# WesleyHsieh0806/TAO-Amodal

Measured on AMD Instinct MI355X. Metric: box-pair IoU+match throughput, higher is better.
Workload: dtype f64

## Files before the change

include/tao_amodal_hip.h:

```cpp
#ifndef TAO_AMODAL_HIP_H
#define TAO_AMODAL_HIP_H

#include <stddef.h>
#include <stdint.h>

#ifdef __cplusplus
extern "C" {
#endif

#define TAOAMD_N_THR 10
#define TAOAMD_N_REC 101
#define TAOAMD_LVIS_RNG 6
#define TAOAMD_TAO_RNG 20

#define TAOAMD_GT_IGNORE 1
#define TAOAMD_GT_OOF 2
#define TAOAMD_GT_ID_HIDDEN 4
#define TAOAMD_DT_IGNORE_UNMATCHED 1
#define TAOAMD_DT_NO_CONSUME 2

#define TAOAMD_OK 0
#define TAOAMD_ERR_HIP 1
#define TAOAMD_ERR_ARG 2
#define TAOAMD_ERR_TOO_LARGE 3
#define TAOAMD_ERR_WORKSPACE 4
#define TAOAMD_JSON_FALLBACK 16

const char *taoamd_strerror(int status);
const char *taoamd_last_error(void);
int taoamd_version(void);

int taoamd_kernel_timing_enable(int on);
int taoamd_kernel_timing_label(const char *label);
int taoamd_kernel_timing_collect(char *names_host, size_t names_bytes,
                                 double *total_ms_host, int64_t *calls_host,
                                 int32_t max_kernels, int32_t *n_kernels_host);

int taoamd_thresholds_host(double *iou_thrs, double *rec_thrs);

int taoamd_set_thresholds(const double *iou_thrs, const double *rec_thrs);
int taoamd_set_ranges(const double *visibility_rng, const double *area_rng,
                      const double *time_rng);

int taoamd_bb_iou(const double *dt, const double *gt, size_t m, size_t n,
                  const unsigned char *iscrowd, double *o, void *stream);
int taoamd_bb_iou_host(const double *dt, const double *gt, size_t m, size_t n,
                       const unsigned char *iscrowd, double *o);

int taoamd_lvis_ranges(int64_t n_gt, const double *gt_vis,
                       const uint8_t *gt_flags, const int32_t *gt_cat,
                       const int32_t *gt_cat_off, int64_t n_dt,
                       const uint8_t *dt_flags, int32_t n_cat,
                       uint32_t *gt_rng, uint32_t *dt_rng, int32_t *num_gt,
                       void *stream);
int taoamd_tao_ranges(int64_t n_gt, const double *gt_area,
                      const int32_t *gt_len, const int32_t *gt_nhp,
                      const uint8_t *gt_flags, const int32_t *gt_cat,
                      const int32_t *gt_cat_off, int64_t n_dt,
                      const double *dt_area, const int32_t *dt_len,
                      const uint8_t *dt_flags, int32_t n_cat,
                      uint32_t *gt_rng, uint32_t *dt_rng, int32_t *num_gt,
                      void *stream);

size_t taoamd_rle_iou_workspace(int64_t n_dt, int64_t dt_total, int64_t n_gt,
                                int64_t gt_total);
int taoamd_rle_iou(int64_t n_cells, const int32_t *cell_dt_off,
                   const int32_t *cell_gt_off, const int64_t *cell_iou_off,
                   int64_t n_dt, int64_t dt_total, const int64_t *dt_off,
                   const uint32_t *dt_runs, const int32_t *dt_hw,
                   const double *dt_bb, int64_t n_gt, int64_t gt_total,
                   const int64_t *gt_off, const uint32_t *gt_runs,
                   const int32_t *gt_hw, const double *gt_bb, double *iou,
                   void *workspace, size_t workspace_bytes, void *stream);

size_t taoamd_track_mask_iou_workspace(int64_t dt_frames, int64_t dt_total,
                                       int64_t gt_frames, int64_t gt_total);
int taoamd_track_mask_iou(int64_t n_cells, const int32_t *cell_dt_off,
                          const int32_t *cell_gt_off, const int64_t *cell_iou_off,
                          int64_t n_pairs, const int32_t *dt_frame_off,
                          const int32_t *dt_frame_pos, int64_t dt_frames,
                          int64_t dt_total, const int64_t *dt_off,
                          const uint32_t *dt_runs, const int32_t *dt_hw,
                          const int32_t *gt_frame_off,
                          const int32_t *gt_frame_pos, int64_t gt_frames,
                          int64_t gt_total, const int64_t *gt_off,
                          const uint32_t *gt_runs, const int32_t *gt_hw,
                          int32_t mode, double *iou,
                          int64_t *pair_frames, void *workspace,
                          size_t workspace_bytes, void *stream);

int taoamd_track_iou(int64_t n_cells, const int32_t *cell_dt_off,
                     const int32_t *cell_gt_off, const int64_t *cell_iou_off,
                     int64_t n_pairs, const int32_t *dt_frame_off,
                     const int32_t *dt_frame_pos, const double *dt_frame_box,
                     const int32_t *gt_frame_off, const int32_t *gt_frame_pos,
                     const double *gt_frame_box, int32_t mode, double *iou,
                     int64_t *pair_frames, void *stream);
int taoamd_track_iou_planned(int64_t n_tasks, const int32_t *tasks,
                             const int32_t *task_rows, const int32_t *task_pairs,
                             const int64_t *task_out, const double *frames,
                             const int32_t *task_base, const int32_t *trk_meta,
                             int32_t mode, double *iou, int64_t *pair_frames,
                             void *stream);

int taoamd_track_iou_single(int64_t n_dt, const int32_t *dt_group,
                            const int64_t *cell_iou_off, const int32_t *dt_frame_pos,
                            const double *dt_frame_box, const int32_t *gt_frame_pos,
                            const double *gt_frame_box, int32_t mode, double *iou,
                            int64_t *pair_frames, void *stream);

int taoamd_track_pad(int64_t n_trk, int64_t n_frames, const int32_t *frame_off,
                     const int32_t *frame_pos, const double *frame_box,
                     const int32_t *meta, int64_t slot_first, int64_t n_slots,
                     double *padded, int32_t *inexact, void *stream);

int taoamd_track_stream(int64_t n_tasks, const int32_t *tasks,
                        const int32_t *task_rows, const int32_t *trk_meta,
                        const int32_t *task_base, const double *padded,
                        double *frames, void *stream);

int taoamd_track_iou_near(int64_t n_cells, const int32_t *cell_gt_off,
                          const int64_t *cell_iou_off, int64_t n_pairs,
                          const double *iou, int32_t max_ulp, int32_t capacity,
                          int32_t *count, int64_t *list, void *stream);

int64_t taoamd_track_iou_setorder_table(int64_t max_dt_frames, int64_t max_gt_frames);
int taoamd_track_iou_setorder(
    int64_t n_cells, const int32_t *cell_dt_off, const int32_t *cell_gt_off,
    const int64_t *cell_iou_off, const int32_t *cell_unit, const int64_t *tl_vid_start,
    const int64_t *tl_image_id, const int32_t *dt_frame_off, const int32_t *dt_frame_pos,
    const double *dt_frame_box, const int32_t *gt_frame_off, const int32_t *gt_frame_pos,
    const double *gt_frame_box, int32_t mode, const int32_t *count, int32_t capacity,
    const int64_t *list, double *iou, int32_t *scratch, int64_t scratch_slots,
    int64_t table_cap, int32_t *status, void *stream);

int taoamd_set_order_iou_host(const int64_t *tl_image_id, int32_t n_dt,
                              const int32_t *dt_pos, const double *dt_box, int32_t n_gt,
                              const int32_t *gt_pos, const double *gt_box, int32_t mode,
                              double *out);
int taoamd_pyset_union_order_host(int64_t n_a, const int64_t *a, int64_t n_b,
                                  const int64_t *b, int64_t *out, int64_t *n_out);

int taoamd_track_iou_plan_host(int64_t n_cells, const int32_t *cell_dt_off_host,
                               const int32_t *cell_gt_off_host,
                               const int64_t *cell_iou_off_host,
                               const int32_t *trk_meta_host, int64_t *sizes,
                               int32_t *tasks_host, int32_t *task_rows_host,
                               int32_t *task_pairs_host, int64_t *task_out_host);

#define TAOAMD_MAX_GT_PER_CELL 3072
int taoamd_match(int64_t n_cells, const int32_t *cell_dt_off,
                 const int32_t *cell_gt_off, const int64_t *cell_iou_off,
                 int32_t max_gt_per_cell, const double *dt_box,
                 const double *gt_box, const double *iou, int32_t n_rng,
                 const uint32_t *gt_rng, const uint32_t *dt_rng,
                 const uint8_t *gt_flags, const uint8_t *dt_flags,
                 const int32_t *dst, int64_t out_stride, uint64_t *matched,
                 uint64_t *ignored, int32_t *match_gt, double *ious_out,
                 const int32_t *dt_group, const uint32_t *dt_meta,
                 const int32_t *groups, int32_t n_groups, const int32_t *singles,
                 int32_t n_singles, void *stream);

int taoamd_flat_map(int64_t n, const int64_t *image_id, const int64_t *category_id,
                    const double *bbox, const double *area_in, int64_t n_img,
                    const int64_t *img_ids, int64_t n_cat, const int64_t *cat_ids,
                    int32_t *img, int32_t *cat, double *area, int32_t *img_count,
                    int32_t *img_start, int32_t *img_first, int32_t *status,
                    void *stream);
int taoamd_flat_rank_drop(int64_t n, const int32_t *order, const int32_t *img,
                          const int32_t *img_start, int32_t max_dets,
                          uint8_t *dropped, void *stream);
int taoamd_flat_filter(int64_t n, const int32_t *unit, const int32_t *cat,
                       const double *area, const int64_t *category_id,
                       const uint8_t *dropped, int32_t n_unit, int64_t n_gkeys,
                       const int32_t *gkeys, const int32_t *unit_row,
                       const int64_t *neg_off, const int64_t *neg_val,
                       const int64_t *nel_off, const int64_t *nel_val,
                       int32_t area_flag, int32_t *key, uint8_t *flags,
                       int32_t *n_keep, void *stream);
int taoamd_flat_gather(int64_t n_keep, const int32_t *order, const double *score,
                       const uint8_t *flags, const int32_t *key,
                       const double *bbox, int32_t n_unit, int32_t *dt_row,
                       double *dt_score, uint8_t *dt_flags, int32_t *dt_key,
                       int32_t *dt_cat, double *dt_box, void *stream);
int taoamd_flat_count_bad(int64_t n, const double *bbox, const uint8_t *dropped,
                          int32_t *count, void *stream);
int taoamd_flat_ordscore(int64_t n, const int32_t *img, const int32_t *img_count,
                         const double *score, int32_t max_dets, double *out,
                         void *stream);
int taoamd_flat_ordinal(int64_t n, const int32_t *order, const int32_t *img,
                        const int32_t *img_start, int32_t max_dets,
                        int32_t *ordinal, uint8_t *dropped, void *stream);
int taoamd_flat_merge_cat(int64_t n, const int64_t *category_id, int64_t n_merge,
                          const int64_t *merge_src, const int64_t *merge_dst,
                          int64_t n_cat, const int64_t *cat_ids, int64_t *merged_id,
                          int32_t *cat, void *stream);
int taoamd_flat_split64(int64_t n, const int64_t *key, const int32_t *order,
                        int32_t *lo, int32_t *hi, void *stream);
int taoamd_flat_compose(int64_t n, const int32_t *outer, const int32_t *inner,
                        int32_t *out, void *stream);
int taoamd_flat_gather_cols(int64_t n, const int32_t *idx, const int32_t *src_i32,
                            int32_t *out_i32, const double *src_f64,
                            double *out_f64, const uint8_t *src_u8,
                            uint8_t *out_u8, void *stream);
int taoamd_flat_track_of(int64_t n, const int32_t *order, const int32_t *run_id,
                         const int32_t *run_start, const int64_t *video_id,
                         int32_t *trk, int32_t *status, void *stream);
int taoamd_flat_keys(int64_t n, const int32_t *img, const int32_t *ordinal,
                     const uint8_t *dropped, const int32_t *cat, const double *area,
                     const int32_t *trk, const int32_t *img_rank,
                     const int32_t *visit_rank, const double *img_frame,
                     const int32_t *tl_pos, double M, double *keep_key,
                     double *visit_key, double *frame_key, double *pos_key,
                     int32_t *trk_keep, int32_t *trk_sel, void *stream);
int taoamd_flat_track_kept(int64_t n_runs, const int32_t *run_trk,
                           const int32_t *run_start, int64_t n_sorted,
                           const int32_t *order_k, const double *score,
                           const int64_t *merged_id, double *trk_score,
                           int32_t *trk_first_kept, int32_t *status, void *stream);
int taoamd_flat_track_sel(int64_t n_runs, const int32_t *run_trk,
                          const int32_t *run_start, int64_t n_sorted,
                          const int32_t *order_s, const double *area,
                          const double *visit_key, const int32_t *img,
                          double *sel_area, int32_t *sel_len, int32_t *sel_frames,
                          double *sel_first, void *stream);
int taoamd_flat_track_filter(int64_t n_runs, const int32_t *run_trk,
                             const int32_t *sel_len, const int32_t *trk_first_kept,
                             const int32_t *cat, const int64_t *merged_id,
                             const int64_t *video_id, const int64_t *track_id,
                             int64_t n_vid, const int64_t *vid_ids, int64_t n_gkeys,
                             const int32_t *gkeys, const int32_t *vid_row,
                             const int64_t *neg_off, const int64_t *neg_val,
                             const int64_t *nel_off, const int64_t *nel_val,
                             int32_t *key, uint8_t *flags, int32_t *n_keep,
                             int32_t *status, void *stream);
int taoamd_flat_frames(int64_t n_trk, const int32_t *trk_run,
                       const int32_t *run_start, int64_t n_runs, int64_t n_sorted,
                       const int32_t *order_s, const int32_t *img,
                       const int32_t *tl_pos, const double *bbox,
                       const int32_t *frame_off, int32_t *frame_pos,
                       double *frame_box, void *stream);
int taoamd_flat_scan(int64_t n, const int32_t *count, int32_t *start,
                     int32_t *status2, void *stream);
size_t taoamd_flat_runs_workspace(int64_t n);
int taoamd_flat_runs(int64_t n, const int32_t *sorted_key, int32_t *run_id,
                     int32_t *run_key, int32_t *run_start, int32_t *n_runs,
                     void *workspace, size_t workspace_bytes, void *stream);
int taoamd_flat_runs_by(int64_t n, const int32_t *key, const int32_t *order,
                        int32_t *run_id, int32_t *run_key, int32_t *run_start,
                        int32_t *n_runs, void *workspace, size_t workspace_bytes,
                        void *stream);
int taoamd_flat_runs64_by(int64_t n, const int64_t *key, const int32_t *order,
                          int32_t *run_id, int64_t *run_key, int32_t *run_start,
                          int32_t *n_runs, void *workspace, size_t workspace_bytes,
                          void *stream);
int taoamd_flat_remap(int64_t n, const int32_t *id, const int32_t *map,
                      int32_t *out, void *stream);

int taoamd_match_plan_host(int64_t n_cells, const int32_t *cell_dt_off_host,
                           const int32_t *cell_gt_off_host, int32_t cap_d,
                           int32_t cap_g, int32_t cap_cell_g, int64_t *sizes,
                           int32_t *groups_host, int32_t *singles_host);

size_t taoamd_sort_workspace(int64_t n);
int taoamd_sort_by_cat_score(int64_t n, const int32_t *dt_cat,
                             const double *dt_score, int32_t *order,
                             int32_t *dst, void *workspace,
                             size_t workspace_bytes, void *stream);

#define TAOAMD_SORT_CHUNK (16 * 2816)
int taoamd_sort_plan_host(int32_t n_cat, const int32_t *cat_off_host, int64_t *sizes,
                          int32_t *chunks, int32_t *split_list, int32_t *stile_chunk,
                          int32_t *bucket_chunk);
size_t taoamd_sort_sampled_workspace(int64_t n, int64_t n_buckets, int32_t merge);
int taoamd_sort_sampled_cap_limit(int32_t limit);
int taoamd_sort_sampled_notify(void *event);
int taoamd_event_create(void **event);
int taoamd_event_destroy(void *event);
int taoamd_stream_wait_event(void *stream, void *event);
int taoamd_sort_sampled(int64_t n, int32_t n_cat, const int32_t *cat_off,
                        const int32_t *tile_off, int32_t n_tiles, int32_t max_segment,
                        const double *dt_score, int32_t n_chunks, const int32_t *chunks,
                        int32_t n_split, const int32_t *split_list, int32_t n_stiles,
                        const int32_t *stile_chunk, int32_t n_buckets,
                        const int32_t *bucket_chunk, int32_t *order, int32_t *dst,
                        void *workspace, size_t workspace_bytes, void *stream);

#define TAOAMD_SEGMENT_TILE 2816
size_t taoamd_sort_segments_workspace(int64_t n);
int taoamd_sort_segments(int64_t n, int32_t n_cat, const int32_t *cat_off,
                         const int32_t *tile_off, int32_t n_tiles,
                         int32_t max_segment, const int32_t *dt_cat,
                         const double *dt_score, int32_t *order, int32_t *dst,
                         void *workspace, size_t workspace_bytes, void *stream);

int taoamd_gather_rows(int64_t n, int32_t n_words, const uint64_t *src_matched,
                       const uint64_t *src_ignored, int64_t src_stride,
                       const int32_t *order, uint64_t *dst_matched,
                       uint64_t *dst_ignored, void *stream);

size_t taoamd_accumulate_workspace(int64_t n_dt, int32_t n_cat, int32_t n_rng);
size_t taoamd_compact_elems(int32_t n_cat, int32_t n_rng);
int taoamd_accumulate_compact(int64_t n_dt, int32_t n_cat, int32_t n_rng,
                              const int32_t *cat_off, const uint64_t *matched,
                              const uint64_t *ignored, const int32_t *num_gt,
                              int32_t k_begin, int32_t k_end, int32_t max_segment,
                              double *val, double *rec, void *workspace,
                              size_t workspace_bytes, void *stream);
int taoamd_finalize(int32_t n_cat, int32_t n_rng, const int32_t *num_gt,
                    const double *val, const double *rec, double *precision,
                    double *recall, void *stream);
int taoamd_accumulate(int64_t n_dt, int32_t n_cat, int32_t n_rng,
                      const int32_t *cat_off, const uint64_t *matched,
                      const uint64_t *ignored,
                      const int32_t *num_gt, int32_t max_segment, double *precision,
                      double *recall, void *workspace, size_t workspace_bytes,
                      void *stream);
int taoamd_accumulate_error(const void *workspace, void *stream, int32_t *flag_host);
int taoamd_accumulate_chunked(int64_t n_dt, int32_t n_cat, int32_t n_rng,
                      const int32_t *cat_off, const uint64_t *matched,
                      const uint64_t *ignored,
                      const int32_t *num_gt, int32_t max_segment, double *precision,
                      double *recall, void *workspace, size_t workspace_bytes,
                      void *stream);
int taoamd_accumulate_compact_chunked(int64_t n_dt, int32_t n_cat, int32_t n_rng,
                              const int32_t *cat_off, const uint64_t *matched,
                              const uint64_t *ignored, const int32_t *num_gt,
                              int32_t k_begin, int32_t k_end, int32_t max_segment,
                              double *val, double *rec, void *workspace,
                              size_t workspace_bytes, void *stream);
int taoamd_accumulate_sweep_mode(int32_t mode);
int taoamd_accumulate_plan_kind(int64_t n_dt, int32_t n_rng, int32_t max_segment);
int taoamd_accumulate_spin_limit(int32_t polls);
int taoamd_accumulate_giveup_counter(uint32_t *device_word);
int taoamd_accumulate_prepare(int64_t n_dt, int32_t n_cat, int32_t n_rng,
                              const int32_t *cat_off, int32_t max_segment,
                              void *workspace, size_t workspace_bytes, void *stream);
int taoamd_accumulate_prepared(int64_t n_dt, int32_t n_cat, int32_t n_rng,
                      const int32_t *cat_off, const uint64_t *matched,
                      const uint64_t *ignored,
                      const int32_t *num_gt, int32_t max_segment, double *precision,
                      double *recall, void *workspace, size_t workspace_bytes,
                      void *stream);
int taoamd_accumulate_by_order(int64_t n_dt, int32_t n_cat, int32_t n_rng,
                               const int32_t *cat_off, const int32_t *order,
                               const uint64_t *matched, const uint64_t *ignored,
                               const int32_t *num_gt, int32_t max_segment,
                               double *precision, double *recall, void *workspace,
                               size_t workspace_bytes, void *stream);
int taoamd_accumulate_by_order_prepared(int64_t n_dt, int32_t n_cat, int32_t n_rng,
                               const int32_t *cat_off, const int32_t *order,
                               const uint64_t *matched, const uint64_t *ignored,
                               const int32_t *num_gt, int32_t max_segment,
                               double *precision, double *recall, void *workspace,
                               size_t workspace_bytes, void *stream);
int taoamd_accumulate_by_order_chunked(int64_t n_dt, int32_t n_cat, int32_t n_rng,
                               const int32_t *cat_off, const int32_t *order,
                               const uint64_t *matched, const uint64_t *ignored,
                               const int32_t *num_gt, int32_t max_segment,
                               double *precision, double *recall, void *workspace,
                               size_t workspace_bytes, void *stream);

size_t taoamd_score_at_recall_workspace(int64_t n_dt, int32_t n_cat, int32_t n_rng);
int taoamd_score_at_recall(int64_t n_dt, int32_t n_cat, int32_t n_rng,
                           const int32_t *cat_off, const int32_t *order,
                           const uint64_t *matched, const uint64_t *ignored,
                           const double *score, const int32_t *score_order,
                           const int32_t *num_gt, double *scores, void *workspace, size_t workspace_bytes,
                           void *stream);

#define TAOAMD_ERROR_TYPES_TILE 256
#define TAOAMD_ERROR_TYPES_MAX_RNG 8
size_t taoamd_error_types_workspace(int64_t n_dt, int64_t n_gt, int32_t n_rng);
int taoamd_error_types(int64_t n_dt, int64_t n_gt, int32_t n_img, int32_t n_cat,
                       int32_t n_rng, int32_t slot, double bg_thr,
                       const int32_t *dt_cat, const double *dt_box,
                       const uint8_t *dt_flags, const int32_t *dt_gt0,
                       const int32_t *match_gt, int64_t match_stride,
                       const int32_t *gt_cat, const double *gt_box,
                       const uint32_t *gt_rng, const int32_t *img_gt_off,
                       const int32_t *img_gt, const int32_t *img_dt_off,
                       const int32_t *img_dt, int64_t *dt_counts, int64_t *gt_counts,
                       uint8_t *dt_type, void *workspace, size_t workspace_bytes,
                       void *stream);

#define TAOAMD_TRACK_ERROR_TYPES_TILE 16
size_t taoamd_track_error_types_workspace(int64_t n_dt, int64_t n_gt, int32_t n_rng);
int taoamd_track_error_types(int64_t n_dt, int64_t n_gt, int64_t n_cells, int64_t n_iou,
                             int32_t n_vid, int32_t n_cat, int32_t n_rng, int32_t slot,
                             double bg_thr, const int32_t *dt_cat, const uint32_t *dt_rng,
                             const int32_t *dt_group, const int64_t *cell_iou_off,
                             const double *iou, const int32_t *match_gt, int64_t match_stride,
                             const int32_t *gt_cat, const uint32_t *gt_rng,
                             const int32_t *dt_frame_off, const int32_t *dt_frame_pos,
                             const double *dt_frame_box, const int32_t *gt_frame_off,
                             const int32_t *gt_frame_pos, const double *gt_frame_box,
                             const int32_t *vid_gt_off, const int32_t *vid_gt,
                             const int32_t *vid_dt_off, const int32_t *vid_dt,
                             int64_t *dt_counts, int64_t *gt_counts, uint8_t *dt_type,
                             uint32_t *dt_over, void *workspace, size_t workspace_bytes,
                             void *stream);

size_t taoamd_exchange_chunk_bytes(int32_t block_cats, int32_t n_rng, int64_t capacity);
size_t taoamd_exchange_workspace(int32_t block_cats, int32_t n_rng, int32_t world);
int taoamd_exchange_sizes(int32_t block_cats, int32_t n_rng, int32_t world,
                          const int32_t *num_gt, int64_t *totals, void *workspace,
                          size_t workspace_bytes, void *stream);
int taoamd_exchange_pack(int32_t n_cat, int32_t n_rng, int32_t block_cats,
                         int32_t world, int32_t rank, const int32_t *num_gt,
                         const double *val, const double *rec, void *chunk,
                         int64_t capacity, int32_t *overflow, void *workspace,
                         size_t workspace_bytes, int32_t maps_ready, void *stream);
int taoamd_exchange_unpack(int32_t n_cat, int32_t n_rng, int32_t block_cats,
                           int32_t world, const void *chunks, int64_t capacity,
                           int32_t *num_gt_out, double *precision, double *recall,
                           int32_t *overflow, void *workspace,
                           size_t workspace_bytes, int32_t maps_ready, void *stream);

int taoamd_exchange_scores(int64_t n, const int32_t *dst, const double *score,
                           int64_t *out, void *stream);
int taoamd_exchange_positions(int64_t n_recv, int32_t world, int32_t block_cats,
                              const int64_t *scores, const int64_t *own_scores,
                              int32_t own_rank, const int64_t *src_base,
                              const int64_t *run_off, const int64_t *cat_base,
                              int32_t *pos, void *stream);
int taoamd_exchange_place(int64_t n_recv, int32_t world, int32_t n_words,
                          const uint64_t *rows, const uint64_t *own_rows,
                          int32_t own_rank, const int64_t *src_base,
                          const int32_t *pos, uint64_t *out, void *stream);

size_t taoamd_json_pred_workspace(size_t file_bytes);
void *taoamd_json_pred_open(const char *path, void *work, size_t work_bytes,
                            int32_t *status, char *err, size_t errlen, void *stream);
int64_t taoamd_json_pred_count(void *handle);
int taoamd_json_pred_convert(void *handle, int64_t *image_id, int64_t *category_id,
                             double *bbox, double *score, int64_t *track_id,
                             int64_t *video_id, int64_t *flag, int64_t *flag_at,
                             int32_t flag_cap, int32_t *n_flagged);
int taoamd_json_pred_read(void *handle, int64_t *image_id, int64_t *category_id,
                          double *bbox, double *score, int64_t *track_id,
                          int64_t *video_id, int64_t *flag, int64_t *flag_at,
                          int32_t flag_cap, int32_t *n_flagged);
void taoamd_json_pred_close(void *handle);

#ifdef __cplusplus
}
#endif
#endif
```

tao_amodal_amd/_lib.py:

```python
import ctypes as C
import os

HERE = os.path.dirname(os.path.abspath(__file__))
SO_PATH = os.environ.get("TAOAMD_LIBRARY") or os.path.join(HERE, "libtao_amodal_hip.so")

OK = 0
ERR_HIP, ERR_ARG, JSON_FALLBACK = 1, 2, 16
N_THR, N_REC = 10, 101
LVIS_RNG, TAO_RNG = 6, 20
MAX_GT_PER_CELL = 3072
SEGMENT_TILE = 2816
ERROR_TYPES_TILE = 256
TRACK_ERROR_TYPES_TILE = 16
ERROR_TYPES = ("TP", "IGNORED", "DUP", "LOC", "CLS", "BOTH", "BKG")

_vp, _i64, _i32, _sz = C.c_void_p, C.c_int64, C.c_int32, C.c_size_t

SIGNATURES = {
    "taoamd_strerror": (C.c_char_p, [C.c_int]),
    "taoamd_last_error": (C.c_char_p, []),
    "taoamd_version": (C.c_int, []),
    "taoamd_thresholds_host": (C.c_int, [_vp, _vp]),
    "taoamd_set_thresholds": (C.c_int, [_vp, _vp]),
    "taoamd_set_ranges": (C.c_int, [_vp, _vp, _vp]),
    "taoamd_kernel_timing_enable": (C.c_int, [C.c_int]),
    "taoamd_kernel_timing_label": (C.c_int, [C.c_char_p]),
    "taoamd_kernel_timing_collect": (C.c_int, [_vp, _sz, _vp, _vp, _i32, _vp]),
    "taoamd_bb_iou": (C.c_int, [_vp, _vp, _sz, _sz, _vp, _vp, _vp]),
    "taoamd_bb_iou_host": (C.c_int, [_vp, _vp, _sz, _sz, _vp, _vp]),
    "taoamd_lvis_ranges": (C.c_int, [_i64, _vp, _vp, _vp, _vp, _i64, _vp,
                                     _i32, _vp, _vp, _vp, _vp]),
    "taoamd_tao_ranges": (C.c_int, [_i64, _vp, _vp, _vp, _vp, _vp, _vp, _i64,
                                    _vp, _vp, _vp, _i32, _vp, _vp, _vp, _vp]),
    "taoamd_sort_segments_workspace": (_sz, [_i64]),
    "taoamd_sort_segments": (C.c_int, [_i64, _i32, _vp, _vp, _i32, _i32, _vp,
                                       _vp, _vp, _vp, _vp, _sz, _vp]),
    "taoamd_sort_plan_host": (C.c_int, [_i32, _vp, _vp, _vp, _vp, _vp, _vp]),
    "taoamd_sort_sampled_workspace": (_sz, [_i64, _i64, _i32]),
    "taoamd_sort_sampled_cap_limit": (C.c_int, [_i32]),
    "taoamd_sort_sampled_notify": (C.c_int, [_vp]),
    "taoamd_event_create": (C.c_int, [_vp]),
    "taoamd_event_destroy": (C.c_int, [_vp]),
    "taoamd_stream_wait_event": (C.c_int, [_vp, _vp]),
    "taoamd_sort_sampled": (C.c_int, [_i64, _i32, _vp, _vp, _i32, _i32, _vp, _i32, _vp,
                                      _i32, _vp, _i32, _vp, _i32, _vp, _vp, _vp, _vp,
                                      _sz, _vp]),
    "taoamd_track_iou": (C.c_int, [_i64, _vp, _vp, _vp, _i64, _vp, _vp, _vp,
                                   _vp, _vp, _vp, _i32, _vp, _vp, _vp]),
    "taoamd_track_iou_single": (C.c_int, [_i64, _vp, _vp, _vp, _vp, _vp, _vp, _i32,
                                          _vp, _vp, _vp]),
    "taoamd_track_iou_planned": (C.c_int, [_i64, _vp, _vp, _vp, _vp, _vp, _vp, _vp,
                                           _i32, _vp, _vp, _vp]),
    "taoamd_track_stream": (C.c_int, [_i64, _vp, _vp, _vp, _vp, _vp, _vp, _vp]),
    "taoamd_json_pred_workspace": (_sz, [_sz]),
    "taoamd_json_pred_open": (_vp, [C.c_char_p, _vp, _sz, _vp, C.c_char_p, _sz, _vp]),
    "taoamd_json_pred_count": (_i64, [_vp]),
    "taoamd_json_pred_read": (C.c_int, [_vp, _vp, _vp, _vp, _vp, _vp, _vp, _vp, _vp,
                                        _i32, _vp]),
    "taoamd_json_pred_convert": (C.c_int, [_vp, _vp, _vp, _vp, _vp, _vp, _vp, _vp, _vp,
                                           _i32, _vp]),
    "taoamd_json_pred_close": (None, [_vp]),
    "taoamd_track_pad": (C.c_int, [_i64, _i64, _vp, _vp, _vp, _vp, _i64, _i64,
                                   _vp, _vp, _vp]),
    "taoamd_track_iou_near": (C.c_int, [_i64, _vp, _vp, _i64, _vp, _i32, _i32,
                                        _vp, _vp, _vp]),
    "taoamd_track_iou_setorder_table": (_i64, [_i64, _i64]),
    "taoamd_track_iou_setorder": (C.c_int, [_i64, _vp, _vp, _vp, _vp, _vp, _vp, _vp,
                                            _vp, _vp, _vp, _vp, _vp, _i32, _vp, _i32,
                                            _vp, _vp, _vp, _i64, _i64, _vp, _vp]),
    "taoamd_set_order_iou_host": (C.c_int, [_vp, _i32, _vp, _vp, _i32, _vp, _vp,
                                            _i32, _vp]),
    "taoamd_pyset_union_order_host": (C.c_int, [_i64, _vp, _i64, _vp, _vp, _vp]),
    "taoamd_track_iou_plan_host": (C.c_int, [_i64, _vp, _vp, _vp, _vp, _vp,
                                             _vp, _vp, _vp, _vp]),
    "taoamd_flat_map": (C.c_int, [_i64, _vp, _vp, _vp, _vp, _i64, _vp, _i64, _vp,
                                  _vp, _vp, _vp, _vp, _vp, _vp, _vp, _vp]),
    "taoamd_flat_count_bad": (C.c_int, [_i64, _vp, _vp, _vp, _vp]),
    "taoamd_flat_ordscore": (C.c_int, [_i64, _vp, _vp, _vp, _i32, _vp, _vp]),
    "taoamd_flat_ordinal": (C.c_int, [_i64, _vp, _vp, _vp, _i32, _vp, _vp, _vp]),
    "taoamd_flat_merge_cat": (C.c_int, [_i64, _vp, _i64, _vp, _vp, _i64, _vp, _vp,
                                        _vp, _vp]),
    "taoamd_flat_split64": (C.c_int, [_i64, _vp, _vp, _vp, _vp, _vp]),
    "taoamd_flat_compose": (C.c_int, [_i64, _vp, _vp, _vp, _vp]),
    "taoamd_flat_gather_cols": (C.c_int, [_i64, _vp, _vp, _vp, _vp, _vp, _vp, _vp,
                                          _vp]),
    "taoamd_flat_track_of": (C.c_int, [_i64, _vp, _vp, _vp, _vp, _vp, _vp, _vp]),
    "taoamd_flat_keys": (C.c_int, [_i64, _vp, _vp, _vp, _vp, _vp, _vp, _vp, _vp,
                                   _vp, _vp, C.c_double, _vp, _vp, _vp, _vp, _vp,
                                   _vp, _vp]),
    "taoamd_flat_track_kept": (C.c_int, [_i64, _vp, _vp, _i64, _vp, _vp, _vp, _vp,
                                         _vp, _vp, _vp]),
    "taoamd_flat_track_sel": (C.c_int, [_i64, _vp, _vp, _i64, _vp, _vp, _vp, _vp,
                                        _vp, _vp, _vp, _vp, _vp]),
    "taoamd_flat_track_filter": (C.c_int, [_i64, _vp, _vp, _vp, _vp, _vp, _vp, _vp,
                                           _i64, _vp, _i64, _vp, _vp, _vp, _vp, _vp,
                                           _vp, _vp, _vp, _vp, _vp, _vp]),
    "taoamd_flat_frames": (C.c_int, [_i64, _vp, _vp, _i64, _i64, _vp, _vp, _vp,
                                     _vp, _vp, _vp, _vp, _vp]),
    "taoamd_flat_scan": (C.c_int, [_i64, _vp, _vp, _vp, _vp]),
    "taoamd_flat_runs_by": (C.c_int, [_i64, _vp, _vp, _vp, _vp, _vp, _vp, _vp, _sz,
                                      _vp]),
    "taoamd_flat_runs64_by": (C.c_int, [_i64, _vp, _vp, _vp, _vp, _vp, _vp, _vp,
                                        _sz, _vp]),
    "taoamd_flat_rank_drop": (C.c_int, [_i64, _vp, _vp, _vp, _i32, _vp, _vp]),
    "taoamd_flat_filter": (C.c_int, [_i64, _vp, _vp, _vp, _vp, _vp, _i32, _i64,
                                     _vp, _vp, _vp, _vp, _vp, _vp, _i32, _vp, _vp,
                                     _vp, _vp]),
    "taoamd_flat_gather": (C.c_int, [_i64, _vp, _vp, _vp, _vp, _vp, _i32, _vp,
                                     _vp, _vp, _vp, _vp, _vp, _vp]),
    "taoamd_flat_runs_workspace": (_sz, [_i64]),
    "taoamd_flat_runs": (C.c_int, [_i64, _vp, _vp, _vp, _vp, _vp, _vp, _sz, _vp]),
    "taoamd_flat_remap": (C.c_int, [_i64, _vp, _vp, _vp, _vp]),
    "taoamd_match_plan_host": (C.c_int, [_i64, _vp, _vp, _i32, _i32, _i32, _vp,
                                         _vp, _vp]),
    "taoamd_match": (C.c_int, [_i64, _vp, _vp, _vp, _i32, _vp, _vp, _vp, _i32,
                               _vp, _vp, _vp, _vp, _vp, _i64, _vp, _vp, _vp,
                               _vp, _vp, _vp, _vp, _i32, _vp, _i32, _vp]),
    "taoamd_gather_rows": (C.c_int, [_i64, _i32, _vp, _vp, _i64, _vp, _vp,
                                     _vp, _vp]),
    "taoamd_compact_elems": (_sz, [_i32, _i32]),
    "taoamd_accumulate_compact": (C.c_int, [_i64, _i32, _i32, _vp, _vp, _vp,
                                            _vp, _i32, _i32, _i32, _vp, _vp,
                                            _vp, _sz, _vp]),
    "taoamd_rle_iou_workspace": (_sz, [_i64, _i64, _i64, _i64]),
    "taoamd_rle_iou": (C.c_int, [_i64, _vp, _vp, _vp, _i64, _i64, _vp, _vp, _vp,
                                 _vp, _i64, _i64, _vp, _vp, _vp, _vp, _vp, _vp,
                                 _sz, _vp]),
    "taoamd_track_mask_iou_workspace": (_sz, [_i64, _i64, _i64, _i64]),
    "taoamd_track_mask_iou": (C.c_int, [_i64, _vp, _vp, _vp, _i64, _vp, _vp, _i64, _i64,
                                        _vp, _vp, _vp, _vp, _vp, _i64, _i64, _vp, _vp,
                                        _vp, _i32, _vp, _vp, _vp, _sz, _vp]),
    "taoamd_finalize": (C.c_int, [_i32, _i32, _vp, _vp, _vp, _vp, _vp, _vp]),
    "taoamd_exchange_chunk_bytes": (_sz, [_i32, _i32, _i64]),
    "taoamd_exchange_workspace": (_sz, [_i32, _i32, _i32]),
    "taoamd_exchange_sizes": (C.c_int, [_i32, _i32, _i32, _vp, _vp, _vp, _sz, _vp]),
    "taoamd_exchange_pack": (C.c_int, [_i32, _i32, _i32, _i32, _i32, _vp, _vp,
                                       _vp, _vp, _i64, _vp, _vp, _sz, _i32, _vp]),
    "taoamd_exchange_unpack": (C.c_int, [_i32, _i32, _i32, _i32, _vp, _i64, _vp,
                                         _vp, _vp, _vp, _vp, _sz, _i32, _vp]),
    "taoamd_exchange_scores": (C.c_int, [_i64, _vp, _vp, _vp, _vp]),
    "taoamd_exchange_positions": (C.c_int, [_i64, _i32, _i32, _vp, _vp, _i32, _vp, _vp,
                                            _vp, _vp, _vp]),
    "taoamd_exchange_place": (C.c_int, [_i64, _i32, _i32, _vp, _vp, _i32, _vp, _vp, _vp,
                                        _vp]),
    "taoamd_sort_workspace": (_sz, [_i64]),
    "taoamd_sort_by_cat_score": (C.c_int, [_i64, _vp, _vp, _vp, _vp, _vp, _sz,
                                           _vp]),
    "taoamd_accumulate_workspace": (_sz, [_i64, _i32, _i32]),
    "taoamd_accumulate": (C.c_int, [_i64, _i32, _i32, _vp, _vp, _vp, _vp, _i32,
                                    _vp, _vp, _vp, _sz, _vp]),
    "taoamd_accumulate_error": (C.c_int, [_vp, _vp, _vp]),
    "taoamd_accumulate_chunked": (C.c_int, [_i64, _i32, _i32, _vp, _vp, _vp, _vp, _i32,
                                            _vp, _vp, _vp, _sz, _vp]),
    "taoamd_accumulate_compact_chunked": (C.c_int, [_i64, _i32, _i32, _vp, _vp, _vp,
                                                    _vp, _i32, _i32, _i32, _vp, _vp,
                                                    _vp, _sz, _vp]),
    "taoamd_accumulate_sweep_mode": (C.c_int, [_i32]),
    "taoamd_accumulate_plan_kind": (C.c_int, [_i64, _i32, _i32]),
    "taoamd_accumulate_spin_limit": (C.c_int, [_i32]),
    "taoamd_accumulate_giveup_counter": (C.c_int, [_vp]),
    "taoamd_accumulate_prepare": (C.c_int, [_i64, _i32, _i32, _vp, _i32, _vp, _sz, _vp]),
    "taoamd_accumulate_prepared": (C.c_int, [_i64, _i32, _i32, _vp, _vp, _vp, _vp, _i32,
                                    _vp, _vp, _vp, _sz, _vp]),
    "taoamd_accumulate_by_order": (C.c_int, [_i64, _i32, _i32, _vp, _vp, _vp, _vp,
                                             _vp, _i32, _vp, _vp, _vp, _sz, _vp]),
    "taoamd_accumulate_by_order_prepared": (C.c_int, [_i64, _i32, _i32, _vp, _vp, _vp, _vp,
                                             _vp, _i32, _vp, _vp, _vp, _sz, _vp]),
    "taoamd_accumulate_by_order_chunked": (C.c_int, [_i64, _i32, _i32, _vp, _vp, _vp, _vp,
                                             _vp, _i32, _vp, _vp, _vp, _sz, _vp]),
    "taoamd_score_at_recall_workspace": (_sz, [_i64, _i32, _i32]),
    "taoamd_score_at_recall": (C.c_int, [_i64, _i32, _i32, _vp, _vp, _vp, _vp, _vp, _vp,
                                         _vp, _vp, _vp, _sz, _vp]),
    "taoamd_error_types_workspace": (_sz, [_i64, _i64, _i32]),
    "taoamd_error_types": (C.c_int, [_i64, _i64, _i32, _i32, _i32, _i32, C.c_double,
                                     _vp, _vp, _vp, _vp, _vp, _i64, _vp, _vp, _vp, _vp,
                                     _vp, _vp, _vp, _vp, _vp, _vp, _vp, _sz, _vp]),
    "taoamd_track_error_types_workspace": (_sz, [_i64, _i64, _i32]),
    "taoamd_track_error_types": (C.c_int, [_i64, _i64, _i64, _i64, _i32, _i32, _i32, _i32,
                                           C.c_double, _vp, _vp, _vp, _vp, _vp, _vp, _i64,
                                           _vp, _vp, _vp, _vp, _vp, _vp, _vp, _vp, _vp, _vp,
                                           _vp, _vp, _vp, _vp, _vp, _vp, _vp, _sz, _vp]),
}

_lib = None


class TaoAmdError(RuntimeError):
    pass


def load():
    global _lib
    if _lib is not None:
        return _lib
    import torch
    if not os.path.exists(SO_PATH):
        raise TaoAmdError(
            "HIP extension not built: %s is missing.  Run "
            "tao_amodal_amd/csrc/build.sh (or __graft_entry__.build()).  "
            "There is no CPU fallback." % SO_PATH)
    lib = C.CDLL(SO_PATH)
    for name, (res, args) in SIGNATURES.items():
        fn = getattr(lib, name)
        fn.restype = res
        fn.argtypes = args
    _lib = lib
    return lib


TIMING = False


def kernel_timing(on):
    global TIMING
    TIMING = bool(on)
    check(load().taoamd_kernel_timing_enable(int(TIMING)),
          "taoamd_kernel_timing_enable")


def kernel_timing_label(label):
    load().taoamd_kernel_timing_label(label.encode() if label else None)


def kernel_timings():
    import numpy as np
    names = C.create_string_buffer(8192)
    ms = np.zeros(128)
    calls = np.zeros(128, dtype=np.int64)
    n = C.c_int32(0)
    check(load().taoamd_kernel_timing_collect(
        C.addressof(names), len(names), ms.ctypes.data, calls.ctypes.data, 128,
        C.addressof(n)), "taoamd_kernel_timing_collect")
    out, raw = {}, names.raw.split(b"\0")
    for k in range(n.value):
        out[raw[k].decode()] = (float(ms[k]), int(calls[k]))
    return out


def set_constants(iou_thrs=None, rec_thrs=None, visibility_rng=None, area_rng=None,
                  time_rng=None):
    import numpy as np

    def arr(a, shape):
        if a is None:
            return None, None
        a = np.ascontiguousarray(a, dtype=np.float64).reshape(shape)
        return a, a.ctypes.data
    lib = load()
    i, ip = arr(iou_thrs, (N_THR,))
    r, rp = arr(rec_thrs, (N_REC,))
    check(lib.taoamd_set_thresholds(ip, rp), "taoamd_set_thresholds")
    v, vp = arr(visibility_rng, (5, 2))
    a, ap = arr(area_rng, (5, 2))
    t, tp = arr(time_rng, (4, 2))
    check(lib.taoamd_set_ranges(vp, ap, tp), "taoamd_set_ranges")


SWEEP_MODES = {"auto": -1, "chunked": 0, "lookback": 1, "twopass": 2}


def sweep_mode(mode="auto", spin_limit=0):
    lib = load()
    check(lib.taoamd_accumulate_sweep_mode(SWEEP_MODES[mode]), "taoamd_accumulate_sweep_mode")
    check(lib.taoamd_accumulate_spin_limit(int(spin_limit)), "taoamd_accumulate_spin_limit")


def check(status, what):
    if status != OK:
        lib = load()
        raise TaoAmdError("%s failed: %s [%s]" % (
            what, lib.taoamd_strerror(status).decode(),
            lib.taoamd_last_error().decode()))
```

tao_amodal_amd/csrc/accumulate.hip:

```cpp
#include <atomic>
#include <cstdlib>
#include <cstring>

#include "common.hpp"
#include "transpose64.hpp"
#include "workspace.hpp"

using namespace taoamd;

#ifndef ACC_CH
#define ACC_CH 256
#endif
#ifndef ACC_INLINE_CHUNKS
#define ACC_INLINE_CHUNKS 64
#endif

struct AccArgs {
    int64_t n_dt;
    int32_t n_cat, n_rng, n_words, n_chunks_max;
    int32_t paired;
    int32_t wide;
    const int32_t *cat_off;
    const uint64_t *matched;
    const uint64_t *ignored;
    const int32_t *order;
    const int32_t *num_gt;
    int32_t *cat_chunk_off;
    const int32_t *chunk_tab;
    uint32_t *cnt_tp, *cnt_fp;
    uint32_t *pre_tp, *pre_fp;
    uint64_t *t_tp, *t_fp;
    uint64_t *cmax;
    int32_t *cj;
    uint64_t *val;
    double *rec;
    int32_t k_begin, k_end;
    int32_t fused_rows;
    int32_t fused_lo;
    int32_t inline_scans;
    int32_t sc_rows;
    uint32_t sc_gen;
    uint64_t *sc_stat;
    uint64_t *sc_max;
    uint8_t *sc_jhi;
    uint32_t *sc_error;
    uint32_t *sc_giveups;
    int32_t *xcd_start;
    int32_t sc_spin;
};

__global__ __launch_bounds__(256) void acc_chunks_kernel(AccArgs a)
{
    __shared__ int32_t part[256];
    const int per = (a.n_cat + 255) / 256;
    const int lo = threadIdx.x * per, hi = min(lo + per, a.n_cat);
    int32_t s = 0;
    auto chunks_of = [&](int k) {
        const int32_t rows = a.cat_off[k + 1] - a.cat_off[k];
        if (a.fused_rows > 0 && rows <= a.fused_rows) return 0;
        if ((a.inline_scans || a.sc_rows) && rows == 0) return 1;
        const int32_t per = a.sc_rows ? a.sc_rows : ACC_CH;
        return (rows + per - 1) / per;
    };
    for (int k = lo; k < hi; k++) s += chunks_of(k);
    part[threadIdx.x] = s;
    __syncthreads();
    for (int off = 1; off < 256; off <<= 1) {
        int32_t v = threadIdx.x >= off ? part[threadIdx.x - off] : 0;
        __syncthreads();
        part[threadIdx.x] += v;
        __syncthreads();
    }
    int32_t run = part[threadIdx.x] - s;
    for (int k = lo; k < hi; k++) {
        a.cat_chunk_off[k] = run;
        run += chunks_of(k);
    }
    if (threadIdx.x == 255) a.cat_chunk_off[a.n_cat] = part[255];
    if (a.xcd_start == nullptr) return;
    __syncthreads();
    if (threadIdx.x <= N_XCD) {
        const int32_t total = part[255];
        const int32_t want = (int32_t)((int64_t)total * threadIdx.x / N_XCD);
        int32_t lo = 0, hi = a.n_cat;
        while (lo < hi) {
            const int32_t mid = (lo + hi) >> 1;
            if (a.cat_chunk_off[mid] < want) lo = mid + 1; else hi = mid;
        }
        a.xcd_start[threadIdx.x] = threadIdx.x == N_XCD ? total : a.cat_chunk_off[lo];
    }
}

__device__ __forceinline__ int32_t chunk_cat(const int32_t *__restrict__ off,
                                             int32_t n_cat, int32_t c)
{
    int32_t lo = 0, hi = n_cat;
    while (hi - lo > 1) {
        int32_t mid = (lo + hi) >> 1;
        if (off[mid] <= c) lo = mid; else hi = mid;
    }
    return lo;
}

__global__ void acc_chunktab_kernel(AccArgs a, int32_t *__restrict__ tab)
{
    const int32_t c = blockIdx.x * blockDim.x + threadIdx.x;
    if (c < a.cat_chunk_off[a.n_cat]) tab[c] = chunk_cat(a.cat_chunk_off, a.n_cat, c);
}

__device__ __forceinline__ uint64_t readlane_u64(uint64_t v, int lane)
{
    uint32_t lo = (uint32_t)__builtin_amdgcn_readlane((int)(uint32_t)v, lane);
    uint32_t hi = (uint32_t)__builtin_amdgcn_readlane((int)(uint32_t)(v >> 32), lane);
    return ((uint64_t)hi << 32) | lo;
}

__device__ __forceinline__ void load_rows(const AccArgs &a, int64_t first, int word,
                                          int n, int lane, uint64_t &tpw,
                                          uint64_t &fpw)
{
    uint64_t m = 0, i = ~0ull;
    if (lane < n) {
        int64_t r = first + lane;
        if (a.order) r = a.order[r];
        if (a.wide) {
            const ulonglong2 v =
                *reinterpret_cast<const ulonglong2 *>(a.matched + 2 * (r * a.n_words + word));
            m = v.x;
            i = v.y;
        } else if (a.paired) {
            m = a.matched[2 * (r * a.n_words + word)];
            i = a.matched[2 * (r * a.n_words + word) + 1];
        } else {
            m = a.matched[r * a.n_words + word];
            i = a.ignored[r * a.n_words + word];
        }
    }
    tpw = m & ~i;
    fpw = ~m & ~i;
}

template <int ACC_BLK_N>
__device__ __forceinline__ void load_chunk(const AccArgs &a, int64_t start, int word, int len,
                                           int lane, uint64_t (&tpw)[ACC_BLK_N],
                                           uint64_t (&fpw)[ACC_BLK_N])
{
    if (a.wide && a.order == nullptr && len > 0) {
        ulonglong2 v[ACC_BLK_N];
#pragma unroll
        for (int blk = 0; blk < ACC_BLK_N; blk++) {
            const int i = blk * WAVE + lane;
            const int64_t r = start + (i < len ? i : 0);
            v[blk] = *reinterpret_cast<const ulonglong2 *>(a.matched + 2 * (r * a.n_words + word));
        }
#pragma unroll
        for (int blk = 0; blk < ACC_BLK_N; blk++) {
            const bool in = blk * WAVE + lane < len;
            const uint64_t m = in ? v[blk].x : 0, i_ = in ? v[blk].y : ~0ull;
            tpw[blk] = m & ~i_;
            fpw[blk] = ~m & ~i_;
        }
        return;
    }
    if (a.wide && a.order != nullptr && len > 0) {
        int32_t at[ACC_BLK_N];
#pragma unroll
        for (int blk = 0; blk < ACC_BLK_N; blk++) {
            const int i = blk * WAVE + lane;
            at[blk] = a.order[start + (i < len ? i : 0)];
        }
        ulonglong2 v[ACC_BLK_N];
#pragma unroll
        for (int blk = 0; blk < ACC_BLK_N; blk++)
            v[blk] = *reinterpret_cast<const ulonglong2 *>(
                a.matched + 2 * ((int64_t)at[blk] * a.n_words + word));
#pragma unroll
        for (int blk = 0; blk < ACC_BLK_N; blk++) {
            const bool in = blk * WAVE + lane < len;
            const uint64_t m = in ? v[blk].x : 0, i_ = in ? v[blk].y : ~0ull;
            tpw[blk] = m & ~i_;
            fpw[blk] = ~m & ~i_;
        }
        return;
    }
#pragma unroll
    for (int blk = 0; blk < ACC_BLK_N; blk++)
        load_rows(a, start + blk * WAVE, word, max(0, min(WAVE, len - blk * WAVE)), lane,
                  tpw[blk], fpw[blk]);
}

template <int ACC_BLK_N, bool GATHER = false>
__device__ __forceinline__ void load_chunk_tv(const AccArgs &a, int64_t start, int word, int len,
                                              int lane, uint64_t (&tpw)[ACC_BLK_N],
                                              uint64_t (&vw)[ACC_BLK_N])
{
    if (GATHER && a.wide && len == ACC_BLK_N * WAVE) {
        const int32_t *__restrict__ ob = a.order + start;
        uint32_t at[ACC_BLK_N];
#pragma unroll
        for (int blk = 0; blk < ACC_BLK_N; blk++) at[blk] = (uint32_t)ob[blk * WAVE + lane];
        const char *base = reinterpret_cast<const char *>(a.matched + 2 * word);
        const uint32_t row_bytes = (uint32_t)a.n_words * 16u;
        ulonglong2 v[ACC_BLK_N];
#pragma unroll
        for (int blk = 0; blk < ACC_BLK_N; blk++)
            v[blk] = *reinterpret_cast<const ulonglong2 *>(base + (uint64_t)at[blk] * row_bytes);
#pragma unroll
        for (int blk = 0; blk < ACC_BLK_N; blk++) {
            tpw[blk] = v[blk].x & ~v[blk].y;
            vw[blk] = ~v[blk].y;
        }
        return;
    }
    if (!GATHER && a.wide && a.order == nullptr && len == ACC_BLK_N * WAVE) {
        const char *base = reinterpret_cast<const char *>(a.matched + 2 * (start * a.n_words + word));
        const uint32_t lane_off = (uint32_t)lane * (uint32_t)a.n_words * 16u;
        const uint32_t blk_off = (uint32_t)WAVE * (uint32_t)a.n_words * 16u;
        ulonglong2 v[ACC_BLK_N];
#pragma unroll
        for (int blk = 0; blk < ACC_BLK_N; blk++)
            v[blk] = *reinterpret_cast<const ulonglong2 *>(base + ((uint32_t)blk * blk_off + lane_off));
#pragma unroll
        for (int blk = 0; blk < ACC_BLK_N; blk++) {
            tpw[blk] = v[blk].x & ~v[blk].y;
            vw[blk] = ~v[blk].y;
        }
        return;
    }
    uint64_t fpw[ACC_BLK_N];
    load_chunk(a, start, word, len, lane, tpw, fpw);
#pragma unroll
    for (int blk = 0; blk < ACC_BLK_N; blk++) vw[blk] = tpw[blk] | fpw[blk];
}

#define ACC_BLK (ACC_CH / WAVE)

struct ChunkInfo {
    int32_t k, first, last;
    int64_t start;
    int32_t len, c, word;
    bool valid;
};

__device__ __forceinline__ ChunkInfo chunk_info(const AccArgs &a)
{
    ChunkInfo ci;
    const int wave = __builtin_amdgcn_readfirstlane(threadIdx.x >> 6);
    const int64_t item = (int64_t)blockIdx.x * 4 + wave;
    ci.c = (int32_t)(item / a.n_words);
    ci.word = (int32_t)(item - (int64_t)ci.c * a.n_words);
    const int32_t total = a.cat_chunk_off[a.n_cat];
    ci.valid = ci.c < total;
    if (!ci.valid) return ci;
    ci.k = a.chunk_tab ? a.chunk_tab[ci.c] : chunk_cat(a.cat_chunk_off, a.n_cat, ci.c);
    const int32_t j = ci.c - a.cat_chunk_off[ci.k];
    ci.start = (int64_t)a.cat_off[ci.k] + (int64_t)j * ACC_CH;
    const int64_t end = a.cat_off[ci.k + 1];
    ci.len = (int32_t)min((int64_t)ACC_CH, end - ci.start);
    ci.first = j == 0;
    ci.last = ci.c + 1 == a.cat_chunk_off[ci.k + 1];
    return ci;
}

__global__ __launch_bounds__(256) void acc_count_kernel(AccArgs a)
{
    const ChunkInfo ci = chunk_info(a);
    if (!ci.valid) return;
    const int lane = lane_id();
    uint32_t tp = 0, fp = 0;
    const int64_t tb = (((int64_t)ci.c * a.n_words + ci.word) * ACC_BLK) * WAVE + lane;
    uint64_t tpw[ACC_BLK], fpw[ACC_BLK];
    load_chunk(a, ci.start, ci.word, ci.len, lane, tpw, fpw);
#pragma unroll
    for (int blk = 0; blk < ACC_BLK; blk++) {
        uint64_t T = 0, F = 0;
        if (blk * WAVE < ci.len) {
            T = transpose64(tpw[blk], lane);
            F = transpose64(fpw[blk], lane);
        }
        a.t_tp[tb + (int64_t)blk * WAVE] = T;
        a.t_fp[tb + (int64_t)blk * WAVE] = F;
        tp += (uint32_t)__popcll(T);
        fp += (uint32_t)__popcll(F);
    }
    const int64_t o = ((int64_t)ci.c * a.n_words + ci.word) * WAVE + lane;
    a.cnt_tp[o] = tp;
    a.cnt_fp[o] = fp;
}

__global__ __launch_bounds__(256) void acc_prefix_kernel(AccArgs a, RecThr rec)
{
    __shared__ uint32_t s_tp[4][WAVE], s_fp[4][WAVE];
    const int wave = __builtin_amdgcn_readfirstlane(threadIdx.x >> 6);
    const int64_t item = blockIdx.x;
    const int32_t k = a.k_begin + (int32_t)(item / a.n_words);
    const int word = (int)(item % a.n_words);
    const int lane = lane_id();
    if (a.fused_rows > 0 && a.cat_off[k + 1] - a.cat_off[k] <= a.fused_rows)
        return;
    if (word == 0)
        for (int i = threadIdx.x; i < a.n_rng * N_REC; i += 256) {
            const int64_t kr = (int64_t)k * a.n_rng + i / N_REC;
            const int32_t ng = a.num_gt[kr];
            if (ng > 0)
                a.cj[kr * N_REC + i % N_REC] = recall_crossing(rec.v[i % N_REC], ng);
        }
    const int32_t c0 = a.cat_chunk_off[k], c1 = a.cat_chunk_off[k + 1];
    const int32_t q = (c1 - c0 + 3) / 4;
    const int32_t lo = min(c1, c0 + wave * q), hi = min(c1, lo + q);
    uint32_t tp = 0, fp = 0;
    for (int32_t c = lo; c < hi; c += 8) {
        uint32_t t_[8], f_[8];
#pragma unroll
        for (int u = 0; u < 8; u++) {
            const int64_t o = ((int64_t)min(c + u, hi - 1) * a.n_words + word) * WAVE + lane;
            t_[u] = a.cnt_tp[o];
            f_[u] = a.cnt_fp[o];
        }
#pragma unroll
        for (int u = 0; u < 8; u++) {
            if (c + u < hi) {
                const int64_t o = ((int64_t)(c + u) * a.n_words + word) * WAVE + lane;
                a.pre_tp[o] = tp;
                a.pre_fp[o] = fp;
                tp += t_[u];
                fp += f_[u];
            }
        }
    }
    s_tp[wave][lane] = tp;
    s_fp[wave][lane] = fp;
    __syncthreads();
    uint32_t btp = 0, bfp = 0;
    for (int w = 0; w < wave; w++) { btp += s_tp[w][lane]; bfp += s_fp[w][lane]; }
    if (wave > 0 && (__ballot(btp | bfp) != 0))
        for (int32_t c = lo; c < hi; c++) {
            const int64_t o = ((int64_t)c * a.n_words + word) * WAVE + lane;
            a.pre_tp[o] += btp;
            a.pre_fp[o] += bfp;
        }
    if (wave != 3) return;
    tp += btp;
    const int combo = word * WAVE + lane;
    if (combo < a.n_rng * N_THR) {
        const int r = combo / N_THR, t = combo - r * N_THR;
        const int32_t ng = a.num_gt[(int64_t)k * a.n_rng + r];
        if (ng > 0) {
            const int64_t kr = (int64_t)k * a.n_rng + r;
            a.rec[kr * N_THR + t] = (double)tp / (double)ng;
// ... 338 lines not shown
    __shared__ uint64_t s_max[FW][WAVE];
    __shared__ int32_t s_cj[32 * N_REC];
    const int lane = lane_id();
    const int wave = __builtin_amdgcn_readfirstlane(threadIdx.x >> 6);
    const int32_t k = a.k_begin + (int32_t)blockIdx.x;
    const int32_t sb = a.cat_off[k], se = a.cat_off[k + 1];
    if (se - sb > a.fused_rows || se - sb <= a.fused_lo) return;
    const int nw = a.n_words;
    const int nch = (se - sb + ACC_CH - 1) / ACC_CH;
    const int j = wave / nw, word = wave - j * nw;
    const bool mine = j < nch;
    const int32_t start = sb + j * ACC_CH;
    const int len = mine ? min(ACC_CH, se - start) : 0;
    for (int i = threadIdx.x; i < a.n_rng * N_REC; i += FW * WAVE) {
        const int q = i / N_REC;
        const int32_t ngq = a.num_gt[(int64_t)k * a.n_rng + q];
        s_cj[i] = ngq > 0 ? recall_crossing(rec.v[i - q * N_REC], ngq) : 0;
    }
    uint64_t T[ACC_BLK], TF[ACC_BLK];
    uint32_t tp_own = 0, fp_own = 0;
    {
        uint64_t tpw[ACC_BLK], fpw[ACC_BLK];
        load_chunk(a, (int64_t)start, word, len, lane, tpw, fpw);
#pragma unroll
        for (int blk = 0; blk < ACC_BLK; blk++) {
            const int base = blk * WAVE;
            uint64_t t_ = 0, f_ = 0;
            if (base < len) {
                t_ = transpose64(tpw[blk], lane);
                f_ = transpose64(fpw[blk], lane);
            }
            T[blk] = t_;
            TF[blk] = t_ | f_;
            tp_own += (uint32_t)__popcll(t_);
            fp_own += (uint32_t)__popcll(f_);
        }
    }
    s_tp[wave][lane] = tp_own;
    s_fp[wave][lane] = fp_own;
    __syncthreads();
    uint32_t tp0 = 0, fp0 = 0;
    for (int jj = 0; jj < j && jj < nch; jj++) {
        tp0 += s_tp[jj * nw + word][lane];
        fp0 += s_fp[jj * nw + word][lane];
    }
    const int combo = word * WAVE + lane;
    const bool active = combo < a.n_rng * N_THR;
    const int r = active ? combo / N_THR : 0;
    const int t = active ? combo - r * N_THR : 0;
    const int32_t ng = active ? a.num_gt[(int64_t)k * a.n_rng + r] : 0;
    const bool live = active && ng > 0;
    const int64_t kr = (int64_t)k * a.n_rng + r;
    uint64_t *__restrict__ out = a.val + (kr * N_THR + t) * N_REC;
    const bool last = mine && j == nch - 1, first = mine && j == 0;
    if (live && (last || (nch == 0 && j == 0 && wave < nw))) {
        a.rec[kr * N_THR + t] = (double)(tp0 + tp_own) / (double)ng;
        if (nch == 0)
            for (int jj = 0; jj < N_REC; jj++) out[jj] = PR_ZERO;
    }
    uint64_t best = PR_ZERO;
    {
        uint32_t tpb = tp0, nb = tp0 + fp0;
#pragma unroll
        for (int blk = 0; blk < ACC_BLK; blk++) {
            best_of_block(T[blk], TF[blk], tpb, nb, best);
        }
    }
    s_max[wave][lane] = best;
    __syncthreads();
    if (!mine) return;
    uint64_t run = PR_ZERO;
    for (int jj = nch - 1; jj > j; jj--) {
        const uint64_t v = s_max[jj * nw + word][lane];
        if (pr_better((uint32_t)(v >> 32), (uint32_t)v, run)) run = v;
    }
    const int32_t *__restrict__ cj = s_cj + r * N_REC;
    uint32_t tp = tp0 + tp_own;
    uint32_t n = tp + fp0 + fp_own;
    int jcur = 0;
    if (live) {
        int lo = 0, hi = N_REC;
        while (lo < hi) {
            const int mid = (lo + hi) >> 1;
            if (cj[mid] <= (int32_t)tp) lo = mid + 1; else hi = mid;
        }
        jcur = lo;
    }
    if (last) {
        const int jz = live ? jcur : N_REC;
        for (int l = 0; l < WAVE; l++) {
            const int jl = __builtin_amdgcn_readlane(jz, l);
            if (jl >= N_REC) continue;
            const int cl = word * WAVE + l;
            const int rl = cl / N_THR, tl = cl - rl * N_THR;
            uint64_t *__restrict__ row =
                a.val + (((int64_t)k * a.n_rng + rl) * N_THR + tl) * N_REC;
            for (int jj = jl + lane; jj < N_REC; jj += WAVE) row[jj] = PR_ZERO;
        }
    }
    int32_t cnext = jcur > 0 ? cj[jcur - 1] : -1;
#pragma unroll
    for (int blk = ACC_BLK - 1; blk >= 0; blk--) {
        if (blk * WAVE >= len) continue;
        emit_block<4>(live ? T[blk] : 0, live ? TF[blk] : 0, tp, n, run, jcur, cnext, out, cj);
    }
    if (live && first && jcur > 0) {
        const uint64_t v = run;
        while (jcur > 0) {
            out[jcur - 1] = v;
            jcur--;
        }
    }
}

#define SC_SPIN_LIMIT (1 << 18)
#define SWEEP_NB 8
#ifndef SWEEP_SW
#define SWEEP_SW 4
#endif
#define SC_FLAG_AGG 1ull
#define SC_FLAG_PRE 2ull
__device__ __forceinline__ uint64_t sc_status(uint32_t gen, uint64_t flag, uint32_t v)
{
    return ((uint64_t)gen << 34) | (flag << 32) | v;
}
__device__ __forceinline__ void sc_publish(uint64_t *p, uint64_t v)
{
    __hip_atomic_store(p, v, __ATOMIC_RELAXED, __HIP_MEMORY_SCOPE_AGENT);
}
__device__ __forceinline__ uint64_t sc_peek(const uint64_t *p)
{
    return __hip_atomic_load(p, __ATOMIC_RELAXED, __HIP_MEMORY_SCOPE_AGENT);
}

__device__ __forceinline__ void sc_raise(uint64_t *__restrict__ out, int jlo, int jhi,
                                         uint64_t later)
{
    const uint32_t lt = (uint32_t)(later >> 32), ln = (uint32_t)later;
    for (int j = jlo; j < jhi; j++) {
        const uint64_t v = out[j];
        if (pr_better(lt, ln, v)) out[j] = later;
    }
}

__global__ void acc_cj_kernel(AccArgs a, RecThr rec)
{
    const int64_t i = (int64_t)blockIdx.x * blockDim.x + threadIdx.x;
    if (i >= (int64_t)a.n_cat * a.n_rng * N_REC) return;
    const int64_t kr = i / N_REC;
    const int32_t ng = a.num_gt[kr];
    a.cj[i] = ng > 0 ? recall_crossing(rec.v[i - kr * N_REC], ng) : 0;
}

template <int SW, int MODE, bool GATHER = false, int NB = SWEEP_NB>
__global__ __launch_bounds__(SW * WAVE) __attribute__((amdgpu_waves_per_eu(8, 8)))
void acc_sweep_kernel(AccArgs a, RecThr rec)
{
    __shared__ uint32_t s_tp[SW][WAVE], s_fp[SW][WAVE];
    __shared__ uint64_t s_max[SW][WAVE];
    __shared__ uint32_t s_pre[2][WAVE];
    __shared__ int32_t s_cj[EMIT_RMAX][N_REC];
    __shared__ uint16_t s_jr[SW][WAVE];
    __shared__ int32_t s_done;
    const int lane = lane_id();
    const int wave = __builtin_amdgcn_readfirstlane(threadIdx.x >> 6);
    if (threadIdx.x == 0) s_done = 0;
    int32_t item = (int32_t)blockIdx.x;
    if (a.xcd_start != nullptr) {
        const int32_t x = item % (int32_t)N_XCD, i = item / (int32_t)N_XCD;
        item = a.xcd_start[x] * a.n_words + i;
        if (item >= a.xcd_start[x + 1] * a.n_words) return;
    }
    const int32_t sc = item / a.n_words;
    const int word = item - sc * a.n_words;
    if (sc >= a.cat_chunk_off[a.n_cat]) return;
    const int32_t k = a.chunk_tab ? a.chunk_tab[sc] : chunk_cat(a.cat_chunk_off, a.n_cat, sc);
    const int32_t jsc = sc - a.cat_chunk_off[k];
    const int64_t cat_begin = a.cat_off[k], cat_end = a.cat_off[k + 1];
    const int64_t start = cat_begin + ((int64_t)jsc * SW + wave) * (NB * WAVE);
    const int len = (int)max((int64_t)0, min((int64_t)(NB * WAVE), cat_end - start));
    const bool swept = k >= a.k_begin && k < a.k_end;
    uint64_t tpw[NB], vw[NB];
    load_chunk_tv<NB, GATHER>(a, start, word, len, lane, tpw, vw);
    const int r_lo = (word * WAVE) / N_THR;
    const int r_hi = min(a.n_rng - 1, (word * WAVE + WAVE - 1) / N_THR);
    if (MODE != 2) {
        const int32_t *__restrict__ src = a.cj + ((int64_t)k * a.n_rng + r_lo) * N_REC;
        for (int i = threadIdx.x; i < (r_hi - r_lo + 1) * N_REC; i += SW * WAVE)
            (&s_cj[0][0])[i] = src[i];
    }
    uint64_t T[NB], TF[NB];
    uint32_t tp_own = 0, n_own = 0;
#pragma unroll
    for (int blk = 0; blk < NB; blk++) {
        uint64_t t_ = 0, v_ = 0;
        if (blk * WAVE < len) {
#if defined(SW_ABLATE) && (SW_ABLATE & 2)
            t_ = tpw[blk];
            v_ = vw[blk];
#else
            t_ = transpose64(tpw[blk], lane);
            v_ = transpose64(vw[blk], lane);
#endif
        }
        T[blk] = t_;
        TF[blk] = v_;
        tp_own += (uint32_t)__popcll(t_);
        n_own += (uint32_t)__popcll(v_);
    }
    const uint32_t fp_own = n_own - tp_own;
#if defined(SW_ABLATE) && (SW_ABLATE & 8)
    if (tp_own + n_own == (uint32_t)a.sc_spin) a.sc_max[0] = n_own;
    return;
#endif
    s_tp[wave][lane] = tp_own;
    s_fp[wave][lane] = fp_own;
    __syncthreads();
    uint32_t tp0 = 0, fp0 = 0;
    for (int w = 0; w < wave; w++) {
        tp0 += s_tp[w][lane];
        fp0 += s_fp[w][lane];
    }
    const int64_t so = ((int64_t)sc * a.n_words + word) * WAVE + lane;
    if (MODE == 2) {
        if (wave == SW - 1) {
            a.cnt_tp[so] = tp0 + tp_own;
            a.cnt_fp[so] = fp0 + fp_own;
        }
        return;
    }
    if (wave == SW - 1) {
        const uint32_t tot_t = tp0 + tp_own, tot_f = fp0 + fp_own;
        uint32_t acc_t = 0, acc_f = 0;
        if (MODE == 0) {
            uint64_t *st = a.sc_stat + 2 * so;
            const uint64_t mine = jsc == 0 ? SC_FLAG_PRE : SC_FLAG_AGG;
            sc_publish(st, sc_status(a.sc_gen, mine, tot_t));
            sc_publish(st + 1, sc_status(a.sc_gen, mine, tot_f));
            bool open = jsc > 0;
#if defined(SW_ABLATE) && (SW_ABLATE & 4)
            open = false;
#endif
            const int64_t stride = 2 * (int64_t)a.n_words * WAVE;
            const uint64_t *p = st - stride;
            for (int32_t jj = jsc - 1; jj >= 0 && __ballot(open) != 0; jj--, p -= stride) {
                uint64_t vt, vf;
                for (int spin = 0;; spin++) {
                    vt = sc_peek(p);
                    vf = sc_peek(p + 1);
                    const uint32_t ft = (uint32_t)(vt >> 32) & 3, ff = (uint32_t)(vf >> 32) & 3;
                    const bool ready = (uint32_t)(vt >> 34) == a.sc_gen &&
                                       (uint32_t)(vf >> 34) == a.sc_gen && ft != 0 && ft == ff;
                    if (a.sc_spin >= 0 && __ballot(open && !ready) == 0) break;
                    if (spin >= a.sc_spin) {
                        if (lane == 0) {
                            atomicOr(a.sc_error, 1u);
                            if (a.sc_giveups) atomicAdd(a.sc_giveups, 1u);
                        }
                        vt = vf = 0;
                        break;
                    }
                    __builtin_amdgcn_s_sleep(2);
                }
                if (open) {
                    acc_t += (uint32_t)vt;
                    acc_f += (uint32_t)vf;
                    if (((vt >> 32) & 3) == SC_FLAG_PRE) open = false;
                }
            }
            if (jsc > 0) {
                sc_publish(st, sc_status(a.sc_gen, SC_FLAG_PRE, acc_t + tot_t));
                sc_publish(st + 1, sc_status(a.sc_gen, SC_FLAG_PRE, acc_f + tot_f));
            }
        } else {
            for (int32_t jj = 0; jj < jsc; jj++) {
                const int64_t o = ((int64_t)(sc - jsc + jj) * a.n_words + word) * WAVE + lane;
                acc_t += a.cnt_tp[o];
                acc_f += a.cnt_fp[o];
            }
        }
        s_pre[0][lane] = acc_t;
        s_pre[1][lane] = acc_f;
    }
    __syncthreads();
    tp0 += s_pre[0][lane];
    fp0 += s_pre[1][lane];
#if defined(SW_ABLATE) && (SW_ABLATE & 16)
    if (tp0 + fp0 == (uint32_t)a.sc_spin) a.sc_max[0] = T[0] ^ TF[NB - 1];
    return;
#endif
    const int combo = word * WAVE + lane;
    const bool active = combo < a.n_rng * N_THR;
    const int r = active ? combo / N_THR : 0;
    const int t = active ? combo - r * N_THR : 0;
    const int64_t kr = (int64_t)k * a.n_rng + r;
    const int32_t ng = active ? a.num_gt[kr] : 0;
    const bool live = active && ng > 0 && swept;
    const int32_t *__restrict__ cj = s_cj[active ? r - r_lo : 0];
    uint64_t *__restrict__ out = a.val + (kr * N_THR + t) * N_REC;
    uint32_t tp = tp0 + tp_own;
    uint32_t n = tp + fp0 + fp_own;
    const bool is_last = len > 0 ? start + len == cat_end : (cat_end == cat_begin && wave == 0);
    const bool is_first = jsc == 0 && wave == 0;
    int jcur = 0;
    if (live) {
        int lo = 0, hi = N_REC;
        while (lo < hi) {
            const int mid = (lo + hi) >> 1;
            if (cj[mid] <= (int32_t)tp) lo = mid + 1; else hi = mid;
        }
        jcur = lo;
    }
    const int jhi = jcur;
    if (is_last) {
        if (live) a.rec[kr * N_THR + t] = (double)tp / (double)ng;
        const int jz = live ? (len == 0 ? 0 : jcur) : N_REC;
        for (uint64_t need = __ballot(jz < N_REC); need != 0; need &= need - 1) {
            const int l = __builtin_ctzll(need);
            const int jl = __builtin_amdgcn_readlane(jz, l);
            uint64_t *__restrict__ row = (uint64_t *)readlane_u64((uint64_t)out, l);
            for (int j = jl + lane; j < N_REC; j += WAVE) row[j] = PR_ZERO;
        }
    }
    uint64_t run = PR_ZERO;
    int32_t cnext = jcur > 0 ? cj[jcur - 1] : -1;
#pragma unroll
    for (int blk = NB - 1; blk >= 0; blk--) {
        if (blk * WAVE >= len) continue;
#if defined(SW_ABLATE) && (SW_ABLATE & 1)
        run ^= T[blk] + TF[blk];
#else
        emit_block<1>(live ? T[blk] : 0, live ? TF[blk] : 0, tp, n, run, jcur, cnext, out, cj);
#endif
    }
    if (live && is_first && jcur > 0 && len > 0) {
        const uint64_t v = run;
        while (jcur > 0) {
            out[jcur - 1] = v;
            jcur--;
        }
    }
    s_max[wave][lane] = run;
    s_jr[wave][lane] = (uint16_t)((len > 0 ? jcur : jhi) | (jhi << 8));
    __builtin_amdgcn_fence(__ATOMIC_RELEASE, "workgroup");
    int done = 0;
    if (lane == 0) done = atomicAdd(&s_done, 1);
    done = __builtin_amdgcn_readfirstlane(done);
    if (done != SW - 1) return;
    __builtin_amdgcn_fence(__ATOMIC_ACQUIRE, "workgroup");
    uint64_t later = PR_ZERO;
    for (int w = SW - 1; w >= 0; w--) {
        const int jr = s_jr[w][lane];
        if (live && later != PR_ZERO) sc_raise(out, jr & 0xff, jr >> 8, later);
        const uint64_t v = s_max[w][lane];
        if (pr_better((uint32_t)(v >> 32), (uint32_t)v, later)) later = v;
    }
    a.sc_max[so] = live ? later : PR_ZERO;
    a.sc_jhi[so] = (uint8_t)(live ? s_jr[SW - 1][lane] >> 8 : 0);
}

__device__ __forceinline__ uint64_t pr_max(uint64_t a, uint64_t b)
{
    return pr_better((uint32_t)(a >> 32), (uint32_t)a, b) ? a : b;
}
__global__ __launch_bounds__(256) void acc_raise_kernel(AccArgs a)
{
    __shared__ uint64_t s_env[4][N_REC + 3];
    const int lane = lane_id();
    const int wave = __builtin_amdgcn_readfirstlane(threadIdx.x >> 6);
    const int64_t row = (int64_t)blockIdx.x * 4 + wave;
    const int64_t rows = (int64_t)(a.k_end - a.k_begin) * a.n_rng * N_THR;
    if (row >= rows) return;
    const int32_t k = a.k_begin + (int32_t)(row / (a.n_rng * N_THR));
    const int combo = (int)(row % (a.n_rng * N_THR));
    const int32_t s0 = a.cat_chunk_off[k], s1 = a.cat_chunk_off[k + 1];
    if (s1 - s0 < 2) return;
    if (a.num_gt[(int64_t)k * a.n_rng + combo / N_THR] <= 0) return;
    uint64_t *env = s_env[wave];
    for (int j = lane; j < N_REC; j += WAVE) env[j] = PR_ZERO;
    const int64_t step = (int64_t)a.n_words * WAVE;
    const int64_t o0 = ((int64_t)combo / WAVE) * WAVE + combo % WAVE;
    uint64_t behind = PR_ZERO;
    for (int32_t top = s1; top > s0; top -= WAVE) {
        const int32_t sc = top - 1 - lane;
        const bool have = sc >= s0;
        const int64_t o = (int64_t)(have ? sc : s0) * step + o0;
        uint64_t v = have ? a.sc_max[o] : PR_ZERO;
        const int jh = have ? (int)a.sc_jhi[o] : 0;
        const int jl = (have && sc > s0) ? (int)a.sc_jhi[o - step] : 0;
#pragma unroll
        for (int d = 1; d < WAVE; d <<= 1) {
            const uint32_t lo = (uint32_t)__shfl_up((int)(uint32_t)v, d, WAVE);
            const uint32_t hi = (uint32_t)__shfl_up((int)(uint32_t)(v >> 32), d, WAVE);
            const uint64_t u = ((uint64_t)hi << 32) | lo;
            if (lane >= d) v = pr_max(u, v);
        }
        const uint32_t elo = (uint32_t)__shfl_up((int)(uint32_t)v, 1, WAVE);
        const uint32_t ehi = (uint32_t)__shfl_up((int)(uint32_t)(v >> 32), 1, WAVE);
        uint64_t after = lane > 0 ? (((uint64_t)ehi << 32) | elo) : PR_ZERO;
        after = pr_max(after, behind);
        if (have && after != PR_ZERO)
            for (int j = jl; j < jh; j++) env[j] = after;
        behind = pr_max(behind, readlane_u64(v, WAVE - 1));
    }
    __builtin_amdgcn_fence(__ATOMIC_ACQ_REL, "workgroup");
    __builtin_amdgcn_wave_barrier();
    uint64_t *__restrict__ out = a.val + ((int64_t)k * a.n_rng * N_THR + combo) * N_REC;
    for (int j = lane; j < N_REC; j += WAVE) {
        const uint64_t e = env[j];
        if (e != PR_ZERO) {
            const uint64_t v = out[j];
            if (pr_better((uint32_t)(e >> 32), (uint32_t)e, v)) out[j] = e;
        }
    }
}

struct FinArgs {
    int32_t n_cat, n_rng;
    const int32_t *num_gt;
    const uint64_t *val;
    const double *rec;
    double *precision, *recall;
};

#define FIN_RT 64
#define FIN_CT 64

__global__ __launch_bounds__(256) void acc_finalize_kernel(FinArgs a)
{
    __shared__ double tile[FIN_RT][FIN_CT + 1];
    const int64_t KR = (int64_t)a.n_cat * a.n_rng;
    const int64_t COLS = (int64_t)N_THR * N_REC;
    const int64_t row0 = (int64_t)blockIdx.x * FIN_RT;
    const int64_t col0 = (int64_t)blockIdx.y * FIN_CT;
    const int lane = lane_id(), wave = threadIdx.x >> 6;
    const int ncol = (int)min((int64_t)FIN_CT, COLS - col0);
    const int64_t orow = row0 + lane;
    const bool olive = orow < KR && a.num_gt[orow] > 0;
    const uint64_t live_rows = __ballot(olive);
    static_assert(FIN_RT == 64 && FIN_CT == 64, "one mask word, one lane per column");
    if (live_rows != 0) {
        uint64_t m = live_rows & (0x1111111111111111ull << wave);
        const int64_t col = col0 + lane;
        const uint64_t *__restrict__ src =
            a.val + row0 * COLS + (lane < ncol ? col : col0);
        while (m != 0) {
            int idx[4];
#pragma unroll
            for (int q = 0; q < 4; q++) {
                idx[q] = m != 0 ? __builtin_ctzll(m) : -1;
                if (m != 0) m &= m - 1;
            }
            uint64_t v[4];
#pragma unroll
            for (int q = 0; q < 4; q++)
                v[q] = idx[q] >= 0 ? src[(int64_t)idx[q] * COLS] : PR_ZERO;
#pragma unroll
            for (int q = 0; q < 4; q++)
                if (idx[q] >= 0) tile[idx[q]][lane] = pr_value(v[q]);
        }
        __syncthreads();
    }
    if (orow < KR)
        for (int c = wave; c < ncol; c += 4)
            a.precision[(col0 + c) * KR + orow] = olive ? tile[lane][c] : -1.0;
    if (blockIdx.y == 0) {
        for (int i = threadIdx.x; i < FIN_RT * N_THR; i += 256) {
            const int64_t row = row0 + i / N_THR;
            const int t = i % N_THR;
            if (row < KR)
                a.recall[(int64_t)t * KR + row] =
                    a.num_gt[row] > 0 ? a.rec[row * N_THR + t] : -1.0;
        }
    }
}

static int32_t max_chunks(int64_t n_dt, int32_t n_cat)
{
    return (int32_t)((n_dt + ACC_CH - 1) / ACC_CH + n_cat);
}

enum { SWEEP_AUTO = -1, SWEEP_CHUNKED = 0, SWEEP_LOOKBACK = 1, SWEEP_TWOPASS = 2 };
#define SWEEP_ONEPASS_MIN 6000000
static std::atomic<int> g_sweep_set{SWEEP_AUTO};
static std::atomic<int> g_sweep_spin{0};
static std::atomic<uint32_t *> g_sweep_giveups{nullptr};
static int sweep_mode(int64_t n_dt)
{
    static const int env = [] {
        const char *e = getenv("TAOAMD_SWEEP");
        if (e && !strcmp(e, "lookback")) return (int)SWEEP_LOOKBACK;
        if (e && !strcmp(e, "twopass")) return (int)SWEEP_TWOPASS;
        if (e && !strcmp(e, "chunked")) return (int)SWEEP_CHUNKED;
        return (int)SWEEP_AUTO;
    }();
    const int set = g_sweep_set.load(std::memory_order_relaxed);
    const int m = set != SWEEP_AUTO ? set : env;
    if (m != SWEEP_AUTO) return m;
    return n_dt >= SWEEP_ONEPASS_MIN ? (int)SWEEP_LOOKBACK : (int)SWEEP_CHUNKED;
}

extern "C" int taoamd_accumulate_sweep_mode(int32_t mode)
{
    if (mode < SWEEP_AUTO || mode > SWEEP_TWOPASS) return TAOAMD_ERR_ARG;
    g_sweep_set.store(mode, std::memory_order_relaxed);
    return TAOAMD_OK;
}

static bool sweep_mode_explicit_onepass()
{
    const int set = g_sweep_set.load(std::memory_order_relaxed);
    const char *e = set == SWEEP_AUTO ? getenv("TAOAMD_SWEEP") : nullptr;
    return set == SWEEP_LOOKBACK || set == SWEEP_TWOPASS ||
           (e && (!strcmp(e, "lookback") || !strcmp(e, "twopass")));
}

extern "C" int taoamd_accumulate_plan_kind(int64_t n_dt, int32_t n_rng, int32_t max_segment)
{
    if (n_rng < 1 || n_rng > 32) return -1;
    const int32_t n_words = (n_rng * N_THR + 63) / 64;
    const int32_t fused_cap = ACC_FUSED_WAVES / n_words * ACC_CH;
    if (max_segment > 0 && max_segment <= fused_cap && !sweep_mode_explicit_onepass()) return 0;
    return 1 + sweep_mode(n_dt);
}

extern "C" int taoamd_accumulate_spin_limit(int32_t polls)
{
    g_sweep_spin.store(polls, std::memory_order_relaxed);
    return TAOAMD_OK;
}

extern "C" int taoamd_accumulate_giveup_counter(uint32_t *device_word)
{
    g_sweep_giveups.store(device_word, std::memory_order_relaxed);
    return TAOAMD_OK;
}
#define SC_TICKETS 64
static std::atomic<uint32_t> g_sc_gen{0};

static size_t max_scs(int64_t n_dt, int32_t n_cat)
{
    return (size_t)(n_dt / (SWEEP_SW * SWEEP_NB * WAVE) + n_cat + 1);
}

extern "C" size_t taoamd_compact_elems(int32_t n_cat, int32_t n_rng)
{
    return (size_t)n_cat * n_rng * N_THR * N_REC;
}

struct AccWs {
    uint32_t *header;
    size_t head_bytes;
    int32_t *xcd_start, *chunk_tab;
};

static AccWs acc_layout(Carve &c, int64_t n_dt, int32_t n_cat, int32_t n_rng, AccArgs &a)
{
    a.n_words = (n_rng * N_THR + 63) / 64;
    a.n_chunks_max = max_chunks(n_dt, n_cat);
    const size_t nw = (size_t)a.n_words, nc = (size_t)a.n_chunks_max;
    const size_t ns = max_scs(n_dt, n_cat);
    AccWs t;
    static_assert(SC_TICKETS * 4 % 256 == 0, "sc_stat starts a 256-byte line");
    t.head_bytes = SC_TICKETS * 4 + ns * nw * WAVE * 16;
    t.header = (uint32_t *)c.take<uint64_t>(t.head_bytes / 8);
    a.sc_stat = (uint64_t *)Carve::at(t.header, SC_TICKETS);
    a.sc_max = c.take<uint64_t>(ns * nw * WAVE);
    a.sc_jhi = c.take<uint8_t>(ns * nw * WAVE);
    a.cat_chunk_off = c.take<int32_t>((size_t)n_cat + 1);
    t.xcd_start = c.take<int32_t>(N_XCD + 1);
    t.chunk_tab = c.take<int32_t>(nc);
    for (uint32_t **p : {&a.cnt_tp, &a.cnt_fp, &a.pre_tp, &a.pre_fp})
        *p = c.take<uint32_t>(nc * nw * WAVE);
    a.cmax = c.take<uint64_t>(nc * nw * WAVE);
    for (uint64_t **p : {&a.t_tp, &a.t_fp}) *p = c.take<uint64_t>(nc * nw * ACC_BLK * WAVE);
    a.cj = c.take<int32_t>((size_t)n_cat * n_rng * N_REC);
    return t;
}

static void acc_full_layout(Carve &c, int64_t n_dt, int32_t n_cat, int32_t n_rng,
                            double *&val, double *&rec)
{
    AccArgs a;
    acc_layout(c, n_dt, n_cat, n_rng, a);
    val = c.take<double>(taoamd_compact_elems(n_cat, n_rng));
    rec = c.take<double>((size_t)n_cat * n_rng * N_THR);
}

extern "C" size_t taoamd_accumulate_workspace(int64_t n_dt, int32_t n_cat,
                                              int32_t n_rng)
{
    double *val, *rec;
    return measure([&](Carve &c) { acc_full_layout(c, n_dt, n_cat, n_rng, val, rec); });
}

enum { ACC_ALL = 0, ACC_PLAN = 1, ACC_SWEEP = 2 };

static int accumulate_compact(int64_t n_dt, int32_t n_cat, int32_t n_rng,
                              const int32_t *cat_off, const int32_t *order,
                              const uint64_t *matched, const uint64_t *ignored,
                              const int32_t *num_gt, int32_t k_begin, int32_t k_end,
                              int32_t max_segment, double *val, double *rec,
                              void *workspace, size_t workspace_bytes, void *stream,
                              int phase = ACC_ALL, int force_mode = SWEEP_AUTO)
{
    if (n_cat <= 0 || n_rng < 1 || n_rng > 32) return TAOAMD_ERR_ARG;
    if (k_begin < 0 || k_end > n_cat || k_begin > k_end) return TAOAMD_ERR_ARG;
    if (!cat_off || !workspace) return TAOAMD_ERR_ARG;
    if (phase != ACC_PLAN && (!num_gt || !val || !rec)) return TAOAMD_ERR_ARG;
    Carve c(workspace);
    AccArgs a;
    const AccWs t = acc_layout(c, n_dt, n_cat, n_rng, a);
    if (!c.fits(workspace, workspace_bytes)) return TAOAMD_ERR_WORKSPACE;
    if (k_begin == k_end) return TAOAMD_OK;
    hipStream_t s = (hipStream_t)stream;
    a.chunk_tab = nullptr;
    a.n_dt = n_dt; a.n_cat = n_cat; a.n_rng = n_rng;
    a.cat_off = cat_off; a.matched = matched; a.ignored = ignored; a.order = order;
    a.paired = matched != nullptr && ignored == matched + 1;
    a.wide = a.paired && ((uintptr_t)matched & 15) == 0;
    a.num_gt = num_gt; a.val = (uint64_t *)val; a.rec = rec;
    a.k_begin = k_begin; a.k_end = k_end;
    a.inline_scans = 0;
    a.sc_rows = 0; a.sc_gen = 0;
    a.sc_error = nullptr;
    a.sc_giveups = g_sweep_giveups.load(std::memory_order_relaxed);
    a.xcd_start = nullptr;
    {
        const int sp = g_sweep_spin.load(std::memory_order_relaxed);
        a.sc_spin = sp == 0 ? SC_SPIN_LIMIT : sp;
    }
    if (phase != ACC_SWEEP)
        TAO_HIP(hipMemsetAsync(t.header, 0, SC_TICKETS * 4, s));
    const int32_t fused_cap = ACC_FUSED_WAVES / a.n_words * ACC_CH;
    const bool all_fused = max_segment > 0 && max_segment <= fused_cap &&
                           (force_mode == SWEEP_CHUNKED || !sweep_mode_explicit_onepass());
    a.fused_rows = 0;
    a.fused_lo = -1;
    if (all_fused && phase == ACC_PLAN) return TAOAMD_OK;
    if (all_fused) {
        const unsigned grid = (unsigned)(k_end - k_begin);
        int32_t lo = -1;
        for (int fw = 4; fw <= ACC_FUSED_WAVES; fw *= 2) {
            const int32_t hi = fw / a.n_words * ACC_CH;
            if (hi <= lo || hi == 0) continue;
            a.fused_lo = lo;
            a.fused_rows = hi;
            if (fw == 4) {
                TAO_TIMED("acc_fused_kernel", s, acc_fused_kernel<4><<<grid, 4 * WAVE, 0, s>>>(a, rec_thr()));
            } else if (fw == 8) {
                TAO_TIMED("acc_fused_kernel", s, acc_fused_kernel<8><<<grid, 8 * WAVE, 0, s>>>(a, rec_thr()));
            } else {
                TAO_TIMED("acc_fused_kernel", s, acc_fused_kernel<16><<<grid, 16 * WAVE, 0, s>>>(a, rec_thr()));
            }
            lo = hi;
            if (max_segment > 0 && max_segment <= hi) break;
        }
        TAO_LAUNCH_CHECK();
        return TAOAMD_OK;
    }
    a.inline_scans = max_segment > 0 && max_segment <= ACC_INLINE_CHUNKS * ACC_CH;
    const size_t nc = (size_t)a.n_chunks_max, nw = (size_t)a.n_words;
    const int mode = force_mode != SWEEP_AUTO ? force_mode : sweep_mode(n_dt);
    if (mode != SWEEP_CHUNKED) {
        a.sc_rows = SWEEP_SW * SWEEP_NB * WAVE;
        a.inline_scans = 0;
    }
    if (mode != SWEEP_CHUNKED && max_segment > 0) a.xcd_start = t.xcd_start;
    if (phase == ACC_SWEEP) a.chunk_tab = t.chunk_tab;
    const unsigned chunk_blocks = (unsigned)((nc * nw + 3) / 4);
    const unsigned cat_blocks = (unsigned)((size_t)(k_end - k_begin) * nw);
    if (phase != ACC_SWEEP)
        TAO_TIMED("acc_chunks_kernel", s, acc_chunks_kernel<<<1, 256, 0, s>>>(a));
    if (phase == ACC_PLAN) {
        TAO_TIMED("acc_chunktab_kernel", s, acc_chunktab_kernel<<<(unsigned)((nc + 255) / 256), 256, 0, s>>>(a, t.chunk_tab));
        if (mode != SWEEP_CHUNKED)
            TAO_HIP(hipMemsetAsync(t.header, 0, t.head_bytes, s));
        TAO_LAUNCH_CHECK();
        return TAOAMD_OK;
    }
    if (mode != SWEEP_CHUNKED) {
        {
            const int64_t n_cj = (int64_t)n_cat * n_rng * N_REC;
            TAO_TIMED("acc_cj_kernel", s, acc_cj_kernel<<<(unsigned)((n_cj + 255) / 256), 256, 0, s>>>(a, rec_thr()));
        }
        const size_t n_sc = (size_t)(n_dt / a.sc_rows) + (size_t)n_cat + 1;
        const unsigned grid = a.xcd_start == nullptr
            ? (unsigned)(n_sc * nw)
            : (unsigned)(N_XCD * (n_sc / N_XCD + (size_t)max_segment / a.sc_rows + 3) * nw);
        if (mode == SWEEP_LOOKBACK) {
            if (phase == ACC_ALL)
                TAO_HIP(hipMemsetAsync(t.header, 0, t.head_bytes, s));
            uint32_t g = ++g_sc_gen;
            a.sc_gen = (g & 0x3fffffffu) ? (g & 0x3fffffffu) : (++g_sc_gen & 0x3fffffffu);
            a.sc_error = t.header;
            if (a.order)
                TAO_TIMED("acc_sweep_kernel", s, (acc_sweep_kernel<SWEEP_SW, 0, true><<<grid, SWEEP_SW * WAVE, 0, s>>>(a, rec_thr())));
            else
                TAO_TIMED("acc_sweep_kernel", s, (acc_sweep_kernel<SWEEP_SW, 0><<<grid, SWEEP_SW * WAVE, 0, s>>>(a, rec_thr())));
        } else if (a.order) {
            TAO_TIMED("acc_sccount_kernel", s, (acc_sweep_kernel<SWEEP_SW, 2, true><<<grid, SWEEP_SW * WAVE, 0, s>>>(a, rec_thr())));
            TAO_TIMED("acc_sweep_kernel", s, (acc_sweep_kernel<SWEEP_SW, 1, true><<<grid, SWEEP_SW * WAVE, 0, s>>>(a, rec_thr())));
        } else {
            TAO_TIMED("acc_sccount_kernel", s, (acc_sweep_kernel<SWEEP_SW, 2><<<grid, SWEEP_SW * WAVE, 0, s>>>(a, rec_thr())));
            TAO_TIMED("acc_sweep_kernel", s, (acc_sweep_kernel<SWEEP_SW, 1><<<grid, SWEEP_SW * WAVE, 0, s>>>(a, rec_thr())));
        }
        const int64_t rows = (int64_t)(k_end - k_begin) * n_rng * N_THR;
        TAO_TIMED("acc_raise_kernel", s, acc_raise_kernel<<<(unsigned)((rows + 3) / 4), 256, 0, s>>>(a));
        TAO_LAUNCH_CHECK();
        return TAOAMD_OK;
    }
    TAO_TIMED("acc_count_kernel", s, acc_count_kernel<<<chunk_blocks, 256, 0, s>>>(a));
    if (a.inline_scans) {
        TAO_TIMED("acc_chunkmax_kernel", s, acc_chunkmax_kernel<true><<<chunk_blocks, 256, 0, s>>>(a, rec_thr()));
        TAO_TIMED("acc_emit_kernel", s, acc_emit_kernel<true><<<chunk_blocks, 256, 0, s>>>(a));
    } else {
        TAO_TIMED("acc_prefix_kernel", s, acc_prefix_kernel<<<cat_blocks, 256, 0, s>>>(a, rec_thr()));
        TAO_TIMED("acc_chunkmax_kernel", s, acc_chunkmax_kernel<false><<<chunk_blocks, 256, 0, s>>>(a, rec_thr()));
        TAO_TIMED("acc_sufmax_kernel", s, acc_sufmax_kernel<<<cat_blocks, 256, 0, s>>>(a));
        TAO_TIMED("acc_emit_kernel", s, acc_emit_kernel<false><<<chunk_blocks, 256, 0, s>>>(a));
    }
    TAO_LAUNCH_CHECK();
    return TAOAMD_OK;
}

extern "C" int taoamd_accumulate_error(const void *workspace, void *stream, int32_t *flag_host)
{
    if (!workspace || !flag_host) return TAOAMD_ERR_ARG;
    Carve c((void *)workspace);
    AccArgs a;
    const uint32_t *w = acc_layout(c, 0, 1, 1, a).header;
    uint32_t f = 0;
    TAO_HIP(hipMemcpyAsync(&f, w, sizeof f, hipMemcpyDeviceToHost, (hipStream_t)stream));
    TAO_HIP(hipStreamSynchronize((hipStream_t)stream));
    *flag_host = (int32_t)f;
    return TAOAMD_OK;
}

extern "C" int taoamd_accumulate_compact(int64_t n_dt, int32_t n_cat,
                                         int32_t n_rng, const int32_t *cat_off,
                                         const uint64_t *matched,
                                         const uint64_t *ignored,
                                         const int32_t *num_gt, int32_t k_begin,
                                         int32_t k_end, int32_t max_segment,
                                         double *val, double *rec,
                                         void *workspace, size_t workspace_bytes,
                                         void *stream)
{
    return accumulate_compact(n_dt, n_cat, n_rng, cat_off, nullptr, matched, ignored,
                              num_gt, k_begin, k_end, max_segment, val, rec,
                              workspace, workspace_bytes, stream);
}

extern "C" int taoamd_finalize(int32_t n_cat, int32_t n_rng,
                               const int32_t *num_gt, const double *val,
                               const double *rec, double *precision,
                               double *recall, void *stream)
{
    if (n_cat <= 0 || n_rng < 1 || n_rng > 32) return TAOAMD_ERR_ARG;
    if (!num_gt || !val || !rec || !precision || !recall) return TAOAMD_ERR_ARG;
    FinArgs f;
    f.n_cat = n_cat; f.n_rng = n_rng; f.num_gt = num_gt; f.val = (const uint64_t *)val; f.rec = rec;
    f.precision = precision; f.recall = recall;
    const int64_t KR = (int64_t)n_cat * n_rng;
    dim3 grid((unsigned)((KR + FIN_RT - 1) / FIN_RT),
              (unsigned)((N_THR * N_REC + FIN_CT - 1) / FIN_CT));
    TAO_TIMED("acc_finalize_kernel", (hipStream_t)stream, acc_finalize_kernel<<<grid, 256, 0, (hipStream_t)stream>>>(f));
    TAO_LAUNCH_CHECK();
    return TAOAMD_OK;
}

static int accumulate_all(int64_t n_dt, int32_t n_cat, int32_t n_rng,
                          const int32_t *cat_off, const int32_t *order,
                          const uint64_t *matched, const uint64_t *ignored,
                          const int32_t *num_gt, int32_t max_segment,
                          double *precision, double *recall, void *workspace,
                          size_t workspace_bytes, void *stream, int phase = ACC_ALL,
                          int force_mode = SWEEP_AUTO)
{
    if (n_cat <= 0 || n_rng < 1 || n_rng > 32) return TAOAMD_ERR_ARG;
    if (!workspace) return TAOAMD_ERR_ARG;
    Carve c(workspace);
    double *val, *rec;
    acc_full_layout(c, n_dt, n_cat, n_rng, val, rec);
    if (!c.fits(workspace, workspace_bytes)) return TAOAMD_ERR_WORKSPACE;
    int st = accumulate_compact(n_dt, n_cat, n_rng, cat_off, order, matched, ignored,
                                num_gt, 0, n_cat, max_segment, val, rec, workspace,
                                workspace_bytes, stream, phase, force_mode);
    if (st != TAOAMD_OK || phase == ACC_PLAN) return st;
    return taoamd_finalize(n_cat, n_rng, num_gt, val, rec, precision, recall, stream);
}

extern "C" int taoamd_accumulate(int64_t n_dt, int32_t n_cat, int32_t n_rng,
                                 const int32_t *cat_off,
                                 const uint64_t *matched,
                                 const uint64_t *ignored, const int32_t *num_gt,
                                 int32_t max_segment, double *precision,
                                 double *recall, void *workspace,
                                 size_t workspace_bytes, void *stream)
{
    return accumulate_all(n_dt, n_cat, n_rng, cat_off, nullptr, matched, ignored,
                          num_gt, max_segment, precision, recall, workspace,
                          workspace_bytes, stream);
}

extern "C" int taoamd_accumulate_chunked(int64_t n_dt, int32_t n_cat, int32_t n_rng,
                                         const int32_t *cat_off,
                                         const uint64_t *matched,
                                         const uint64_t *ignored, const int32_t *num_gt,
                                         int32_t max_segment, double *precision,
                                         double *recall, void *workspace,
                                         size_t workspace_bytes, void *stream)
{
    return accumulate_all(n_dt, n_cat, n_rng, cat_off, nullptr, matched, ignored,
                          num_gt, max_segment, precision, recall, workspace,
                          workspace_bytes, stream, ACC_ALL, SWEEP_CHUNKED);
}

extern "C" int taoamd_accumulate_compact_chunked(int64_t n_dt, int32_t n_cat,
                                                 int32_t n_rng, const int32_t *cat_off,
                                                 const uint64_t *matched,
                                                 const uint64_t *ignored,
                                                 const int32_t *num_gt, int32_t k_begin,
                                                 int32_t k_end, int32_t max_segment,
                                                 double *val, double *rec,
                                                 void *workspace, size_t workspace_bytes,
                                                 void *stream)
{
    return accumulate_compact(n_dt, n_cat, n_rng, cat_off, nullptr, matched, ignored,
                              num_gt, k_begin, k_end, max_segment, val, rec,
                              workspace, workspace_bytes, stream, ACC_ALL, SWEEP_CHUNKED);
}

extern "C" int taoamd_accumulate_by_order(int64_t n_dt, int32_t n_cat, int32_t n_rng,
                                          const int32_t *cat_off,
                                          const int32_t *order,
                                          const uint64_t *matched,
                                          const uint64_t *ignored,
                                          const int32_t *num_gt, int32_t max_segment,
                                          double *precision, double *recall,
                                          void *workspace, size_t workspace_bytes,
                                          void *stream)
{
    if (!order) return TAOAMD_ERR_ARG;
    return accumulate_all(n_dt, n_cat, n_rng, cat_off, order, matched, ignored,
                          num_gt, max_segment, precision, recall, workspace,
                          workspace_bytes, stream);
}

extern "C" int taoamd_accumulate_by_order_prepared(int64_t n_dt, int32_t n_cat, int32_t n_rng,
                                                   const int32_t *cat_off,
                                                   const int32_t *order,
                                                   const uint64_t *matched,
                                                   const uint64_t *ignored,
                                                   const int32_t *num_gt, int32_t max_segment,
                                                   double *precision, double *recall,
                                                   void *workspace, size_t workspace_bytes,
                                                   void *stream)
{
    if (!order) return TAOAMD_ERR_ARG;
    return accumulate_all(n_dt, n_cat, n_rng, cat_off, order, matched, ignored,
                          num_gt, max_segment, precision, recall, workspace,
                          workspace_bytes, stream, ACC_SWEEP);
}

extern "C" int taoamd_accumulate_by_order_chunked(int64_t n_dt, int32_t n_cat, int32_t n_rng,
                                                  const int32_t *cat_off,
                                                  const int32_t *order,
                                                  const uint64_t *matched,
                                                  const uint64_t *ignored,
                                                  const int32_t *num_gt, int32_t max_segment,
                                                  double *precision, double *recall,
                                                  void *workspace, size_t workspace_bytes,
                                                  void *stream)
{
    if (!order) return TAOAMD_ERR_ARG;
    return accumulate_all(n_dt, n_cat, n_rng, cat_off, order, matched, ignored,
                          num_gt, max_segment, precision, recall, workspace,
                          workspace_bytes, stream, ACC_ALL, SWEEP_CHUNKED);
}

extern "C" int taoamd_accumulate_prepare(int64_t n_dt, int32_t n_cat, int32_t n_rng,
                                         const int32_t *cat_off, int32_t max_segment,
                                         void *workspace, size_t workspace_bytes,
                                         void *stream)
{
    return accumulate_all(n_dt, n_cat, n_rng, cat_off, nullptr, nullptr, nullptr,
                          nullptr, max_segment, nullptr, nullptr, workspace,
                          workspace_bytes, stream, ACC_PLAN);
}

extern "C" int taoamd_accumulate_prepared(int64_t n_dt, int32_t n_cat, int32_t n_rng,
                                          const int32_t *cat_off,
                                          const uint64_t *matched,
                                          const uint64_t *ignored,
                                          const int32_t *num_gt, int32_t max_segment,
                                          double *precision, double *recall,
                                          void *workspace, size_t workspace_bytes,
                                          void *stream)
{
    return accumulate_all(n_dt, n_cat, n_rng, cat_off, nullptr, matched, ignored,
                          num_gt, max_segment, precision, recall, workspace,
                          workspace_bytes, stream, ACC_SWEEP);
}
```

tao_amodal_amd/csrc/iou_match.hip:

```cpp
#include <cstdlib>

#include "common.hpp"

using namespace taoamd;

static IouThr match_thr()
{
    IouThr t = iou_thr();
    for (int q = 0; q < N_THR; q++) t.v[q] = t.v[q] < 1 - 1e-10 ? t.v[q] : 1 - 1e-10;
    return t;
}


__global__ void bb_iou_kernel(const double *__restrict__ dt,
                              const double *__restrict__ gt, size_t m,
                              size_t n, const unsigned char *__restrict__ crowd,
                              double *__restrict__ o)
{
    size_t total = m * n;
    for (size_t i = blockIdx.x * (size_t)blockDim.x + threadIdx.x; i < total;
         i += (size_t)gridDim.x * blockDim.x) {
        size_t g = i / m, d = i - g * m;
        const double4 D = reinterpret_cast<const double4 *>(dt)[d];
        const double4 G = reinterpret_cast<const double4 *>(gt)[g];
        double v;
        if (crowd != nullptr && crowd[g]) {
            double da = D.z * D.w;
            double w = raw_fmin(D.z + D.x, G.z + G.x) - raw_fmax(D.x, G.x);
            double h = raw_fmin(D.w + D.y, G.w + G.y) - raw_fmax(D.y, G.y);
            v = (w <= 0 || h <= 0) ? 0.0 : (w * h) / da;
        } else {
            v = box_iou(D.x, D.y, D.z, D.w, G.x, G.y, G.z, G.w);
        }
        o[i] = v;
    }
}

__global__ void lvis_ranges_kernel(int64_t n_gt, const double *__restrict__ vis,
                                   const uint8_t *__restrict__ gflags,
                                   const int32_t *__restrict__ gcat,
                                   int64_t n_dt,
                                   const uint8_t *__restrict__ dflags,
                                   uint32_t *__restrict__ gt_rng,
                                   uint32_t *__restrict__ dt_rng,
                                   int32_t *__restrict__ num_gt, RangeTab tab)
{
    const double *lo = tab.vis_lo, *hi = tab.vis_hi;
    int64_t i = blockIdx.x * (int64_t)blockDim.x + threadIdx.x;
    if (i < n_gt) {
        uint32_t m = 0;
        bool ign = gflags[i] & TAOAMD_GT_IGNORE;
        double v = vis[i];
#pragma unroll
        for (int r = 0; r < 5; r++)
            if (ign || v < lo[r] || v > hi[r]) m |= 1u << r;
        if (ign || !(gflags[i] & TAOAMD_GT_OOF)) m |= 1u << 5;
        gt_rng[i] = m;
        if (num_gt != nullptr) {
            int32_t *row = num_gt + (int64_t)gcat[i] * TAOAMD_LVIS_RNG;
#pragma unroll
            for (int r = 0; r < TAOAMD_LVIS_RNG; r++)
                if (!((m >> r) & 1u)) atomicAdd(row + r, 1);
        }
    }
    if (i < n_dt)
        dt_rng[i] = (dflags[i] & TAOAMD_DT_IGNORE_UNMATCHED) ? 0x3fu : 0u;
}

__global__ void tao_ranges_kernel(
    int64_t n_gt, const double *__restrict__ garea,
    const int32_t *__restrict__ glen, const int32_t *__restrict__ gnhp,
    const uint8_t *__restrict__ gflags, const int32_t *__restrict__ gcat,
    int64_t n_dt, const double *__restrict__ darea,
    const int32_t *__restrict__ dlen, const uint8_t *__restrict__ dflags,
    uint32_t *__restrict__ gt_rng, uint32_t *__restrict__ dt_rng,
    int32_t *__restrict__ num_gt, RangeTab tab)
{
    const double *alo = tab.area_lo, *ahi = tab.area_hi;
    const double *tlo = tab.time_lo, *thi = tab.time_hi;
    int64_t i = blockIdx.x * (int64_t)blockDim.x + threadIdx.x;
    if (i < n_gt) {
        uint32_t m = 0;
        bool ign = gflags[i] & TAOAMD_GT_IGNORE;
        double a_ = garea[i], len = (double)glen[i];
        bool few_hp = gnhp[i] <= 5;
#pragma unroll
        for (int a = 0; a < 5; a++)
#pragma unroll
            for (int t = 0; t < 4; t++) {
                bool bad = ign || a_ < alo[a] || a_ > ahi[a] || len < tlo[t] ||
                           len > thi[t] || (a == 4 && few_hp);
                if (bad) m |= 1u << (a * 4 + t);
            }
        gt_rng[i] = m;
        if (num_gt != nullptr) {
            int32_t *row = num_gt + (int64_t)gcat[i] * TAOAMD_TAO_RNG;
            for (int r = 0; r < TAOAMD_TAO_RNG; r++)
                if (!((m >> r) & 1u)) atomicAdd(row + r, 1);
        }
    }
    if (i < n_dt) {
        uint32_t m = 0;
        bool nel = dflags[i] & TAOAMD_DT_IGNORE_UNMATCHED;
        double a_ = darea[i], len = (double)dlen[i];
#pragma unroll
        for (int a = 0; a < 5; a++)
#pragma unroll
            for (int t = 0; t < 4; t++)
                if (nel || a_ < alo[a] || a_ > ahi[a] || len < tlo[t] ||
                    len > thi[t])
                    m |= 1u << (a * 4 + t);
        dt_rng[i] = m;
    }
}

__global__ __launch_bounds__(256) void count_gt_kernel(
    int32_t n_cat, int32_t n_rng, const int32_t *__restrict__ gt_cat_off,
    const uint32_t *__restrict__ gt_rng, int32_t *__restrict__ num_gt)
{
    __shared__ int32_t part[4][32];
    const int wave = __builtin_amdgcn_readfirstlane(threadIdx.x >> 6);
    const int32_t k = blockIdx.x;
    const int lane = lane_id();
    const int32_t b = gt_cat_off[k], e = gt_cat_off[k + 1];
    int32_t mine = 0;
    for (int32_t base = b + wave * WAVE; base < e; base += 4 * 4 * WAVE) {
        uint32_t m[4];
#pragma unroll
        for (int u = 0; u < 4; u++) {
            const int32_t i = base + u * 4 * WAVE + lane;
            m[u] = i < e ? gt_rng[i] : 0xffffffffu;
        }
#pragma unroll
        for (int u = 0; u < 4; u++)
            for (int r = 0; r < n_rng; r++) {
                const int c = __popcll(__ballot(!((m[u] >> r) & 1u)));
                if (lane == r) mine += c;
            }
    }
    if (lane < 32) part[wave][lane] = mine;
    __syncthreads();
    if (threadIdx.x < (unsigned)n_rng)
        num_gt[(int64_t)k * n_rng + threadIdx.x] =
            part[0][threadIdx.x] + part[1][threadIdx.x] + part[2][threadIdx.x] +
            part[3][threadIdx.x];
}

struct MatchArgs {
    int64_t n_cells;
    const int32_t *cell_dt_off;
    const int32_t *cell_gt_off;
    const int64_t *cell_iou_off;
    const double *dt_box;
    const double *gt_box;
    const double *iou;
    const uint32_t *gt_rng;
    const uint32_t *dt_rng;
    const uint8_t *gt_flags;
    const uint8_t *dt_flags;
    const int32_t *dst;
    uint64_t *matched;
    uint64_t *ignored;
    int32_t *match_gt;
    double *ious_out;
    int32_t n_rng;
    int32_t n_words;
    int64_t out_stride;
    int32_t paired;
    int32_t wide;
    const int32_t *dt_group;
    const uint32_t *dt_meta;
    const int32_t *groups;
    const int32_t *singles;
    int32_t n_groups, n_singles;
    int32_t xcd;
};

__device__ __forceinline__ void store_row(const MatchArgs &a, int64_t row, int word,
                                          uint64_t m, uint64_t i)
{
    if (a.wide) {
        ulonglong2 v;
        v.x = m;
        v.y = i;
        *reinterpret_cast<ulonglong2 *>(a.matched + row * a.out_stride + 2 * word) = v;
    } else if (a.paired) {
        a.matched[row * a.out_stride + 2 * word] = m;
        a.matched[row * a.out_stride + 2 * word + 1] = i;
    } else {
        a.matched[row * a.out_stride + word] = m;
        a.ignored[row * a.out_stride + word] = i;
    }
}

__device__ __forceinline__ uint32_t dt_rng_of(const MatchArgs &a, int64_t d, uint32_t flags)
{
    if (a.dt_rng != nullptr) return a.dt_rng[d];
    return (flags & TAOAMD_DT_IGNORE_UNMATCHED) ? 0xffffffffu >> (32 - a.n_rng) : 0u;
}

#define GRP_GCAP 8

template <bool FUSED>
__global__ __launch_bounds__(256) void match_kernel(MatchArgs a, IouThr thr)
{
    const int lane = lane_id();
    const int wave = __builtin_amdgcn_readfirstlane(threadIdx.x >> 6);
    const int64_t item = (int64_t)blockIdx.x * 4 + wave;
    const int64_t n_items = a.singles != nullptr ? a.n_singles : a.n_cells;
    if (item >= n_items * a.n_words) return;
    const int64_t ci = item / a.n_words;
    const int word = (int)(item - ci * a.n_words);
    const int64_t cell = a.singles != nullptr ? a.singles[ci] : ci;
    const int32_t d0 = __builtin_amdgcn_readfirstlane(a.cell_dt_off[cell]);
    const int32_t D = __builtin_amdgcn_readfirstlane(a.cell_dt_off[cell + 1]) - d0;
    const int32_t g0 = __builtin_amdgcn_readfirstlane(a.cell_gt_off[cell]);
    const int32_t G = __builtin_amdgcn_readfirstlane(a.cell_gt_off[cell + 1]) - g0;
    if (D == 0 || G > WAVE) return;
    const int n_combo = a.n_rng * N_THR;
    const int combo = word * WAVE + lane;
    const bool active = combo < n_combo;
    const int r = active ? combo / N_THR : 0;
    const int t = active ? combo - r * N_THR : 0;
    const double thr0 = thr.v[t];
    const int64_t ioff = (FUSED && a.ious_out == nullptr && a.iou == nullptr)
                             ? 0 : a.cell_iou_off[cell];

    uint64_t IG = 0, HID = 0;
    for (int g = 0; g < G; g++) {
        uint32_t m = a.gt_rng[g0 + g];
        IG |= (uint64_t)((m >> r) & 1u) << g;
        HID |= (uint64_t)((a.gt_flags[g0 + g] & TAOAMD_GT_ID_HIDDEN) ? 1 : 0) << g;
    }
    const int TD = G > 0 ? WAVE / G : WAVE;
    double gx = 0, gy = 0, gw = 0, gh = 0;
    const int my_dd = G > 0 ? lane / G : 0;
    const int my_g = G > 0 ? lane - my_dd * G : 0;
    if (FUSED && G > 0 && my_dd < TD) {
        const double4 B = reinterpret_cast<const double4 *>(a.gt_box)[g0 + my_g];
        gx = B.x; gy = B.y; gw = B.z; gh = B.w;
    }

    uint64_t taken = 0;
    for (int32_t base = 0; base < D; base += TD) {
        const int nd = min(TD, D - base);
        double v_tile = 0.0;
        if (G > 0 && my_dd < nd) {
            if (FUSED) {
                const double4 B =
                    reinterpret_cast<const double4 *>(a.dt_box)[d0 + base + my_dd];
                v_tile = box_iou(B.x, B.y, B.z, B.w, gx, gy, gw, gh);
                if (a.ious_out != nullptr && word == 0)
                    a.ious_out[ioff + (int64_t)(base + my_dd) * G + my_g] = v_tile;
            } else {
                v_tile = a.iou[ioff + (int64_t)(base + my_dd) * G + my_g];
            }
        }
        int32_t t_flags = 0, t_rng = 0;
        int64_t t_row = 0;
        if (lane < nd) {
            const int32_t d = d0 + base + lane;
            t_flags = a.dt_flags[d];
            t_rng = (int32_t)dt_rng_of(a, d, (uint32_t)t_flags);
            t_row = a.dst != nullptr ? a.dst[d] : d;
        }
        uint64_t my_m = 0, my_i = 0;
        for (int dd = 0; dd < nd; dd++) {
            const int32_t d = d0 + base + dd;
            double best1 = thr0, best2 = thr0;
            int m1 = -1, m2 = -1;
            const uint64_t free1 = ~taken & ~IG, free2 = ~taken & IG;
            for (int g = 0; g < G; g++) {
                const double v = readlane_f64(v_tile, dd * G + g);
                const bool ok1 = ((free1 >> g) & 1) && !(v < best1);
                const bool ok2 = ((free2 >> g) & 1) && !(v < best2);
                best1 = ok1 ? v : best1;  m1 = ok1 ? g : m1;
                best2 = ok2 ? v : best2;  m2 = ok2 ? g : m2;
            }
            const int m = m1 >= 0 ? m1 : m2;
            const uint32_t df = (uint32_t)__builtin_amdgcn_readlane(t_flags, dd);
            const uint32_t drng = (uint32_t)__builtin_amdgcn_readlane(t_rng, dd);
            if (m >= 0 && !(df & TAOAMD_DT_NO_CONSUME)) taken |= 1ull << m;
            const bool vis = m >= 0 && !((HID >> m) & 1);
            bool ig = m >= 0 && ((IG >> m) & 1);
            if (!vis && ((drng >> r) & 1u)) ig = true;
            const uint64_t mw = __ballot(active && vis);
            const uint64_t iw = __ballot(active && ig);
            if (lane == dd) { my_m = mw; my_i = iw; }
            if (a.match_gt != nullptr && active)
                a.match_gt[(int64_t)d * n_combo + combo] = m;
        }
        if (lane < nd) {
            store_row(a, t_row, word, my_m, my_i);
        }
    }
}

template <bool FUSED, bool FAST = false, bool SCATTER = true>
__global__ __launch_bounds__(256) __attribute__((amdgpu_waves_per_eu(8, 8))) void match_group_kernel(MatchArgs a, IouThr thr)
{
    __shared__ double4 s_gt[4][WAVE];
    __shared__ double s_iou[4][FUSED ? 1 : WAVE * GRP_GCAP];
    const int lane = lane_id();
    const int wave = __builtin_amdgcn_readfirstlane(threadIdx.x >> 6);
    const uint32_t blk = a.xcd ? xcd_block(blockIdx.x, gridDim.x) : blockIdx.x;
    const int64_t item = (int64_t)blk * 4 + wave;
    if (item >= (int64_t)a.n_groups * a.n_words) return;
    const int64_t grp = a.n_words == 1 ? item : a.n_words == 4 ? item >> 2 : item / a.n_words;
    const int word = (int)(item - grp * a.n_words);
    const int4 run = reinterpret_cast<const int4 *>(a.groups)[grp];
    const int32_t d0 = __builtin_amdgcn_readfirstlane(run.x);
    const int32_t nD = __builtin_amdgcn_readfirstlane(run.y);
    const int32_t g0 = __builtin_amdgcn_readfirstlane(run.z);
    const int32_t nG = __builtin_amdgcn_readfirstlane(run.w);
    if (nD == 0) return;
    const int n_combo = a.n_rng * N_THR;

    int32_t t_flags = 0, t_rng = 0, gb = 0, dloc = 0, Gc = 0;
    int64_t t_row = 0, t_ioff = 0;
    double4 B = make_double4(0, 0, 0, 0);
    uint32_t grng = 0xffffffffu;
    bool ghid = false;
    if (FAST) {
        const int32_t d = d0 + min(lane, nD - 1);
        const int32_t g = g0 + min(lane, max(nG, 1) - 1);
        const uint32_t mt = a.dt_meta[d];
#ifdef TAOAMD_ABLATE_SCATTER
        const int32_t row = SCATTER ? d + (a.dst[d] & 0) : d;
#else
        const int32_t row = SCATTER ? a.dst[d] : d;
#endif
        const double4 box = reinterpret_cast<const double4 *>(a.dt_box)[d];
        uint32_t gr = 0xffffffffu;
        uint8_t gf = 0;
        double4 gbx = make_double4(0, 0, 0, 0);
        if (nG > 0) {
            gr = a.gt_rng[g];
            gf = a.gt_flags[g];
            gbx = reinterpret_cast<const double4 *>(a.gt_box)[g];
        }
        if (lane < nD) {
            t_flags = (int32_t)(mt & 0xffu);
            gb = (int32_t)((mt >> 8) & 63u);
            Gc = (int32_t)((mt >> 14) & 15u);
            dloc = (int32_t)(mt >> 18);
            t_rng = (int32_t)((t_flags & TAOAMD_DT_IGNORE_UNMATCHED)
                                  ? 0xffffffffu >> (32 - a.n_rng) : 0u);
            t_row = row;
            B = box;
        }
        if (lane < nG) {
            grng = gr;
            ghid = gf & TAOAMD_GT_ID_HIDDEN;
            s_gt[wave][lane] = gbx;
        }
    } else if (lane < nD) {
        const int32_t d = d0 + lane;
        if (FUSED && a.dt_meta != nullptr) {
            static_assert(GRP_GCAP <= 15 && WAVE <= 64, "fields of dt_meta");
            const uint32_t mt = a.dt_meta[d];
            t_flags = (int32_t)(mt & 0xffu);
            gb = (int32_t)((mt >> 8) & 63u);
            Gc = (int32_t)((mt >> 14) & 15u);
            dloc = (int32_t)(mt >> 18);
        } else {
            const int4 dg = reinterpret_cast<const int4 *>(a.dt_group)[d];
            t_flags = a.dt_flags[d];
            Gc = dg.y;
            gb = dg.x - g0;
            dloc = dg.z;
            if (a.cell_iou_off != nullptr) t_ioff = a.cell_iou_off[dg.w];
        }
        t_rng = (int32_t)dt_rng_of(a, d, (uint32_t)t_flags);
        t_row = a.dst != nullptr ? a.dst[d] : d;
        if (FUSED) B = reinterpret_cast<const double4 *>(a.dt_box)[d];
    }
    if (!FAST && lane < nG) {
        grng = a.gt_rng[g0 + lane];
        ghid = a.gt_flags[g0 + lane] & TAOAMD_GT_ID_HIDDEN;
        if (FUSED) s_gt[wave][lane] = reinterpret_cast<const double4 *>(a.gt_box)[g0 + lane];
    }
    const uint64_t HID = __ballot(ghid);
    __builtin_amdgcn_fence(__ATOMIC_ACQ_REL, "workgroup");
    __builtin_amdgcn_wave_barrier();
    const double tmin = thr.v[0];
    int cand = -1, ncand = 0;
    double vc = 0.0;
    double vmem[FUSED ? 1 : GRP_GCAP];
    if (!FUSED) {
        const int64_t base = t_ioff + (int64_t)dloc * Gc;
#pragma unroll
        for (int k = 0; k < GRP_GCAP; k++)
            vmem[k] = a.iou[lane < nD && k < Gc ? base + k : 0];
    }
#pragma unroll
    for (int k = 0; k < GRP_GCAP; k++) {
        const bool has = lane < nD && k < Gc;
        if (__ballot(has) == 0) break;
        if (has) {
            double v;
            if (FUSED) {
                const double4 A = s_gt[wave][gb + k];
                v = box_iou(B.x, B.y, B.z, B.w, A.x, A.y, A.z, A.w);
                if (!FAST && a.ious_out != nullptr && word == 0)
                    a.ious_out[t_ioff + (int64_t)dloc * Gc + k] = v;
            } else {
                v = vmem[k];
                s_iou[wave][lane * GRP_GCAP + k] = v;
            }
            if (!(v < tmin)) { ncand += v != v ? 2 : 1; cand = k; vc = v; }
        }
    }
    if (!FUSED) {
        __builtin_amdgcn_fence(__ATOMIC_ACQ_REL, "workgroup");
        __builtin_amdgcn_wave_barrier();
    }
    uint64_t my_m = 0, my_i = 0;
    const uint64_t starts = __ballot(lane < nD && dloc == 0);
    const int ca = lane - dloc;
    const uint64_t above = lane >= 63 ? 0ull : starts & ~((2ull << lane) - 1);
    const int ce = above ? __builtin_ctzll(above) : nD;
    const uint64_t below_ca = (1ull << ca) - 1;
    const uint64_t cell_all = (ce >= 64 ? ~0ull : ((1ull << ce) - 1)) & ~below_ca;
    const uint64_t multi = __ballot(lane < nD && ncand >= 2);
    const bool simple = lane < nD && (multi & cell_all) == 0;
    {
        uint32_t mygrng = 0;
        bool myghid = false;
        const uint32_t grng_c = (uint32_t)__shfl((int)grng, (gb + max(cand, 0)) & 63);
        if (simple && cand >= 0) {
            mygrng = grng_c;
            myghid = (HID >> (gb + cand)) & 1ull;
        }
        const bool consumes = !(t_flags & TAOAMD_DT_NO_CONSUME);
        int qpass = 0;
        if (simple && cand >= 0) {
#pragma unroll
            for (int q = 0; q < N_THR; q++) qpass += !(vc < thr.v[q]) ? 1 : 0;
        }
        const int val = consumes ? qpass : 0;
        int M = 0;
        const uint32_t cell_no = (uint32_t)__popcll(starts & (lane >= 63 ? ~0ull : ((2ull << lane) - 1)));
        for (int c = 0; c < GRP_GCAP; c++) {
            if (__ballot(simple && cand >= c) == 0) break;
            static_assert(N_THR < 16, "value bits of the keyed scan");
            uint32_t x = (lane < nD ? cell_no << 4 : 0u) | (uint32_t)(cand == c ? val : 0);
#define TAOAMD_SCAN_STEP(CTRL, ROWS)                                                         \
            x = max(x, (uint32_t)__builtin_amdgcn_update_dpp(0, (int)x, CTRL, ROWS, 0xF, false))
            TAOAMD_SCAN_STEP(0x111, 0xF);
            TAOAMD_SCAN_STEP(0x112, 0xF);
            TAOAMD_SCAN_STEP(0x114, 0xF);
            TAOAMD_SCAN_STEP(0x118, 0xF);
            TAOAMD_SCAN_STEP(0x142, 0xA);
            TAOAMD_SCAN_STEP(0x143, 0xC);
#undef TAOAMD_SCAN_STEP
            const uint32_t prev = (uint32_t)__builtin_amdgcn_update_dpp(0, (int)x, 0x138, 0xF, 0xF, true);
            if (cand == c) M = (prev >> 4) == cell_no ? (int)(prev & 15u) : 0;
        }
        const uint32_t m10 = qpass > M ? ((1u << qpass) - 1) & ~((1u << M) - 1) : 0u;
        if (FAST) {
            static_assert(N_THR == 10, "bit layout of the fast word");
            constexpr uint64_t S_ALL = 1ull | 1ull << 10 | 1ull << 20 | 1ull << 30 |
                                       1ull << 40 | 1ull << 50;
            constexpr uint64_t C9 = 1ull | 1ull << 9 | 1ull << 18 | 1ull << 27 |
                                    1ull << 36 | 1ull << 45;
            const uint32_t all10 = (1u << N_THR) - 1;
            const uint32_t rmask = 0xffffffffu >> (32 - a.n_rng);
            const uint64_t sall = ((uint64_t)rmask * C9) & S_ALL;
            const uint64_t sg = ((uint64_t)(mygrng & rmask) * C9) & S_ALL;
            const uint64_t sd = ((uint64_t)((uint32_t)t_rng & rmask) * C9) & S_ALL;
            const uint32_t X = myghid ? all10 : (~m10 & all10);
            if (simple) {
                my_m = myghid ? 0ull : (uint64_t)m10 * sall;
                my_i = (uint64_t)m10 * sg | (uint64_t)X * sd;
            }
        } else if (simple) {
            const uint32_t all10 = (1u << N_THR) - 1;
            const int r_lo = (word * WAVE) / N_THR;
            const int r_hi = min(a.n_rng - 1, (word * WAVE + WAVE - 1) / N_THR);
            for (int q = r_lo; q <= r_hi; q++) {
                const bool igr = (mygrng >> q) & 1u, dig = ((uint32_t)t_rng >> q) & 1u;
                const uint64_t mb = myghid ? 0u : m10;
                const uint64_t ib = (igr ? m10 : 0u) |
                                    (dig ? (myghid ? all10 : (~m10 & all10)) : 0u);
                const int o = q * N_THR - word * WAVE;
                my_m |= o >= 0 ? mb << o : mb >> (-o);
                my_i |= o >= 0 ? ib << o : ib >> (-o);
            }
            if (a.match_gt != nullptr)
                for (int cc = 0; cc < WAVE && word * WAVE + cc < n_combo; cc++)
                    a.match_gt[(int64_t)(d0 + lane) * n_combo + word * WAVE + cc] =
                        ((m10 >> ((word * WAVE + cc) % N_THR)) & 1u) ? cand : -1;
        }
    }
    const uint64_t todo = __ballot(lane < nD && !simple);
    if (todo == 0) {
        if (lane < nD) store_row(a, t_row, word, my_m, my_i);
        return;
    }
    const int combo = word * WAVE + lane;
    const bool active = combo < n_combo;
    const int r = active ? combo / N_THR : 0;
    const int t = active ? combo - r * N_THR : 0;
    const double thr0 = thr.v[t];
    uint64_t IG = 0;
    for (int q = 0; q < a.n_rng; q++) {
        const uint64_t m = __ballot(lane < nG && ((grng >> q) & 1u));
        IG = (q == r) ? m : IG;
    }
    const int32_t meta = (gb & 0xff) | ((Gc & 0xff) << 8) | ((t_flags & 0xff) << 16);
    uint64_t taken = 0;
    for (uint64_t rest = todo; rest != 0; rest &= rest - 1) {
        const int i = __builtin_ctzll(rest);
        const uint32_t mt = (uint32_t)__builtin_amdgcn_readlane(meta, i);
        const int gbi = mt & 0xff, gci = (mt >> 8) & 0xff;
        const uint32_t df = (mt >> 16) & 0xff;
        const uint32_t drng = (uint32_t)__builtin_amdgcn_readlane(t_rng, i);
        const uint32_t cellbits = (1u << gci) - 1;
        const uint32_t igl = (uint32_t)(IG >> gbi) & cellbits;
        const uint32_t freel = ~(uint32_t)(taken >> gbi) & cellbits;
        const uint32_t free1 = freel & ~igl, free2 = freel & igl;
        double best1 = thr0, best2 = thr0;
        int m1 = -1, m2 = -1;
        const double *__restrict__ row = &s_iou[wave][FUSED ? 0 : i * GRP_GCAP];
        double bx = 0, by = 0, bw = 0, bh = 0;
        if (FUSED) {
            bx = readlane_f64(B.x, i); by = readlane_f64(B.y, i);
            bw = readlane_f64(B.z, i); bh = readlane_f64(B.w, i);
        }
        for (int g = 0; g < gci; g++) {
            double v;
            if (FUSED) {
                const double4 A = s_gt[wave][gbi + g];
                v = box_iou(bx, by, bw, bh, A.x, A.y, A.z, A.w);
            } else {
                v = row[g];
            }
            const bool ok1 = ((free1 >> g) & 1u) && !(v < best1);
            const bool ok2 = ((free2 >> g) & 1u) && !(v < best2);
            best1 = ok1 ? v : best1;  m1 = ok1 ? g : m1;
            best2 = ok2 ? v : best2;  m2 = ok2 ? g : m2;
        }
        const int m = m1 >= 0 ? m1 : m2;
        if (m >= 0 && !(df & TAOAMD_DT_NO_CONSUME)) taken |= 1ull << (gbi + m);
        const bool vis = m >= 0 && !((HID >> (gbi + (m >= 0 ? m : 0))) & 1);
        bool ig = m >= 0 && ((igl >> (m >= 0 ? m : 0)) & 1u);
        if (!vis && ((drng >> r) & 1u)) ig = true;
        const uint64_t mw = __ballot(active && vis);
        const uint64_t iw = __ballot(active && ig);
        if (lane == i) { my_m = mw; my_i = iw; }
        if (a.match_gt != nullptr && active)
            a.match_gt[(int64_t)(d0 + i) * n_combo + combo] = m;
    }
    if (lane < nD) {
        store_row(a, t_row, word, my_m, my_i);
    }
}

template <bool FUSED>
__global__ __launch_bounds__(64) void match_big_kernel(MatchArgs a, IouThr thr,
                                                       int32_t g_cap)
{
    extern __shared__ __attribute__((aligned(16))) unsigned char smem[];
    double *row = reinterpret_cast<double *>(smem);
    uint32_t *takenw = reinterpret_cast<uint32_t *>(smem + (size_t)g_cap * 8);
    const int lane = lane_id();
    const int64_t item = blockIdx.x;
    const int64_t ci = item / a.n_words;
    const int word = (int)(item - ci * a.n_words);
    const int64_t cell = a.singles != nullptr ? a.singles[ci] : ci;
    const int32_t d0 = a.cell_dt_off[cell], D = a.cell_dt_off[cell + 1] - d0;
    const int32_t g0 = a.cell_gt_off[cell], G = a.cell_gt_off[cell + 1] - g0;
    if (D == 0 || G <= WAVE) return;
    const int n_combo = a.n_rng * N_THR;
    const int combo = word * WAVE + lane;
    const bool active = combo < n_combo;
    const int r = active ? combo / N_THR : 0;
    const int t = active ? combo - r * N_THR : 0;
    const double thr0 = thr.v[t];
    const int64_t ioff = a.cell_iou_off != nullptr ? a.cell_iou_off[cell] : 0;
    const int n_tw = (G + 31) / 32;
    for (int w = 0; w < n_tw; w++) takenw[w * WAVE + lane] = 0;
    for (int32_t dd = 0; dd < D; dd++) {
        const int32_t d = d0 + dd;
        __syncthreads();
        if (FUSED) {
            const double4 B = reinterpret_cast<const double4 *>(a.dt_box)[d];
            for (int g = lane; g < G; g += WAVE) {
                const double4 A = reinterpret_cast<const double4 *>(a.gt_box)[g0 + g];
                const double v = box_iou(B.x, B.y, B.z, B.w, A.x, A.y, A.z, A.w);
                row[g] = v;
                if (a.ious_out != nullptr && word == 0)
                    a.ious_out[ioff + (int64_t)dd * G + g] = v;
            }
        } else {
            for (int g = lane; g < G; g += WAVE)
                row[g] = a.iou[ioff + (int64_t)dd * G + g];
        }
        __syncthreads();
        double best1 = thr0, best2 = thr0;
        int m1 = -1, m2 = -1;
        uint32_t tw = 0;
        for (int g = 0; g < G; g++) {
            if ((g & 31) == 0) tw = takenw[(g >> 5) * WAVE + lane];
            const double v = row[g];
            const bool ign = (a.gt_rng[g0 + g] >> r) & 1u;
            const bool fr = !((tw >> (g & 31)) & 1u);
            const bool ok1 = fr && !ign && !(v < best1);
            const bool ok2 = fr && ign && !(v < best2);
            best1 = ok1 ? v : best1;  m1 = ok1 ? g : m1;
            best2 = ok2 ? v : best2;  m2 = ok2 ? g : m2;
        }
        const int m = m1 >= 0 ? m1 : m2;
        const uint8_t df = a.dt_flags[d];
        if (m >= 0 && !(df & TAOAMD_DT_NO_CONSUME))
            takenw[(m >> 5) * WAVE + lane] |= 1u << (m & 31);
        const bool vis = m >= 0 && !(a.gt_flags[g0 + max(m, 0)] & TAOAMD_GT_ID_HIDDEN);
        bool ig = m >= 0 && ((a.gt_rng[g0 + max(m, 0)] >> r) & 1u);
        if (!vis && ((dt_rng_of(a, d, df) >> r) & 1u)) ig = true;
        const uint64_t mw = __ballot(active && vis);
        const uint64_t iw = __ballot(active && ig);
        if (lane == 0) {
            const int64_t rowi = a.dst != nullptr ? a.dst[d] : d;
            store_row(a, rowi, word, mw, iw);
        }
        if (a.match_gt != nullptr && active)
            a.match_gt[(int64_t)d * n_combo + combo] = m;
    }
}

extern "C" int taoamd_bb_iou(const double *dt, const double *gt, size_t m,
                             size_t n, const unsigned char *iscrowd, double *o,
                             void *stream)
{
    if (m == 0 || n == 0) return TAOAMD_OK;
    if (!dt || !gt || !o) return TAOAMD_ERR_ARG;
    size_t total = m * n;
    unsigned blocks = (unsigned)((total + 255) / 256 < 4096 ? (total + 255) / 256 : 4096);
    TAO_TIMED("bb_iou_kernel", (hipStream_t)stream, bb_iou_kernel<<<blocks, 256, 0, (hipStream_t)stream>>>(dt, gt, m, n, iscrowd, o));
    TAO_LAUNCH_CHECK();
    return TAOAMD_OK;
}

extern "C" int taoamd_bb_iou_host(const double *dt, const double *gt, size_t m,
                                  size_t n, const unsigned char *iscrowd,
                                  double *o)
{
    if (m == 0 || n == 0) return TAOAMD_OK;
    if (!dt || !gt || !o) return TAOAMD_ERR_ARG;
    double *d_dt = nullptr, *d_gt = nullptr, *d_o = nullptr;
    unsigned char *d_c = nullptr;
    TAO_HIP(hipMalloc(&d_dt, m * 32));
    TAO_HIP(hipMalloc(&d_gt, n * 32));
    TAO_HIP(hipMalloc(&d_o, m * n * 8));
    TAO_HIP(hipMemcpy(d_dt, dt, m * 32, hipMemcpyHostToDevice));
    TAO_HIP(hipMemcpy(d_gt, gt, n * 32, hipMemcpyHostToDevice));
    if (iscrowd) {
        TAO_HIP(hipMalloc(&d_c, n));
        TAO_HIP(hipMemcpy(d_c, iscrowd, n, hipMemcpyHostToDevice));
    }
    int st = taoamd_bb_iou(d_dt, d_gt, m, n, d_c, d_o, nullptr);
    if (st == TAOAMD_OK) {
        TAO_HIP(hipMemcpy(o, d_o, m * n * 8, hipMemcpyDeviceToHost));
    }
    (void)hipFree(d_dt); (void)hipFree(d_gt); (void)hipFree(d_o);
    if (d_c) (void)hipFree(d_c);
    return st;
}

extern "C" int taoamd_lvis_ranges(int64_t n_gt, const double *gt_vis,
                                  const uint8_t *gt_flags,
                                  const int32_t *gt_cat,
                                  const int32_t *gt_cat_off, int64_t n_dt,
                                  const uint8_t *dt_flags, int32_t n_cat,
                                  uint32_t *gt_rng, uint32_t *dt_rng,
                                  int32_t *num_gt, void *stream)
{
    hipStream_t s = (hipStream_t)stream;
    const bool grouped = gt_cat_off != nullptr;
    if (!grouped)
        TAO_HIP(hipMemsetAsync(num_gt, 0, sizeof(int32_t) * (size_t)n_cat * TAOAMD_LVIS_RNG, s));
    if (dt_rng == nullptr) n_dt = 0;
    int64_t n = n_gt > n_dt ? n_gt : n_dt;
    if (n > 0) {
        TAO_TIMED("lvis_ranges_kernel", s, lvis_ranges_kernel<<<(unsigned)((n + 255) / 256), 256, 0, s>>>(
            n_gt, gt_vis, gt_flags, gt_cat, n_dt, dt_flags, gt_rng, dt_rng,
            grouped ? nullptr : num_gt, range_tab()));
    }
    if (grouped)
        TAO_TIMED("count_gt_kernel", s, count_gt_kernel<<<(unsigned)n_cat, 256, 0, s>>>(
            n_cat, TAOAMD_LVIS_RNG, gt_cat_off, gt_rng, num_gt));
    TAO_LAUNCH_CHECK();
    return TAOAMD_OK;
}

extern "C" int taoamd_tao_ranges(int64_t n_gt, const double *gt_area,
                                 const int32_t *gt_len, const int32_t *gt_nhp,
                                 const uint8_t *gt_flags, const int32_t *gt_cat,
                                 const int32_t *gt_cat_off, int64_t n_dt,
                                 const double *dt_area, const int32_t *dt_len,
                                 const uint8_t *dt_flags, int32_t n_cat,
                                 uint32_t *gt_rng, uint32_t *dt_rng,
                                 int32_t *num_gt, void *stream)
{
    hipStream_t s = (hipStream_t)stream;
    const bool grouped = gt_cat_off != nullptr;
    if (!grouped)
        TAO_HIP(hipMemsetAsync(num_gt, 0, sizeof(int32_t) * (size_t)n_cat * TAOAMD_TAO_RNG, s));
    int64_t n = n_gt > n_dt ? n_gt : n_dt;
    if (n > 0) {
        TAO_TIMED("tao_ranges_kernel", s, tao_ranges_kernel<<<(unsigned)((n + 255) / 256), 256, 0, s>>>(
            n_gt, gt_area, gt_len, gt_nhp, gt_flags, gt_cat, n_dt, dt_area,
            dt_len, dt_flags, gt_rng, dt_rng, grouped ? nullptr : num_gt, range_tab()));
    }
    if (grouped)
        TAO_TIMED("count_gt_kernel", s, count_gt_kernel<<<(unsigned)n_cat, 256, 0, s>>>(
            n_cat, TAOAMD_TAO_RNG, gt_cat_off, gt_rng, num_gt));
    TAO_LAUNCH_CHECK();
    return TAOAMD_OK;
}

extern "C" int taoamd_match_plan_host(int64_t n_cells, const int32_t *cell_dt_off,
                                      const int32_t *cell_gt_off, int32_t cap_d,
                                      int32_t cap_g, int32_t cap_cell_g,
                                      int64_t *sizes, int32_t *groups,
                                      int32_t *singles)
{
    if (n_cells < 0 || !cell_dt_off || !cell_gt_off || !sizes) return TAOAMD_ERR_ARG;
    if ((groups == nullptr) != (singles == nullptr)) return TAOAMD_ERR_ARG;
    int64_t ng = 0, ns = 0, c = 0;
    auto small = [&](int64_t k) {
        return cell_dt_off[k + 1] - cell_dt_off[k] <= cap_d &&
               cell_gt_off[k + 1] - cell_gt_off[k] <= cap_cell_g;
    };
    while (c < n_cells) {
        if (!small(c)) {
            if (cell_dt_off[c + 1] > cell_dt_off[c]) {
                if (singles) singles[ns] = (int32_t)c;
                ns++;
            }
            c++;
            continue;
        }
        int64_t e = c + 1;
        while (e < n_cells && small(e) &&
               cell_dt_off[e + 1] - cell_dt_off[c] <= cap_d &&
               cell_gt_off[e + 1] - cell_gt_off[c] <= cap_g)
            e++;
        if (cell_dt_off[e] > cell_dt_off[c]) {
            if (groups) {
                groups[2 * ng] = (int32_t)c;
                groups[2 * ng + 1] = (int32_t)e;
            }
            ng++;
        }
        c = e;
    }
    sizes[0] = ng;
    sizes[1] = ns;
    return TAOAMD_OK;
}

extern "C" int taoamd_match(int64_t n_cells, const int32_t *cell_dt_off,
                            const int32_t *cell_gt_off,
                            const int64_t *cell_iou_off,
                            int32_t max_gt_per_cell, const double *dt_box,
                            const double *gt_box, const double *iou,
                            int32_t n_rng, const uint32_t *gt_rng,
                            const uint32_t *dt_rng, const uint8_t *gt_flags,
                            const uint8_t *dt_flags, const int32_t *dst,
                            int64_t out_stride, uint64_t *matched,
                            uint64_t *ignored, int32_t *match_gt,
                            double *ious_out, const int32_t *dt_group,
                            const uint32_t *dt_meta,
                            const int32_t *groups, int32_t n_groups,
                            const int32_t *singles, int32_t n_singles,
                            void *stream)
{
    if (n_cells == 0) return TAOAMD_OK;
    if (n_rng < 1 || n_rng > 32) return TAOAMD_ERR_ARG;
    const bool fused = dt_box != nullptr;
    if (fused ? (gt_box == nullptr) : (iou == nullptr)) return TAOAMD_ERR_ARG;
    if (max_gt_per_cell > TAOAMD_MAX_GT_PER_CELL) return TAOAMD_ERR_TOO_LARGE;
    if ((!fused || ious_out) && cell_iou_off == nullptr) return TAOAMD_ERR_ARG;
    const bool planned = groups != nullptr;
    if (planned && (dt_group == nullptr || (n_singles > 0 && singles == nullptr)))
        return TAOAMD_ERR_ARG;
    MatchArgs a;
    a.n_cells = n_cells; a.cell_dt_off = cell_dt_off; a.cell_gt_off = cell_gt_off;
    a.cell_iou_off = cell_iou_off; a.dt_box = dt_box; a.gt_box = gt_box;
    a.iou = iou; a.gt_rng = gt_rng; a.dt_rng = dt_rng; a.gt_flags = gt_flags;
    a.dt_flags = dt_flags; a.dst = dst; a.matched = matched; a.ignored = ignored;
    a.match_gt = match_gt; a.ious_out = ious_out; a.n_rng = n_rng;
    a.n_words = (n_rng * N_THR + 63) / 64;
    a.paired = matched != nullptr && ignored == matched + 1;
    a.out_stride = out_stride > 0 ? out_stride : (a.paired ? 2 : 1) * a.n_words;
    if (a.out_stride < (a.paired ? 2 : 1) * a.n_words) return TAOAMD_ERR_ARG;
    a.wide = a.paired && (((uintptr_t)matched) & 15) == 0 && (a.out_stride & 1) == 0;
    a.dt_meta = fused && ious_out == nullptr ? dt_meta : nullptr;
    a.dt_group = dt_group; a.groups = groups; a.n_groups = planned ? n_groups : 0;
    a.singles = planned ? singles : nullptr; a.n_singles = planned ? n_singles : 0;
    static const int xcd_env = getenv("TAOAMD_XCD") ? atoi(getenv("TAOAMD_XCD")) : 1;
    a.xcd = xcd_env;
    hipStream_t s = (hipStream_t)stream;
    if (planned && n_groups > 0) {
        const unsigned gb = (unsigned)(((int64_t)n_groups * a.n_words + 3) / 4);
        const bool fast = fused && a.dt_meta && !a.dt_rng && !a.ious_out && !a.match_gt &&
                          a.n_words == 1 && n_rng <= 6;
        if (fast && a.dst) TAO_TIMED("match_group_kernel", s, (match_group_kernel<true, true><<<gb, 256, 0, s>>>(a, match_thr())));
        else if (fast) TAO_TIMED("match_group_kernel", s, (match_group_kernel<true, true, false><<<gb, 256, 0, s>>>(a, match_thr())));
        else if (fused) TAO_TIMED("match_group_kernel", s, match_group_kernel<true><<<gb, 256, 0, s>>>(a, match_thr()));
        else TAO_TIMED("match_group_kernel", s, match_group_kernel<false><<<gb, 256, 0, s>>>(a, match_thr()));
    }
    const int64_t cells = planned ? n_singles : n_cells;
    const int64_t items = cells * a.n_words;
    if (items > 0) {
        const unsigned blocks = (unsigned)((items + 3) / 4);
        if (fused) TAO_TIMED("match_kernel", s, match_kernel<true><<<blocks, 256, 0, s>>>(a, match_thr()));
        else TAO_TIMED("match_kernel", s, match_kernel<false><<<blocks, 256, 0, s>>>(a, match_thr()));
        if (max_gt_per_cell > WAVE) {
            const int32_t cap = (max_gt_per_cell + 31) / 32 * 32;
            const size_t lds = (size_t)cap * 8 + (size_t)(cap / 32) * WAVE * 4;
            if (fused)
                TAO_TIMED("match_big_kernel", s, match_big_kernel<true><<<(unsigned)items, 64, lds, s>>>(a, match_thr(), cap));
            else
                TAO_TIMED("match_big_kernel", s, match_big_kernel<false><<<(unsigned)items, 64, lds, s>>>(a, match_thr(), cap));
        }
    }
    TAO_LAUNCH_CHECK();
    return TAOAMD_OK;
}

__global__ void gather_rows_kernel(int64_t n, int32_t n_words,
                                   const uint64_t *__restrict__ sm,
                                   const uint64_t *__restrict__ si,
                                   int64_t stride,
                                   const int32_t *__restrict__ order,
                                   uint64_t *__restrict__ dm,
                                   uint64_t *__restrict__ di)
{
    const int64_t total = n * n_words;
    for (int64_t i = blockIdx.x * (int64_t)blockDim.x + threadIdx.x; i < total;
         i += (int64_t)gridDim.x * blockDim.x) {
        const int64_t p = i / n_words;
        const int w = (int)(i - p * n_words);
        const int64_t src = (int64_t)order[p] * stride + w;
        dm[i] = sm[src];
        di[i] = si[src];
    }
}

extern "C" int taoamd_gather_rows(int64_t n, int32_t n_words,
                                  const uint64_t *src_matched,
                                  const uint64_t *src_ignored,
                                  int64_t src_stride, const int32_t *order,
                                  uint64_t *dst_matched, uint64_t *dst_ignored,
                                  void *stream)
{
    if (n == 0) return TAOAMD_OK;
    if (n_words < 1 || src_stride < n_words) return TAOAMD_ERR_ARG;
    if (dst_ignored == dst_matched + 1 && n * n_words > 1) return TAOAMD_ERR_ARG;
    const int64_t total = n * n_words;
    unsigned blocks = (unsigned)((total + 255) / 256 < 8192 ? (total + 255) / 256 : 8192);
    TAO_TIMED("gather_rows_kernel", (hipStream_t)stream, gather_rows_kernel<<<blocks, 256, 0, (hipStream_t)stream>>>(
        n, n_words, src_matched, src_ignored, src_stride, order, dst_matched,
        dst_ignored));
    TAO_LAUNCH_CHECK();
    return TAOAMD_OK;
}
```

tao_amodal_amd/engine.py:

```python
import os

import numpy as np
import torch

from . import _lib

N_THR, N_REC = _lib.N_THR, _lib.N_REC


def _ptr(t):
    return None if t is None else t.data_ptr()


def _stream():
    return torch.cuda.current_stream().cuda_stream


def _to_device(v, device):
    from .flatten import LazyRows
    if not isinstance(v, LazyRows):
        return torch.from_numpy(np.ascontiguousarray(v)).to(device)
    from .flatten_dev import device_copy
    src = device_copy(v.source, device)
    if len(v.index) == 0:
# ... 221 lines not shown
            rid = (torch.searchsorted(runs_t[:, 0].contiguous(), d, right=True) - 1
                   ).clamp_(min=0)
            self.t["dt_meta"] = (
                self.t["dt_flags"].to(torch.int32)
                | (((dg[:, 0] - runs_t[:, 2][rid]) & 63) << 8)
                | (dg[:, 1].clamp(max=15) << 14) | ((dg[:, 2] & 63) << 18)).contiguous()
        self.t["singles"] = torch.from_numpy(
            singles if len(singles) else np.zeros(1, np.int32)).to(self.device)
        self.t["cell_iou_off"] = torch.from_numpy(iou_off).to(self.device)
        self.t["cat_off"] = torch.from_numpy(cat_off).to(self.device)
        self.t["gt_cat_off"] = torch.from_numpy(gt_cat_off).to(self.device)
        self.t["tile_off"] = torch.from_numpy(tile_off).to(self.device)
        self.cat_off_host = cat_off
        self.ss_sizes, self.ss_merge = (0, 0, 0, 0), False
        if self.grouped and self.n_dt:
            tabs, self.ss_sizes, self.ss_merge = sort_plan(cat_off)
            for name, tab in zip(("ss_chunks", "ss_split", "ss_stile", "ss_bucket"), tabs):
                self.t[name] = torch.from_numpy(tab).to(self.device)

    def _plan_track_iou(self, flat):
        lib = _lib.load()
        self._drop_plan()
        if self.device.type != "cuda":
            return
        if self.mask_iou:
            return
        meta, sides, n_slots = track_meta(flat)
        n_frames = sum(int(getattr(flat, "dev", {})[k].numel())
                       if k in getattr(flat, "dev", {}) and not dict.__contains__(flat, k)
                       else len(flat[k]) for k in ("dt_frame_pos", "gt_frame_pos"))
        self.n_slots = n_slots
        if n_slots > 4 * n_frames + (1 << 20) or n_slots >= 2 ** 31 - 1:
            return
        self.single_frame = (len(meta) > 0 and n_frames == len(meta)
                             and bool((meta[:, 0] == meta[:, 1]).all())
                             and os.environ.get("TAOAMD_SINGLE_FRAME", "1") != "0")
        if self.single_frame:
            self.exact_terms = True
            return
        tasks, rows, pairs, out = track_iou_plan(flat, meta)
        self.n_tasks = len(tasks)
        if self.n_tasks == 0:
            return
        dev = self.device
        self.t["tasks"] = torch.from_numpy(tasks).to(dev)
        self.t["task_rows"] = torch.from_numpy(rows).to(dev)
        self.t["task_pairs"] = torch.from_numpy(pairs).to(dev)
        self.t["task_out"] = torch.from_numpy(out).to(dev)
        self.t["trk_meta"] = torch.from_numpy(
            np.ascontiguousarray(meta, dtype=np.int32)).to(dev)
        padded = torch.empty((n_slots, 4), dtype=torch.float64, device=dev)
        n_dt = int(self.t["dt_frame_off"].numel()) - 1
        inexact = torch.zeros(1, dtype=torch.int32, device=dev)
        with torch.cuda.device(dev):
            for side, row0 in (("dt", 0), ("gt", n_dt)):
                slot0, slots = sides[side]
                n_trk = int(self.t[side + "_frame_off"].numel()) - 1
                _lib.check(lib.taoamd_track_pad(
                    n_trk, int(self.t[side + "_frame_pos"].numel()),
                    _ptr(self.t[side + "_frame_off"]),
                    _ptr(self.t[side + "_frame_pos"]),
                    _ptr(self.t[side + "_frame_box"]),
                    self.t["trk_meta"].data_ptr() + 16 * row0, slot0, slots,
                    _ptr(padded), _ptr(inexact), _stream()),
                    "taoamd_track_pad")
            has = meta[:, 1] >= meta[:, 0]
            trk_pieces = np.where(has, (meta[:, 1] >> 3) - (meta[:, 0] >> 3) + 1, 0)
            task_pieces = np.add.reduceat(trk_pieces[rows].astype(np.int64),
                                          tasks[:, 0].astype(np.int64))
            base = 1 + np.cumsum(task_pieces) - task_pieces
            n_pieces = 1 + int(task_pieces.sum())
            if n_pieces >= 2 ** 31 - 1 or int(task_pieces.max()) * 256 >= 2 ** 32:
                self._drop_plan()
                return
            self.t["task_base"] = torch.from_numpy(base.astype(np.int32)).to(dev)
            self.t["frames"] = torch.empty(((n_pieces + 64) * 8, 4), dtype=torch.float64,
                                           device=dev)
            _lib.check(lib.taoamd_track_stream(
                self.n_tasks, _ptr(self.t["tasks"]), _ptr(self.t["task_rows"]),
                _ptr(self.t["trk_meta"]), _ptr(self.t["task_base"]), _ptr(padded),
                _ptr(self.t["frames"]), _stream()), "taoamd_track_stream")
            del padded
        longest = int((meta[:, 1] - meta[:, 0]).max()) + 1 if len(meta) else 0
        flags = int(inexact.item())
        self.exact_terms = not (flags & 1) and longest <= 4096
        if flags & 2:
            self._drop_plan()

    PLAN_TABLES = ("tasks", "task_rows", "task_pairs", "task_out", "frames",
                   "task_base", "trk_meta")

    def _drop_plan(self):
        for k in self.PLAN_TABLES:
            self.t[k] = None

    def guard_active(self):
        return (self.kind == "tao" and self.n_iou > 0 and self.iou_mode != 2
                and not self.mask_iou
                and not (self.exact_terms and self.iou_mode == 0)
                and not self.single_frame and self.device.type == "cuda")

    def _plan_guard(self, flat, guard):
        if not self.guard_active():
            return
        lens = [int(np.diff(np.asarray(flat[s + "_frame_off"])).max())
                if len(flat[s + "_frame_off"]) > 1 else 0 for s in ("dt", "gt")]
        self.max_frames = lens
        self.near_ulp = int(min(8 * (lens[0] + lens[1]) + 8, 2 ** 31 - 1))
        tl_id = np.ascontiguousarray(flat.tl_image_id, dtype=np.int64)
        ids_ok = len(tl_id) == 0 or (int(tl_id.min()) >= 0
                                     and int(tl_id.max()) < 2 ** 61 - 1)
        if guard == "device" and ids_ok:
            self.guard_on_device = True
            dev = self.device
            self.t["cell_unit"] = torch.from_numpy(
                np.ascontiguousarray(flat.cell_unit, dtype=np.int32)).to(dev)
            self.t["tl_vid_start"] = torch.from_numpy(
                np.ascontiguousarray(flat.tl_vid_start, dtype=np.int64)).to(dev)
            self.t["tl_image_id"] = torch.from_numpy(tl_id).to(dev)
        else:
            self.guard_flat = flat

    def input_bytes(self):
        return sum(v.numel() * v.element_size() for v in self.t.values()
                   if v is not None)


class Workspace:

    def __init__(self, dp, detail=False, dt_rng_table=False, keep_order=False):
        lib = _lib.load()
        dev = dp.device
        u8 = torch.uint8
        self.gather = not detail and gathers_rows(dp)

        def buf(nbytes):
            return torch.empty(max(int(nbytes), 256), dtype=u8, device=dev)
        self.gt_rng = torch.empty(max(dp.n_gt, 1), dtype=torch.int32, device=dev)
        self.dt_rng = None if dp.kind == "lvis" and not (detail or dt_rng_table) \
            else torch.empty(max(dp.n_dt, 1), dtype=torch.int32, device=dev)
        self.num_gt = torch.empty((dp.n_cat, dp.n_rng), dtype=torch.int32,
                                  device=dev)
        self.order_buf = torch.empty(max(dp.n_dt, 1), dtype=torch.int32, device=dev) \
            if (detail or keep_order or self.gather or SORT_ASIDE) else None
        self._n_dt = dp.n_dt
        self.dst = torch.empty(max(dp.n_dt, 1), dtype=torch.int32, device=dev)
        self.dst_identity = False
        self.cell_order = False
        self.sort_bytes = max(lib.taoamd_sort_workspace(dp.n_dt),
                              lib.taoamd_sort_segments_workspace(dp.n_dt),
                              lib.taoamd_sort_sampled_workspace(
                                  dp.n_dt, dp.ss_sizes[3], int(dp.ss_merge)))
        self.sort_ws = buf(self.sort_bytes)
        self.rows = torch.empty((max(dp.n_dt, 1), dp.n_words, 2),
                                dtype=torch.int64, device=dev)
        self.matched, self.ignored = self.rows[..., 0], self.rows[..., 1]
        self.acc_bytes = lib.taoamd_accumulate_workspace(dp.n_dt, dp.n_cat,
                                                         dp.n_rng)
        self.acc_ws = buf(self.acc_bytes)
        self.acc_prepared = None
        self.sweep_recovered = 0
        if torch.device(dev).type == "cuda":
            prepare_sweep(dp, self)
        self.precision = torch.empty((N_THR, N_REC, dp.n_cat, dp.n_rng),
                                     dtype=torch.float64, device=dev)
        self.recall = torch.empty((N_THR, dp.n_cat, dp.n_rng),
                                  dtype=torch.float64, device=dev)
        self.iou = None
        self.pair_frames = None
        if dp.kind == "tao":
            self.iou = torch.empty(max(dp.n_iou, 1), dtype=torch.float64,
                                   device=dev)
            self.pair_frames = torch.zeros(1, dtype=torch.int64, device=dev)
            self.near_count = torch.zeros(1, dtype=torch.int32, device=dev)
            self.guarded_pairs = 0
            self.near_cap = int(min(max(dp.n_iou, 1), 2 ** 31 - 1)) \
                if dp.guard_active() else 1
            self.near_list = torch.empty(self.near_cap, dtype=torch.int64, device=dev)
            if dp.guard_on_device:
                self.guard_table = int(lib.taoamd_track_iou_setorder_table(
                    *dp.max_frames))
                workers = GUARD_SCRATCH_BYTES // (12 * self.guard_table)
                workers = int(min(max(workers // 64 * 64, 64), 4096))
                self.guard_slots = workers * 3 * self.guard_table
                self.guard_scratch = torch.empty(self.guard_slots, dtype=torch.int32,
                                                 device=dev)
                self.guard_status = torch.zeros(1, dtype=torch.int32, device=dev)
        elif dp.mask_iou:
            self.iou = torch.empty(max(dp.n_iou, 1), dtype=torch.float64,
                                   device=dev)
        if dp.mask_iou:
            ws_bytes = lib.taoamd_rle_iou_workspace if dp.kind == "lvis" else \
                lib.taoamd_track_mask_iou_workspace
            self.rle_bytes = ws_bytes(dp.rle_rows["dt"], dp.rle_total["dt"],
                                      dp.rle_rows["gt"], dp.rle_total["gt"])
            self.rle_ws = buf(self.rle_bytes)
        self.match_gt = None
        self.ious_out = None
        if detail:
            self.match_gt = torch.empty((max(dp.n_dt, 1), dp.n_rng * N_THR),
                                        dtype=torch.int32, device=dev)
            if dp.kind == "lvis":
                self.ious_out = torch.empty(max(dp.n_iou, 1),
                                            dtype=torch.float64, device=dev)


def _order_of(ws):
    if ws.order_buf is not None:
        return ws.order_buf
    n = ws._n_dt
    out = torch.empty(max(n, 1), dtype=torch.int32, device=ws.dst.device)
    if n:
        out[ws.dst[:n].long()] = torch.arange(n, dtype=torch.int32, device=ws.dst.device)
    return out


Workspace.order = property(_order_of)


def stage_ranges(dp, ws):
    lib, t, s = _lib.load(), dp.t, _stream()
    if dp.kind == "lvis":
        _lib.check(lib.taoamd_lvis_ranges(
            dp.n_gt, _ptr(t["gt_vis"]), _ptr(t["gt_flags"]), _ptr(t["gt_cat"]),
            _ptr(t["gt_cat_off"]) if dp.grouped else None,
            dp.n_dt, _ptr(t["dt_flags"]), dp.n_cat, _ptr(ws.gt_rng),
            _ptr(ws.dt_rng), _ptr(ws.num_gt), s), "taoamd_lvis_ranges")
    else:
        _lib.check(lib.taoamd_tao_ranges(
            dp.n_gt, _ptr(t["gt_area"]), _ptr(t["gt_len"]), _ptr(t["gt_nhp"]),
            _ptr(t["gt_flags"]), _ptr(t["gt_cat"]),
            _ptr(t["gt_cat_off"]) if dp.grouped else None, dp.n_dt,
            _ptr(t["dt_area"]), _ptr(t["dt_len"]), _ptr(t["dt_flags"]),
            dp.n_cat, _ptr(ws.gt_rng), _ptr(ws.dt_rng), _ptr(ws.num_gt), s),
            "taoamd_tao_ranges")


import os as _os0
SORT_SAMPLED_MIN = 1_500_000
_SORT_FORCE = _os0.environ.get("TAOAMD_SORT", "")


def sort_is_sampled(dp):
    if _SORT_FORCE in ("sampled", "segments"):
        return _SORT_FORCE == "sampled"
    return dp.n_dt >= SORT_SAMPLED_MIN


_ASIDE_ENV = _os0.environ.get("TAOAMD_SORT_ASIDE", "")
SORT_ASIDE = None if _ASIDE_ENV == "" else _ASIDE_ENV != "0"


def gathers_rows(dp):
    if SORT_ASIDE is not None:
        return False
    return (dp.kind == "lvis" and not dp.mask_iou and dp.grouped and dp.n_dt > 0
            and dp.device.type == "cuda" and sort_is_sampled(dp)
            and _plan_key(dp)[1] in (2, 3))


def stage_sort(dp, ws, order_only=False):
    lib, t, s = _lib.load(), dp.t, _stream()
    if not order_only:
        ws.dst_identity = False
    if dp.grouped and dp.n_dt and sort_is_sampled(dp):
        nc, ns, nt, nb = dp.ss_sizes
        _lib.check(lib.taoamd_sort_sampled(
            dp.n_dt, dp.n_cat, _ptr(t["cat_off"]), _ptr(t["tile_off"]), dp.n_tiles,
            dp.max_segment, _ptr(t["dt_score"]), nc, _ptr(t["ss_chunks"]), ns,
            _ptr(t["ss_split"]), nt, _ptr(t["ss_stile"]), nb, _ptr(t["ss_bucket"]),
            _ptr(ws.order_buf), None if order_only else _ptr(ws.dst), _ptr(ws.sort_ws),
            ws.sort_bytes, s),
            "taoamd_sort_sampled")
        return
    if dp.grouped:
        _lib.check(lib.taoamd_sort_segments(
            dp.n_dt, dp.n_cat, _ptr(t["cat_off"]), _ptr(t["tile_off"]),
            dp.n_tiles, dp.max_segment, _ptr(t["dt_cat"]), _ptr(t["dt_score"]),
            _ptr(ws.order_buf), _ptr(ws.dst), _ptr(ws.sort_ws), ws.sort_bytes, s),
            "taoamd_sort_segments")
        return
    _lib.check(lib.taoamd_sort_by_cat_score(
        dp.n_dt, _ptr(t["dt_cat"]), _ptr(t["dt_score"]), _ptr(ws.order_buf),
        _ptr(ws.dst), _ptr(ws.sort_ws), ws.sort_bytes, s),
        "taoamd_sort_by_cat_score")


def stage_mask_iou(dp, ws):
    if not dp.mask_iou or dp.n_iou == 0:
        return
    lib, t, s = _lib.load(), dp.t, _stream()
    _lib.check(lib.taoamd_rle_iou(
        dp.n_cells, _ptr(t["cell_dt_off"]), _ptr(t["cell_gt_off"]),
        _ptr(t["cell_iou_off"]), dp.n_dt, dp.rle_total["dt"],
        _ptr(t["dt_rle_off"]), _ptr(t["dt_rle_runs"]), _ptr(t["dt_rle_hw"]),
        _ptr(t["dt_rle_bb"]), dp.n_gt, dp.rle_total["gt"],
        _ptr(t["gt_rle_off"]), _ptr(t["gt_rle_runs"]), _ptr(t["gt_rle_hw"]),
        _ptr(t["gt_rle_bb"]), _ptr(ws.iou), _ptr(ws.rle_ws), ws.rle_bytes, s),
        "taoamd_rle_iou")


def stage_track_mask_iou(dp, ws):
    lib, t, s = _lib.load(), dp.t, _stream()
    _lib.check(lib.taoamd_track_mask_iou(
        dp.n_cells, _ptr(t["cell_dt_off"]), _ptr(t["cell_gt_off"]),
        _ptr(t["cell_iou_off"]), dp.n_iou, _ptr(t["dt_frame_off"]),
        _ptr(t["dt_frame_pos"]), dp.rle_rows["dt"], dp.rle_total["dt"],
        _ptr(t["dt_rle_off"]), _ptr(t["dt_rle_runs"]), _ptr(t["dt_rle_hw"]),
        _ptr(t["gt_frame_off"]), _ptr(t["gt_frame_pos"]), dp.rle_rows["gt"],
        dp.rle_total["gt"], _ptr(t["gt_rle_off"]), _ptr(t["gt_rle_runs"]),
        _ptr(t["gt_rle_hw"]), dp.iou_mode, _ptr(ws.iou), _ptr(ws.pair_frames), _ptr(ws.rle_ws),
        ws.rle_bytes, s), "taoamd_track_mask_iou")


def stage_track_iou(dp, ws):
    if dp.kind == "lvis":
        return stage_mask_iou(dp, ws)
    if dp.kind != "tao" or dp.n_iou == 0:
        return
    if dp.mask_iou:
        return stage_track_mask_iou(dp, ws)
    lib, t, s = _lib.load(), dp.t, _stream()
    if dp.single_frame:
        _lib.check(lib.taoamd_track_iou_single(
            dp.n_dt, _ptr(t["dt_group"]), _ptr(t["cell_iou_off"]),
            _ptr(t["dt_frame_pos"]), _ptr(t["dt_frame_box"]), _ptr(t["gt_frame_pos"]),
            _ptr(t["gt_frame_box"]), dp.iou_mode, _ptr(ws.iou), _ptr(ws.pair_frames), s),
            "taoamd_track_iou_single")
        return
    if t["tasks"] is not None:
        counted = getattr(ws, "pairs_counted", False) and dp.iou_mode == 0
        _lib.check(lib.taoamd_track_iou_planned(
            dp.n_tasks, _ptr(t["tasks"]), _ptr(t["task_rows"]),
            _ptr(t["task_pairs"]), _ptr(t["task_out"]), _ptr(t["frames"]),
            _ptr(t["task_base"]), _ptr(t["trk_meta"]), dp.iou_mode, _ptr(ws.iou),
            None if counted else _ptr(ws.pair_frames), s), "taoamd_track_iou_planned")
        ws.pairs_counted = True
        return
    _lib.check(lib.taoamd_track_iou(
        dp.n_cells, _ptr(t["cell_dt_off"]), _ptr(t["cell_gt_off"]),
        _ptr(t["cell_iou_off"]), dp.n_iou, _ptr(t["dt_frame_off"]),
        _ptr(t["dt_frame_pos"]), _ptr(t["dt_frame_box"]),
        _ptr(t["gt_frame_off"]), _ptr(t["gt_frame_pos"]),
        _ptr(t["gt_frame_box"]), dp.iou_mode, _ptr(ws.iou),
        _ptr(ws.pair_frames), s), "taoamd_track_iou")


GUARD_SCRATCH_BYTES = 64 << 20


def stage_iou_guard(dp, ws):
    if not dp.guard_active():
        return
    lib, t, s = _lib.load(), dp.t, _stream()
    _lib.check(lib.taoamd_track_iou_near(
        dp.n_cells, _ptr(t["cell_gt_off"]), _ptr(t["cell_iou_off"]), dp.n_iou,
        _ptr(ws.iou), dp.near_ulp, ws.near_cap, _ptr(ws.near_count),
        _ptr(ws.near_list), s), "taoamd_track_iou_near")
    if not dp.guard_on_device:
        return
    _lib.check(lib.taoamd_track_iou_setorder(
        dp.n_cells, _ptr(t["cell_dt_off"]), _ptr(t["cell_gt_off"]),
        _ptr(t["cell_iou_off"]), _ptr(t["cell_unit"]), _ptr(t["tl_vid_start"]),
        _ptr(t["tl_image_id"]), _ptr(t["dt_frame_off"]), _ptr(t["dt_frame_pos"]),
        _ptr(t["dt_frame_box"]), _ptr(t["gt_frame_off"]), _ptr(t["gt_frame_pos"]),
        _ptr(t["gt_frame_box"]), dp.iou_mode, _ptr(ws.near_count), ws.near_cap,
        _ptr(ws.near_list), _ptr(ws.iou), _ptr(ws.guard_scratch), ws.guard_slots,
        ws.guard_table, _ptr(ws.guard_status), s), "taoamd_track_iou_setorder")


def apply_iou_guard(dp, ws, flat=None):
    if not dp.guard_active() or dp.guard_on_device:
        return 0
    flat = flat if flat is not None else dp.guard_flat
    n = int(ws.near_count.item())
    if n == 0:
        return 0
    pairs = ws.near_list[:n].cpu().numpy()
    vals = set_order_iou(flat, pairs, dp.iou_mode)
    ws.iou[torch.from_numpy(pairs).to(dp.device)] = torch.from_numpy(vals).to(dp.device)
    return n


def _plan_key(dp):
    return (dp.acc_hint, int(_lib.load().taoamd_accumulate_plan_kind(
        dp.n_dt, dp.n_rng, dp.acc_hint)))


def prepare_sweep(dp, ws):
    with torch.cuda.device(dp.device):
        _lib.check(_lib.load().taoamd_accumulate_prepare(
            dp.n_dt, dp.n_cat, dp.n_rng, _ptr(dp.t["cat_off"]), dp.acc_hint,
            _ptr(ws.acc_ws), ws.acc_bytes, _stream()), "taoamd_accumulate_prepare")
    ws.acc_prepared = _plan_key(dp)


def sweep_flag(acc_ws, device):
    import ctypes as C
    flag = C.c_int32(0)
    with torch.cuda.device(device):
        _lib.check(_lib.load().taoamd_accumulate_error(
            _ptr(acc_ws), _stream(), C.addressof(flag)), "taoamd_accumulate_error")
    return int(flag.value)


def sweep_ok(dp, ws):
    if dp.device.type != "cuda" or not sweep_flag(ws.acc_ws, dp.device):
        return False
    import logging
    logging.getLogger("tao_amodal_amd").warning(
        "the one-pass sweep's look-back between workgroups timed out (a busy or "
        "shared GPU?): this pass is swept again with the chunked kernels")
    lib, t = _lib.load(), dp.t
    with torch.cuda.device(dp.device):
        if ws.cell_order:
            _lib.check(lib.taoamd_accumulate_by_order_chunked(
                dp.n_dt, dp.n_cat, dp.n_rng, _ptr(t["cat_off"]), _ptr(ws.order),
                _ptr(ws.matched), _ptr(ws.ignored), _ptr(ws.num_gt), dp.acc_hint,
                _ptr(ws.precision), _ptr(ws.recall), _ptr(ws.acc_ws), ws.acc_bytes,
                _stream()), "taoamd_accumulate_by_order_chunked")
        else:
            _lib.check(lib.taoamd_accumulate_chunked(
                dp.n_dt, dp.n_cat, dp.n_rng, _ptr(t["cat_off"]), _ptr(ws.matched),
                _ptr(ws.ignored), _ptr(ws.num_gt), dp.acc_hint, _ptr(ws.precision),
                _ptr(ws.recall), _ptr(ws.acc_ws), ws.acc_bytes, _stream()),
                "taoamd_accumulate_chunked")
    prepare_sweep(dp, ws)
    torch.cuda.synchronize(dp.device)
    ws.sweep_recovered += 1
    return True


def guarded_pairs(dp, ws, check_sweep=True):
    if check_sweep:
        sweep_ok(dp, ws)
    if not dp.guard_active():
        return 0
    if dp.guard_on_device and int(ws.guard_status.item()):
        raise _lib.TaoAmdError("frame-order guard: a track pair outgrew the set "
                               "tables sized for the longest tracks")
    n = int(ws.near_count.item())
    if n > max(dp.n_iou // 8, 1024):
        import logging
        logging.getLogger("tao_amodal_amd").warning(
            "frame-order guard: %d of %d track pairs were recomputed in the "
            "reference's frame order (slow path)", n, dp.n_iou)
    return n


def _fmax(a, b):
    return b if (b > a or a != a) else a


def _fmin(a, b):
    return b if (b < a or a != a) else a


def _pos(w):
    return 0 if (0 > w or w != w) else w


def set_order_iou(flat, pairs, mode=0):
    ioff = np.asarray(flat.cell_iou_off)
    d_off, g_off = np.asarray(flat.cell_dt_off), np.asarray(flat.cell_gt_off)
    tl_id, tl_start = np.asarray(flat.tl_image_id), np.asarray(flat.tl_vid_start)
    unit = np.asarray(flat.cell_unit)
    fr = {}
    for side in ("dt", "gt"):
        fr[side] = (np.asarray(flat[side + "_frame_off"]),
                    np.asarray(flat[side + "_frame_pos"]),
                    np.asarray(flat[side + "_frame_box"]))
    cache = {}

    def track_map(side, t, v):
        key = (side, t)
        if key not in cache:
            off, pos, box = fr[side]
            a, b = int(off[t]), int(off[t + 1])
            ids = tl_id[tl_start[v] + pos[a:b]].tolist()
            cache[key] = dict(zip(ids, np.asarray(box[a:b]).tolist()))
        return cache[key]
    out = np.zeros(len(pairs))
    cells = np.searchsorted(ioff, pairs, "right") - 1
    for k, (p, c) in enumerate(zip(pairs.tolist(), cells.tolist())):
        G = int(g_off[c + 1] - g_off[c])
        local = p - int(ioff[c])
        v = int(unit[c])
        dmap = track_map("dt", int(d_off[c]) + local // G, v)
        gmap = track_map("gt", int(g_off[c]) + local % G, v)
        i = u = 0
        ious = []
        for im in set(gmap.keys()) | set(dmap.keys()):
            g, d = gmap.get(im), dmap.get(im)
            if d and g:
                w = _pos(_fmin(d[0] + d[2], g[0] + g[2]) - _fmax(d[0], g[0]))
                h = _pos(_fmin(d[1] + d[3], g[1] + g[3]) - _fmax(d[1], g[1]))
                i_ = w * h
                u_ = d[2] * d[3] + g[2] * g[3] - i_
                i += i_
                u += u_
                ious.append(i_ / u_ if u_ > 0 else 0)
            elif g:
                u += g[2] * g[3]
                ious.append(0)
            elif d:
                u += d[2] * d[3]
                ious.append(0)
        out[k] = (i / u if u > 0 else 0) if mode == 0 else float(np.mean(ious))
    return out


def stage_match(dp, ws, scatter=True, groups=None, singles=None, match_gt=None):
    if dp.n_dt == 0:
        return
    lib, t, s = _lib.load(), dp.t, _stream()
    g_ptr, n_g = _ptr(t["groups"]), dp.n_groups
    s_ptr, n_s = _ptr(t["singles"]), dp.n_singles
    if groups is not None:
        g_ptr, n_g = groups[0].data_ptr() + 16 * groups[1], groups[2]
        s_ptr, n_s = singles[0].data_ptr() + 4 * singles[1], singles[2]
        if n_g == 0 and n_s == 0:
            return
    fused = dp.kind == "lvis" and not dp.mask_iou
    if groups is None:
        ws.cell_order = not scatter
    _lib.check(lib.taoamd_match(
        dp.n_cells, _ptr(t["cell_dt_off"]), _ptr(t["cell_gt_off"]),
        _ptr(t["cell_iou_off"]), dp.max_g,
        _ptr(t["dt_box"]) if fused else None,
        _ptr(t["gt_box"]) if fused else None,
        None if fused else _ptr(ws.iou), dp.n_rng, _ptr(ws.gt_rng),
        None if dp.kind == "lvis" else _ptr(ws.dt_rng),
        _ptr(t["gt_flags"]), _ptr(t["dt_flags"]),
        _ptr(ws.dst) if scatter else None, 0, _ptr(ws.matched),
        _ptr(ws.ignored), _ptr(ws.match_gt if match_gt is None else match_gt),
        _ptr(ws.ious_out),
        _ptr(t["dt_group"]), _ptr(t["dt_meta"]), g_ptr, n_g,
        s_ptr, n_s, s), "taoamd_match")


def stage_accumulate_by_order(dp, ws):
    lib, t, s = _lib.load(), dp.t, _stream()
    fn = lib.taoamd_accumulate_by_order_prepared if ws.acc_prepared == _plan_key(dp) \
        else lib.taoamd_accumulate_by_order
    _lib.check(fn(
        dp.n_dt, dp.n_cat, dp.n_rng, _ptr(t["cat_off"]), _ptr(ws.order),
        _ptr(ws.matched), _ptr(ws.ignored), _ptr(ws.num_gt), dp.acc_hint,
        _ptr(ws.precision), _ptr(ws.recall), _ptr(ws.acc_ws), ws.acc_bytes, s),
        "taoamd_accumulate_by_order")


def stage_accumulate(dp, ws):
    lib, t, s = _lib.load(), dp.t, _stream()
    fn = lib.taoamd_accumulate_prepared if ws.acc_prepared == _plan_key(dp) \
        else lib.taoamd_accumulate
    _lib.check(fn(
        dp.n_dt, dp.n_cat, dp.n_rng, _ptr(t["cat_off"]), _ptr(ws.matched),
        _ptr(ws.ignored), _ptr(ws.num_gt), dp.acc_hint, _ptr(ws.precision),
        _ptr(ws.recall), _ptr(ws.acc_ws), ws.acc_bytes, s),
        "taoamd_accumulate")


def stage_scores(dp, ws):
    lib, t, s = _lib.load(), dp.t, _stream()
    if getattr(ws, "scores", None) is None:
        ws.score_bytes = lib.taoamd_score_at_recall_workspace(dp.n_dt, dp.n_cat, dp.n_rng)
        ws.score_ws = torch.empty(max(int(ws.score_bytes), 256), dtype=torch.uint8,
                                  device=dp.device)
        ws.scores = torch.empty((N_THR, N_REC, dp.n_cat, dp.n_rng), dtype=torch.float64,
                                device=dp.device)
    ws.score_order = ws.order
    order = _ptr(ws.score_order)
    _lib.check(lib.taoamd_score_at_recall(
        dp.n_dt, dp.n_cat, dp.n_rng, _ptr(t["cat_off"]), order if ws.cell_order else None,
        _ptr(ws.matched), _ptr(ws.ignored), _ptr(t["dt_score"]), order, _ptr(ws.num_gt),
        _ptr(ws.scores), _ptr(ws.score_ws), ws.score_bytes, s), "taoamd_score_at_recall")


def _rows_by_unit(unit, n_unit):
    off = torch.zeros(n_unit + 1, dtype=torch.int32, device=unit.device)
    if unit.numel() == 0:
        return off, torch.zeros(1, dtype=torch.int32, device=unit.device)
    off[1:] = torch.cumsum(torch.bincount(unit, minlength=n_unit), 0)
    return off, torch.argsort(unit, stable=True).to(torch.int32)


def error_match_gt(dp, ws):
    if getattr(ws, "err_match_gt", None) is None:
        ws.err_match_gt = torch.empty((max(dp.n_dt, 1), dp.n_rng * N_THR), dtype=torch.int32,
                                      device=dp.device)
    return ws.err_match_gt


def stage_error_types(dp, ws, slot, tb, per_detection=False):
    if dp.kind != "lvis" or dp.mask_iou:
        raise _lib.TaoAmdError("the error breakdown is the image level's, on boxes")
    if dp.cell_unit_host is None:
        raise _lib.TaoAmdError("the error breakdown needs the cells' images (flat.cell_unit)")
    lib, t, s = _lib.load(), dp.t, _stream()
    dev = dp.device
    if getattr(dp, "err_tabs", None) is None:
        cell_unit = torch.from_numpy(np.ascontiguousarray(dp.cell_unit_host, dtype=np.int64)
                                     ).to(dev)
        n_img = int(dp.cell_unit_host.max()) + 1 if dp.n_cells else 0
        cells = torch.arange(dp.n_cells, dtype=torch.int64, device=dev)
        gt_cell = torch.repeat_interleave(
            cells, (t["cell_gt_off"][1:] - t["cell_gt_off"][:-1]).long())
        dt_cell = t["dt_cell"][:dp.n_dt].long()
        dp.err_tabs = (n_img,) + _rows_by_unit(cell_unit[gt_cell], n_img) \
            + _rows_by_unit(cell_unit[dt_cell], n_img) \
            + (t["dt_group"][:, 0].contiguous(),)
    n_img, img_gt_off, img_gt, img_dt_off, img_dt, dt_gt0 = dp.err_tabs
    if getattr(ws, "err_dt_counts", None) is None:
        ws.err_bytes = lib.taoamd_error_types_workspace(dp.n_dt, dp.n_gt, dp.n_rng)
        ws.err_ws = torch.empty(max(int(ws.err_bytes), 256), dtype=torch.uint8, device=dev)
        ws.err_dt_counts = torch.empty((dp.n_rng, dp.n_cat, 7), dtype=torch.int64, device=dev)
        ws.err_gt_counts = torch.empty((dp.n_rng, dp.n_cat, 3), dtype=torch.int64, device=dev)
        ws.err_dt_type = None
    match_gt = ws.match_gt
    if match_gt is None:
        if getattr(ws, "err_match_gt", None) is None and dp.n_dt:
            stage_match(dp, ws, scatter=not ws.cell_order, match_gt=error_match_gt(dp, ws))
        match_gt = getattr(ws, "err_match_gt", None)
    if per_detection and ws.err_dt_type is None:
        ws.err_dt_type = torch.empty((max(dp.n_dt, 1), dp.n_rng), dtype=torch.uint8, device=dev)
    _lib.check(lib.taoamd_error_types(
        dp.n_dt, dp.n_gt, n_img, dp.n_cat, dp.n_rng, int(slot), float(tb),
        _ptr(t["dt_cat"]), _ptr(t["dt_box"]), _ptr(t["dt_flags"]), _ptr(dt_gt0),
        _ptr(match_gt), dp.n_rng * N_THR, _ptr(t["gt_cat"]), _ptr(t["gt_box"]),
        _ptr(ws.gt_rng), _ptr(img_gt_off), _ptr(img_gt), _ptr(img_dt_off), _ptr(img_dt),
        _ptr(ws.err_dt_counts), _ptr(ws.err_gt_counts),
        _ptr(ws.err_dt_type) if per_detection else None,
        _ptr(ws.err_ws), ws.err_bytes, s), "taoamd_error_types")


def stage_track_error_types(dp, ws, slot, tb, per_detection=False):
    if dp.kind != "tao" or dp.mask_iou:
        raise _lib.TaoAmdError("the track-level error breakdown is the track level's, on boxes")
    if dp.iou_mode != 0:
        raise _lib.TaoAmdError("the track-level error breakdown is defined for the 3d_iou metric")
    if dp.cell_unit_host is None:
        raise _lib.TaoAmdError("the error breakdown needs the cells' videos (flat.cell_unit)")
    lib, t, s = _lib.load(), dp.t, _stream()
    dev = dp.device
    if getattr(dp, "err_tabs", None) is None:
        cell_unit = torch.from_numpy(np.ascontiguousarray(dp.cell_unit_host, dtype=np.int64)
                                     ).to(dev)
        n_vid = int(dp.cell_unit_host.max()) + 1 if dp.n_cells else 0
        cells = torch.arange(dp.n_cells, dtype=torch.int64, device=dev)
        gt_cell = torch.repeat_interleave(
            cells, (t["cell_gt_off"][1:] - t["cell_gt_off"][:-1]).long())
        dt_cell = t["dt_cell"][:dp.n_dt].long()
        dp.err_tabs = (n_vid,) + _rows_by_unit(cell_unit[gt_cell], n_vid) \
            + _rows_by_unit(cell_unit[dt_cell], n_vid)
    n_vid, vid_gt_off, vid_gt, vid_dt_off, vid_dt = dp.err_tabs
    if getattr(ws, "err_dt_counts", None) is None:
        ws.err_bytes = lib.taoamd_track_error_types_workspace(dp.n_dt, dp.n_gt, dp.n_rng)
        ws.err_ws = torch.empty(max(int(ws.err_bytes), 256), dtype=torch.uint8, device=dev)
        ws.err_dt_counts = torch.empty((dp.n_rng, dp.n_cat, 7), dtype=torch.int64, device=dev)
        ws.err_gt_counts = torch.empty((dp.n_rng, dp.n_cat, 3), dtype=torch.int64, device=dev)
        ws.err_dt_type = None
    match_gt = ws.match_gt
    if match_gt is None:
        if getattr(ws, "err_match_gt", None) is None and dp.n_dt:
            stage_match(dp, ws, scatter=not ws.cell_order, match_gt=error_match_gt(dp, ws))
        match_gt = getattr(ws, "err_match_gt", None)
    if per_detection and ws.err_dt_type is None:
        ws.err_dt_type = torch.empty((max(dp.n_dt, 1), dp.n_rng), dtype=torch.uint8, device=dev)
    _lib.check(lib.taoamd_track_error_types(
        dp.n_dt, dp.n_gt, dp.n_cells, dp.n_iou, n_vid, dp.n_cat, dp.n_rng, int(slot), float(tb),
        _ptr(t["dt_cat"]), _ptr(ws.dt_rng), _ptr(t["dt_group"]), _ptr(t["cell_iou_off"]),
        _ptr(ws.iou), _ptr(match_gt), dp.n_rng * N_THR, _ptr(t["gt_cat"]), _ptr(ws.gt_rng),
        _ptr(t["dt_frame_off"]), _ptr(t["dt_frame_pos"]), _ptr(t["dt_frame_box"]),
        _ptr(t["gt_frame_off"]), _ptr(t["gt_frame_pos"]), _ptr(t["gt_frame_box"]),
        _ptr(vid_gt_off), _ptr(vid_gt), _ptr(vid_dt_off), _ptr(vid_dt),
        _ptr(ws.err_dt_counts), _ptr(ws.err_gt_counts),
        _ptr(ws.err_dt_type) if per_detection else None, None,
        _ptr(ws.err_ws), ws.err_bytes, s), "taoamd_track_error_types")


def stage_track_iou_guarded(dp, ws):
    stage_track_iou(dp, ws)
    stage_iou_guard(dp, ws)


STAGES = (("ranges", stage_ranges), ("sort", stage_sort),
          ("track_iou", stage_track_iou_guarded), ("match", stage_match),
          ("accumulate", stage_accumulate))


def run(dp, ws):
    if _lib.TIMING:
        _lib.kernel_timing_label(dp.kind)
    for name, fn in STAGES:
        fn(dp, ws)
        if name == "track_iou" and dp.guard_flat is not None:
# ... 220 lines not shown
```

Measured before the change: 41620.

## Emit compact 32-bit match words and decode them in the accumulate sweep

Adds a compact match path. The match kernel writes one 32-bit word per detection (match bits, gt range, flags), with an escape flag that falls back to full 16-byte rows. The sweep kernel decodes these words through a 256-entry shared table, and the full rows are expanded lazily only when other stages read them. This cuts global memory traffic between match and accumulate, at the cost of extra decode logic, a shared-memory table, and more complex lazy-state handling in Python.

```diff
diff --git a/include/tao_amodal_hip.h b/include/tao_amodal_hip.h
--- a/include/tao_amodal_hip.h
+++ b/include/tao_amodal_hip.h
@@ -160,6 +160,17 @@
                  const int32_t *dt_group, const uint32_t *dt_meta,
                  const int32_t *groups, int32_t n_groups, const int32_t *singles,
                  int32_t n_singles, void *stream);
+
+int taoamd_match_compact(int64_t n_cells, const int32_t *cell_dt_off,
+                         const int32_t *cell_gt_off, int32_t max_gt_per_cell,
+                         const double *dt_box, const double *gt_box, int32_t n_rng,
+                         const uint32_t *gt_rng, const uint8_t *gt_flags,
+                         const uint8_t *dt_flags, uint64_t *rows, uint32_t *compact,
+                         const int32_t *dt_group, const uint32_t *dt_meta,
+                         const int32_t *groups, int32_t n_groups, const int32_t *singles,
+                         int32_t n_singles, void *stream);
+int taoamd_expand_rows(int64_t n_dt, int32_t n_rng, const uint32_t *compact,
+                       uint64_t *rows, void *stream);
 
 int taoamd_flat_map(int64_t n, const int64_t *image_id, const int64_t *category_id,
                     const double *bbox, const double *area_in, int64_t n_img,
@@ -360,6 +371,12 @@
                                const int32_t *num_gt, int32_t max_segment,
                                double *precision, double *recall, void *workspace,
                                size_t workspace_bytes, void *stream);
+int taoamd_accumulate_by_order_compact(int64_t n_dt, int32_t n_cat, int32_t n_rng,
+                               const int32_t *cat_off, const int32_t *order,
+                               const uint32_t *compact, const uint64_t *rows,
+                               const int32_t *num_gt, int32_t max_segment,
+                               double *precision, double *recall, void *workspace,
+                               size_t workspace_bytes, int32_t prepared, void *stream);
 
 size_t taoamd_score_at_recall_workspace(int64_t n_dt, int32_t n_cat, int32_t n_rng);
 int taoamd_score_at_recall(int64_t n_dt, int32_t n_cat, int32_t n_rng,
diff --git a/tao_amodal_amd/_lib.py b/tao_amodal_amd/_lib.py
--- a/tao_amodal_amd/_lib.py
+++ b/tao_amodal_amd/_lib.py
@@ -116,6 +116,9 @@
     "taoamd_match": (C.c_int, [_i64, _vp, _vp, _vp, _i32, _vp, _vp, _vp, _i32,
                                _vp, _vp, _vp, _vp, _vp, _i64, _vp, _vp, _vp,
                                _vp, _vp, _vp, _vp, _i32, _vp, _i32, _vp]),
+    "taoamd_match_compact": (C.c_int, [_i64, _vp, _vp, _i32, _vp, _vp, _i32, _vp, _vp, _vp,
+                                       _vp, _vp, _vp, _vp, _vp, _i32, _vp, _i32, _vp]),
+    "taoamd_expand_rows": (C.c_int, [_i64, _i32, _vp, _vp, _vp]),
     "taoamd_gather_rows": (C.c_int, [_i64, _i32, _vp, _vp, _i64, _vp, _vp,
                                      _vp, _vp]),
     "taoamd_compact_elems": (_sz, [_i32, _i32]),
@@ -168,6 +171,9 @@
                                              _vp, _i32, _vp, _vp, _vp, _sz, _vp]),
     "taoamd_accumulate_by_order_chunked": (C.c_int, [_i64, _i32, _i32, _vp, _vp, _vp, _vp,
                                              _vp, _i32, _vp, _vp, _vp, _sz, _vp]),
+    "taoamd_accumulate_by_order_compact": (C.c_int, [_i64, _i32, _i32, _vp, _vp, _vp, _vp,
+                                                     _vp, _i32, _vp, _vp, _vp, _sz, _i32,
+                                                     _vp]),
     "taoamd_score_at_recall_workspace": (_sz, [_i64, _i32, _i32]),
     "taoamd_score_at_recall": (C.c_int, [_i64, _i32, _i32, _vp, _vp, _vp, _vp, _vp, _vp,
                                          _vp, _vp, _vp, _sz, _vp]),
diff --git a/tao_amodal_amd/csrc/accumulate.hip b/tao_amodal_amd/csrc/accumulate.hip
--- a/tao_amodal_amd/csrc/accumulate.hip
+++ b/tao_amodal_amd/csrc/accumulate.hip
@@ -24,6 +24,7 @@
     const uint64_t *matched;
     const uint64_t *ignored;
     const int32_t *order;
+    const uint32_t *compact;
     const int32_t *num_gt;
     int32_t *cat_chunk_off;
     const int32_t *chunk_tab;
@@ -189,12 +190,110 @@
                   tpw[blk], fpw[blk]);
 }
 
-template <int ACC_BLK_N, bool GATHER = false>
+#define CROW_ESCAPE 0x80000000u
+#define CROW_KEYS 256
+
+__device__ __forceinline__ uint64_t crow_all(int32_t n_rng)
+{
+    constexpr uint64_t S_ALL = 1ull | 1ull << 10 | 1ull << 20 | 1ull << 30 |
+                               1ull << 40 | 1ull << 50;
+    constexpr uint64_t C9 = 1ull | 1ull << 9 | 1ull << 18 | 1ull << 27 |
+                            1ull << 36 | 1ull << 45;
+    return ((((uint64_t)(0xffffffffu >> (32 - n_rng))) * C9) & S_ALL) * 0x3ffull;
+}
+
+__device__ __forceinline__ void crow_table(ulonglong2 *tab, int32_t n_rng)
+{
+    constexpr uint64_t S_ALL = 1ull | 1ull << 10 | 1ull << 20 | 1ull << 30 |
+                               1ull << 40 | 1ull << 50;
+    constexpr uint64_t C9 = 1ull | 1ull << 9 | 1ull << 18 | 1ull << 27 |
+                            1ull << 36 | 1ull << 45;
+    const uint32_t rmask = 0xffffffffu >> (32 - n_rng);
+    const uint64_t all = crow_all(n_rng);
+    for (int key = threadIdx.x; key < CROW_KEYS; key += blockDim.x) {
+        const uint32_t g = (uint32_t)key & 63u & rmask;
+        const bool u = (key >> 6) & 1, h = (key >> 7) & 1;
+        const uint64_t A = h && u ? all : (((uint64_t)g * C9) & S_ALL) * 0x3ffull;
+        ulonglong2 e;
+        e.x = (h ? 0ull : all) & ~A;
+        e.y = ~A;
+        tab[key] = e;
+    }
+}
+
+__device__ __forceinline__ void crow_expand(uint32_t w, const ulonglong2 *tab, uint32_t nall_lo,
+                                            uint32_t nall_hi, uint64_t &tpw, uint64_t &vw)
+{
+    const uint32_t m10 = w & 0x3ffu;
+    uint32_t lo = m10 | m10 << 10;
+    lo |= lo << 20;
+    const uint32_t hi = m10 >> 2 | m10 << 8 | m10 << 18;
+    const ulonglong2 e = tab[(w >> 10) & (CROW_KEYS - 1)];
+    const uint64_t T = e.x, nA = e.y;
+    const uint32_t nu = ~(uint32_t)((int32_t)(w << 15) >> 31);
+    const uint32_t t_lo = lo & (uint32_t)T, t_hi = hi & (uint32_t)(T >> 32);
+    const uint32_t v_lo = (lo & (uint32_t)nA) | (~lo & (nu | nall_lo));
+    const uint32_t v_hi = (hi & (uint32_t)(nA >> 32)) | (~hi & (nu | nall_hi));
+    tpw = (uint64_t)t_hi << 32 | t_lo;
+    vw = (uint64_t)v_hi << 32 | v_lo;
+}
+
+template <int ACC_BLK_N>
+__device__ __forceinline__ void load_chunk_compact(const AccArgs &a, int64_t start, int len,
+                                                   int lane, uint32_t (&w)[ACC_BLK_N],
+                                                   ulonglong2 *tab)
+{
+    const bool full = len == ACC_BLK_N * WAVE;
+    const int32_t *__restrict__ ob = a.order + start;
+    uint32_t at[ACC_BLK_N];
+    if (full) {
+#pragma unroll
+        for (int blk = 0; blk < ACC_BLK_N; blk++) at[blk] = (uint32_t)ob[blk * WAVE + lane];
+    } else {
+#pragma unroll
+        for (int blk = 0; blk < ACC_BLK_N; blk++) {
+            const int i = blk * WAVE + lane;
+            at[blk] = len > 0 ? (uint32_t)ob[i < len ? i : 0] : 0u;
+        }
+    }
+    crow_table(tab, a.n_rng);
+    __syncthreads();
+    if (full || len > 0) {
+#pragma unroll
+        for (int blk = 0; blk < ACC_BLK_N; blk++) w[blk] = a.compact[at[blk]];
+    } else {
+#pragma unroll
+        for (int blk = 0; blk < ACC_BLK_N; blk++) w[blk] = 0;
+    }
+}
+
+template <int ACC_BLK_N>
+__device__ __forceinline__ void crow_rows(const AccArgs &a, int64_t start, int len, int lane,
+                                          int blk, uint32_t w, const ulonglong2 *tab,
+                                          uint32_t nall_lo, uint32_t nall_hi,
+                                          uint64_t &tpw, uint64_t &vw)
+{
+    const bool full = len == ACC_BLK_N * WAVE;
+    crow_expand(w, tab, nall_lo, nall_hi, tpw, vw);
+    if (__ballot(w & CROW_ESCAPE) != 0) {
+        if (w & CROW_ESCAPE) {
+            const int i = blk * WAVE + lane;
+            const uint32_t r = (uint32_t)a.order[start + (full || i < len ? i : 0)];
+            const ulonglong2 v = *reinterpret_cast<const ulonglong2 *>(
+                reinterpret_cast<const char *>(a.matched) + (uint64_t)r * 16u);
+            tpw = v.x & ~v.y;
+            vw = ~v.y;
+        }
+    }
+    if (!full && blk * WAVE + lane >= len) { tpw = 0; vw = 0; }
+}
+
+template <int ACC_BLK_N, int GATHER = 0>
 __device__ __forceinline__ void load_chunk_tv(const AccArgs &a, int64_t start, int word, int len,
                                               int lane, uint64_t (&tpw)[ACC_BLK_N],
                                               uint64_t (&vw)[ACC_BLK_N])
 {
-    if (GATHER && a.wide && len == ACC_BLK_N * WAVE) {
+    if (GATHER == 1 && a.wide && len == ACC_BLK_N * WAVE) {
         const int32_t *__restrict__ ob = a.order + start;
         uint32_t at[ACC_BLK_N];
 #pragma unroll
@@ -839,7 +938,7 @@
     a.cj[i] = ng > 0 ? recall_crossing(rec.v[i - kr * N_REC], ng) : 0;
 }
 
-template <int SW, int MODE, bool GATHER = false, int NB = SWEEP_NB>
+template <int SW, int MODE, int GATHER = 0, int NB = SWEEP_NB>
 __global__ __launch_bounds__(SW * WAVE) __attribute__((amdgpu_waves_per_eu(8, 8)))
 void acc_sweep_kernel(AccArgs a, RecThr rec)
 {
@@ -849,6 +948,7 @@
     __shared__ int32_t s_cj[EMIT_RMAX][N_REC];
     __shared__ uint16_t s_jr[SW][WAVE];
     __shared__ int32_t s_done;
+    __shared__ ulonglong2 s_crow[GATHER == 2 ? CROW_KEYS : 1];
     const int lane = lane_id();
     const int wave = __builtin_amdgcn_readfirstlane(threadIdx.x >> 6);
     if (threadIdx.x == 0) s_done = 0;
@@ -868,7 +968,16 @@
     const int len = (int)max((int64_t)0, min((int64_t)(NB * WAVE), cat_end - start));
     const bool swept = k >= a.k_begin && k < a.k_end;
     uint64_t tpw[NB], vw[NB];
-    load_chunk_tv<NB, GATHER>(a, start, word, len, lane, tpw, vw);
+    uint32_t cw[NB];
+    uint32_t nall_lo = 0, nall_hi = 0;
+    if (GATHER == 2) {
+        load_chunk_compact<NB>(a, start, len, lane, cw, s_crow);
+        const uint64_t nall = ~crow_all(a.n_rng);
+        nall_lo = (uint32_t)nall;
+        nall_hi = (uint32_t)(nall >> 32);
+    } else {
+        load_chunk_tv<NB, GATHER>(a, start, word, len, lane, tpw, vw);
+    }
     const int r_lo = (word * WAVE) / N_THR;
     const int r_hi = min(a.n_rng - 1, (word * WAVE + WAVE - 1) / N_THR);
     if (MODE != 2) {
@@ -879,9 +988,13 @@
     uint64_t T[NB], TF[NB];
     uint32_t tp_own = 0, n_own = 0;
 #pragma unroll
-    for (int blk = 0; blk < NB; blk++) {
+    for (int b_ = 0; b_ < NB; b_++) {
+        const int blk = GATHER == 2 ? NB - 1 - b_ : b_;
         uint64_t t_ = 0, v_ = 0;
         if (blk * WAVE < len) {
+            if (GATHER == 2)
+                crow_rows<NB>(a, start, len, lane, blk, cw[blk], s_crow, nall_lo, nall_hi,
+                              tpw[blk], vw[blk]);
 #if defined(SW_ABLATE) && (SW_ABLATE & 2)
             t_ = tpw[blk];
             v_ = vw[blk];
@@ -1042,8 +1155,9 @@
         const uint64_t v = s_max[w][lane];
         if (pr_better((uint32_t)(v >> 32), (uint32_t)v, later)) later = v;
     }
-    a.sc_max[so] = live ? later : PR_ZERO;
-    a.sc_jhi[so] = (uint8_t)(live ? s_jr[SW - 1][lane] >> 8 : 0);
+    const int64_t so_end = GATHER == 2 ? (int64_t)sc * WAVE + lane : so;
+    a.sc_max[so_end] = live ? later : PR_ZERO;
+    a.sc_jhi[so_end] = (uint8_t)(live ? s_jr[SW - 1][lane] >> 8 : 0);
 }
 
 __device__ __forceinline__ uint64_t pr_max(uint64_t a, uint64_t b)
@@ -1289,7 +1403,8 @@
                               const int32_t *num_gt, int32_t k_begin, int32_t k_end,
                               int32_t max_segment, double *val, double *rec,
                               void *workspace, size_t workspace_bytes, void *stream,
-                              int phase = ACC_ALL, int force_mode = SWEEP_AUTO)
+                              int phase = ACC_ALL, int force_mode = SWEEP_AUTO,
+                              const uint32_t *compact = nullptr)
 {
     if (n_cat <= 0 || n_rng < 1 || n_rng > 32) return TAOAMD_ERR_ARG;
     if (k_begin < 0 || k_end > n_cat || k_begin > k_end) return TAOAMD_ERR_ARG;
@@ -1304,6 +1419,7 @@
     a.chunk_tab = nullptr;
     a.n_dt = n_dt; a.n_cat = n_cat; a.n_rng = n_rng;
     a.cat_off = cat_off; a.matched = matched; a.ignored = ignored; a.order = order;
+    a.compact = compact;
     a.paired = matched != nullptr && ignored == matched + 1;
     a.wide = a.paired && ((uintptr_t)matched & 15) == 0;
     a.num_gt = num_gt; a.val = (uint64_t *)val; a.rec = rec;
@@ -1325,6 +1441,7 @@
     a.fused_rows = 0;
     a.fused_lo = -1;
     if (all_fused && phase == ACC_PLAN) return TAOAMD_OK;
+    if (all_fused && compact != nullptr) return TAOAMD_ERR_ARG;
     if (all_fused) {
         const unsigned grid = (unsigned)(k_end - k_begin);
         int32_t lo = -1;
@@ -1349,6 +1466,8 @@
     a.inline_scans = max_segment > 0 && max_segment <= ACC_INLINE_CHUNKS * ACC_CH;
     const size_t nc = (size_t)a.n_chunks_max, nw = (size_t)a.n_words;
     const int mode = force_mode != SWEEP_AUTO ? force_mode : sweep_mode(n_dt);
+    if (compact != nullptr && (mode == SWEEP_CHUNKED || !order || !a.wide || a.n_words != 1 || n_rng > 6))
+        return TAOAMD_ERR_ARG;
     if (mode != SWEEP_CHUNKED) {
         a.sc_rows = SWEEP_SW * SWEEP_NB * WAVE;
         a.inline_scans = 0;
@@ -1381,13 +1500,18 @@
             uint32_t g = ++g_sc_gen;
             a.sc_gen = (g & 0x3fffffffu) ? (g & 0x3fffffffu) : (++g_sc_gen & 0x3fffffffu);
             a.sc_error = t.header;
-            if (a.order)
-                TAO_TIMED("acc_sweep_kernel", s, (acc_sweep_kernel<SWEEP_SW, 0, true><<<grid, SWEEP_SW * WAVE, 0, s>>>(a, rec_thr())));
+            if (a.compact)
+                TAO_TIMED("acc_sweep_kernel", s, (acc_sweep_kernel<SWEEP_SW, 0, 2><<<grid, SWEEP_SW * WAVE, 0, s>>>(a, rec_thr())));
+            else if (a.order)
+                TAO_TIMED("acc_sweep_kernel", s, (acc_sweep_kernel<SWEEP_SW, 0, 1><<<grid, SWEEP_SW * WAVE, 0, s>>>(a, rec_thr())));
             else
                 TAO_TIMED("acc_sweep_kernel", s, (acc_sweep_kernel<SWEEP_SW, 0><<<grid, SWEEP_SW * WAVE, 0, s>>>(a, rec_thr())));
+        } else if (a.compact) {
+            TAO_TIMED("acc_sccount_kernel", s, (acc_sweep_kernel<SWEEP_SW, 2, 2><<<grid, SWEEP_SW * WAVE, 0, s>>>(a, rec_thr())));
+            TAO_TIMED("acc_sweep_kernel", s, (acc_sweep_kernel<SWEEP_SW, 1, 2><<<grid, SWEEP_SW * WAVE, 0, s>>>(a, rec_thr())));
         } else if (a.order) {
-            TAO_TIMED("acc_sccount_kernel", s, (acc_sweep_kernel<SWEEP_SW, 2, true><<<grid, SWEEP_SW * WAVE, 0, s>>>(a, rec_thr())));
-            TAO_TIMED("acc_sweep_kernel", s, (acc_sweep_kernel<SWEEP_SW, 1, true><<<grid, SWEEP_SW * WAVE, 0, s>>>(a, rec_thr())));
+            TAO_TIMED("acc_sccount_kernel", s, (acc_sweep_kernel<SWEEP_SW, 2, 1><<<grid, SWEEP_SW * WAVE, 0, s>>>(a, rec_thr())));
+            TAO_TIMED("acc_sweep_kernel", s, (acc_sweep_kernel<SWEEP_SW, 1, 1><<<grid, SWEEP_SW * WAVE, 0, s>>>(a, rec_thr())));
         } else {
             TAO_TIMED("acc_sccount_kernel", s, (acc_sweep_kernel<SWEEP_SW, 2><<<grid, SWEEP_SW * WAVE, 0, s>>>(a, rec_thr())));
             TAO_TIMED("acc_sweep_kernel", s, (acc_sweep_kernel<SWEEP_SW, 1><<<grid, SWEEP_SW * WAVE, 0, s>>>(a, rec_thr())));
@@ -1463,7 +1587,7 @@
                           const int32_t *num_gt, int32_t max_segment,
                           double *precision, double *recall, void *workspace,
                           size_t workspace_bytes, void *stream, int phase = ACC_ALL,
-                          int force_mode = SWEEP_AUTO)
+                          int force_mode = SWEEP_AUTO, const uint32_t *compact = nullptr)
 {
     if (n_cat <= 0 || n_rng < 1 || n_rng > 32) return TAOAMD_ERR_ARG;
     if (!workspace) return TAOAMD_ERR_ARG;
@@ -1473,7 +1597,7 @@
     if (!c.fits(workspace, workspace_bytes)) return TAOAMD_ERR_WORKSPACE;
     int st = accumulate_compact(n_dt, n_cat, n_rng, cat_off, order, matched, ignored,
                                 num_gt, 0, n_cat, max_segment, val, rec, workspace,
-                                workspace_bytes, stream, phase, force_mode);
+                                workspace_bytes, stream, phase, force_mode, compact);
     if (st != TAOAMD_OK || phase == ACC_PLAN) return st;
     return taoamd_finalize(n_cat, n_rng, num_gt, val, rec, precision, recall, stream);
 }
@@ -1551,6 +1675,23 @@
                           workspace_bytes, stream, ACC_SWEEP);
 }
 
+extern "C" int taoamd_accumulate_by_order_compact(int64_t n_dt, int32_t n_cat, int32_t n_rng,
+                                                  const int32_t *cat_off,
+                                                  const int32_t *order,
+                                                  const uint32_t *compact,
+                                                  const uint64_t *rows,
+                                                  const int32_t *num_gt, int32_t max_segment,
+                                                  double *precision, double *recall,
+                                                  void *workspace, size_t workspace_bytes,
+                                                  int32_t prepared, void *stream)
+{
+    if (!order || !compact || !rows) return TAOAMD_ERR_ARG;
+    return accumulate_all(n_dt, n_cat, n_rng, cat_off, order, rows, rows + 1,
+                          num_gt, max_segment, precision, recall, workspace,
+                          workspace_bytes, stream, prepared ? ACC_SWEEP : ACC_ALL,
+                          SWEEP_AUTO, compact);
+}
+
 extern "C" int taoamd_accumulate_by_order_chunked(int64_t n_dt, int32_t n_cat, int32_t n_rng,
                                                   const int32_t *cat_off,
                                                   const int32_t *order,
diff --git a/tao_amodal_amd/csrc/iou_match.hip b/tao_amodal_amd/csrc/iou_match.hip
--- a/tao_amodal_amd/csrc/iou_match.hip
+++ b/tao_amodal_amd/csrc/iou_match.hip
@@ -174,7 +174,10 @@
     const int32_t *singles;
     int32_t n_groups, n_singles;
     int32_t xcd;
+    uint32_t *compact;
 };
+
+#define TAOAMD_ROW_ESCAPE 0x80000000u
 
 __device__ __forceinline__ void store_row(const MatchArgs &a, int64_t row, int word,
                                           uint64_t m, uint64_t i)
@@ -292,13 +295,15 @@
         }
         if (lane < nd) {
             store_row(a, t_row, word, my_m, my_i);
-        }
-    }
-}
-
-template <bool FUSED, bool FAST = false, bool SCATTER = true>
+            if (a.compact != nullptr) a.compact[t_row] = TAOAMD_ROW_ESCAPE;
+        }
+    }
+}
+
+template <bool FUSED, bool FAST = false, bool SCATTER = true, bool COMPACT = false>
 __global__ __launch_bounds__(256) __attribute__((amdgpu_waves_per_eu(8, 8))) void match_group_kernel(MatchArgs a, IouThr thr)
 {
+    static_assert(!COMPACT || (FAST && !SCATTER), "compact rows: the fast cell-order instance");
     __shared__ double4 s_gt[4][WAVE];
     __shared__ double s_iou[4][FUSED ? 1 : WAVE * GRP_GCAP];
     const int lane = lane_id();
@@ -416,6 +421,7 @@
         __builtin_amdgcn_wave_barrier();
     }
     uint64_t my_m = 0, my_i = 0;
+    uint32_t my_c = TAOAMD_ROW_ESCAPE;
     const uint64_t starts = __ballot(lane < nD && dloc == 0);
     const int ca = lane - dloc;
     const uint64_t above = lane >= 63 ? 0ull : starts & ~((2ull << lane) - 1);
@@ -470,7 +476,12 @@
             const uint64_t sg = ((uint64_t)(mygrng & rmask) * C9) & S_ALL;
             const uint64_t sd = ((uint64_t)((uint32_t)t_rng & rmask) * C9) & S_ALL;
             const uint32_t X = myghid ? all10 : (~m10 & all10);
-            if (simple) {
+            if (COMPACT) {
+                if (simple)
+                    my_c = m10 | (mygrng & rmask) << 10 |
+                           (((uint32_t)t_rng & rmask) ? 1u << 16 : 0u) |
+                           (myghid ? 1u << 17 : 0u);
+            } else if (simple) {
                 my_m = myghid ? 0ull : (uint64_t)m10 * sall;
                 my_i = (uint64_t)m10 * sg | (uint64_t)X * sd;
             }
@@ -495,7 +506,11 @@
     }
     const uint64_t todo = __ballot(lane < nD && !simple);
     if (todo == 0) {
-        if (lane < nD) store_row(a, t_row, word, my_m, my_i);
+        if (COMPACT) {
+            if (lane < nD) a.compact[t_row] = my_c;
+        } else if (lane < nD) {
+            store_row(a, t_row, word, my_m, my_i);
+        }
         return;
     }
     const int combo = word * WAVE + lane;
@@ -552,7 +567,10 @@
         if (a.match_gt != nullptr && active)
             a.match_gt[(int64_t)(d0 + i) * n_combo + combo] = m;
     }
-    if (lane < nD) {
+    if (COMPACT) {
+        if (lane < nD) a.compact[t_row] = my_c;
+        if ((todo >> lane) & 1ull) store_row(a, t_row, word, my_m, my_i);
+    } else if (lane < nD) {
         store_row(a, t_row, word, my_m, my_i);
     }
 }
@@ -623,6 +641,7 @@
         if (lane == 0) {
             const int64_t rowi = a.dst != nullptr ? a.dst[d] : d;
             store_row(a, rowi, word, mw, iw);
+            if (a.compact != nullptr) a.compact[rowi] = TAOAMD_ROW_ESCAPE;
         }
         if (a.match_gt != nullptr && active)
             a.match_gt[(int64_t)d * n_combo + combo] = m;
@@ -761,21 +780,21 @@
     return TAOAMD_OK;
 }
 
-extern "C" int taoamd_match(int64_t n_cells, const int32_t *cell_dt_off,
-                            const int32_t *cell_gt_off,
-                            const int64_t *cell_iou_off,
-                            int32_t max_gt_per_cell, const double *dt_box,
-                            const double *gt_box, const double *iou,
-                            int32_t n_rng, const uint32_t *gt_rng,
-                            const uint32_t *dt_rng, const uint8_t *gt_flags,
-                            const uint8_t *dt_flags, const int32_t *dst,
-                            int64_t out_stride, uint64_t *matched,
-                            uint64_t *ignored, int32_t *match_gt,
-                            double *ious_out, const int32_t *dt_group,
-                            const uint32_t *dt_meta,
-                            const int32_t *groups, int32_t n_groups,
-                            const int32_t *singles, int32_t n_singles,
-                            void *stream)
+static int match_launch(int64_t n_cells, const int32_t *cell_dt_off,
+                        const int32_t *cell_gt_off,
+                        const int64_t *cell_iou_off,
+                        int32_t max_gt_per_cell, const double *dt_box,
+                        const double *gt_box, const double *iou,
+                        int32_t n_rng, const uint32_t *gt_rng,
+                        const uint32_t *dt_rng, const uint8_t *gt_flags,
+                        const uint8_t *dt_flags, const int32_t *dst,
+                        int64_t out_stride, uint64_t *matched,
+                        uint64_t *ignored, int32_t *match_gt,
+                        double *ious_out, const int32_t *dt_group,
+                        const uint32_t *dt_meta,
+                        const int32_t *groups, int32_t n_groups,
+                        const int32_t *singles, int32_t n_singles,
+                        uint32_t *compact, void *stream)
 {
     if (n_cells == 0) return TAOAMD_OK;
     if (n_rng < 1 || n_rng > 32) return TAOAMD_ERR_ARG;
@@ -802,12 +821,18 @@
     a.singles = planned ? singles : nullptr; a.n_singles = planned ? n_singles : 0;
     static const int xcd_env = getenv("TAOAMD_XCD") ? atoi(getenv("TAOAMD_XCD")) : 1;
     a.xcd = xcd_env;
+    a.compact = compact;
+    if (compact != nullptr &&
+        !(planned && fused && a.dt_meta && !a.dt_rng && !a.ious_out && !a.match_gt &&
+          a.n_words == 1 && n_rng <= 6 && !a.dst && a.wide && a.out_stride == 2))
+        return TAOAMD_ERR_ARG;
     hipStream_t s = (hipStream_t)stream;
     if (planned && n_groups > 0) {
         const unsigned gb = (unsigned)(((int64_t)n_groups * a.n_words + 3) / 4);
         const bool fast = fused && a.dt_meta && !a.dt_rng && !a.ious_out && !a.match_gt &&
                           a.n_words == 1 && n_rng <= 6;
         if (fast && a.dst) TAO_TIMED("match_group_kernel", s, (match_group_kernel<true, true><<<gb, 256, 0, s>>>(a, match_thr())));
+        else if (fast && compact) TAO_TIMED("match_group_kernel", s, (match_group_kernel<true, true, false, true><<<gb, 256, 0, s>>>(a, match_thr())));
         else if (fast) TAO_TIMED("match_group_kernel", s, (match_group_kernel<true, true, false><<<gb, 256, 0, s>>>(a, match_thr())));
         else if (fused) TAO_TIMED("match_group_kernel", s, match_group_kernel<true><<<gb, 256, 0, s>>>(a, match_thr()));
         else TAO_TIMED("match_group_kernel", s, match_group_kernel<false><<<gb, 256, 0, s>>>(a, match_thr()));
@@ -831,6 +856,82 @@
     return TAOAMD_OK;
 }
 
+extern "C" int taoamd_match(int64_t n_cells, const int32_t *cell_dt_off,
+                            const int32_t *cell_gt_off,
+                            const int64_t *cell_iou_off,
+                            int32_t max_gt_per_cell, const double *dt_box,
+                            const double *gt_box, const double *iou,
+                            int32_t n_rng, const uint32_t *gt_rng,
+                            const uint32_t *dt_rng, const uint8_t *gt_flags,
+                            const uint8_t *dt_flags, const int32_t *dst,
+                            int64_t out_stride, uint64_t *matched,
+                            uint64_t *ignored, int32_t *match_gt,
+                            double *ious_out, const int32_t *dt_group,
+                            const uint32_t *dt_meta,
+                            const int32_t *groups, int32_t n_groups,
+                            const int32_t *singles, int32_t n_singles,
+                            void *stream)
+{
+    return match_launch(n_cells, cell_dt_off, cell_gt_off, cell_iou_off, max_gt_per_cell,
+                        dt_box, gt_box, iou, n_rng, gt_rng, dt_rng, gt_flags, dt_flags, dst,
+                        out_stride, matched, ignored, match_gt, ious_out, dt_group, dt_meta,
+                        groups, n_groups, singles, n_singles, nullptr, stream);
+}
+
+extern "C" int taoamd_match_compact(int64_t n_cells, const int32_t *cell_dt_off,
+                                    const int32_t *cell_gt_off, int32_t max_gt_per_cell,
+                                    const double *dt_box, const double *gt_box,
+                                    int32_t n_rng, const uint32_t *gt_rng,
+                                    const uint8_t *gt_flags, const uint8_t *dt_flags,
+                                    uint64_t *rows, uint32_t *compact,
+                                    const int32_t *dt_group, const uint32_t *dt_meta,
+                                    const int32_t *groups, int32_t n_groups,
+                                    const int32_t *singles, int32_t n_singles,
+                                    void *stream)
+{
+    if (!compact || !rows || !dt_box) return TAOAMD_ERR_ARG;
+    return match_launch(n_cells, cell_dt_off, cell_gt_off, nullptr, max_gt_per_cell,
+                        dt_box, gt_box, nullptr, n_rng, gt_rng, nullptr, gt_flags, dt_flags,
+                        nullptr, 0, rows, rows + 1, nullptr, nullptr, dt_group, dt_meta,
+                        groups, n_groups, singles, n_singles, compact, stream);
+}
+
+__global__ __launch_bounds__(256) void expand_rows_kernel(int64_t n, uint32_t rmask,
+                                                          const uint32_t *__restrict__ compact,
+                                                          ulonglong2 *__restrict__ rows)
+{
+    constexpr uint64_t S_ALL = 1ull | 1ull << 10 | 1ull << 20 | 1ull << 30 |
+                               1ull << 40 | 1ull << 50;
+    constexpr uint64_t C9 = 1ull | 1ull << 9 | 1ull << 18 | 1ull << 27 |
+                            1ull << 36 | 1ull << 45;
+    const uint64_t sall = ((uint64_t)rmask * C9) & S_ALL;
+    for (int64_t d = blockIdx.x * (int64_t)blockDim.x + threadIdx.x; d < n;
+         d += (int64_t)gridDim.x * blockDim.x) {
+        const uint32_t w = compact[d];
+        if (w & TAOAMD_ROW_ESCAPE) continue;
+        const uint32_t m10 = w & 0x3ffu, g = (w >> 10) & rmask;
+        const bool un = (w >> 16) & 1u, hid = (w >> 17) & 1u;
+        const uint64_t sg = ((uint64_t)g * C9) & S_ALL;
+        const uint32_t X = hid ? 0x3ffu : (~m10 & 0x3ffu);
+        ulonglong2 v;
+        v.x = hid ? 0ull : (uint64_t)m10 * sall;
+        v.y = (uint64_t)m10 * sg | (un ? (uint64_t)X * sall : 0ull);
+        rows[d] = v;
+    }
+}
+
+extern "C" int taoamd_expand_rows(int64_t n_dt, int32_t n_rng, const uint32_t *compact,
+                                  uint64_t *rows, void *stream)
+{
+    if (n_dt == 0) return TAOAMD_OK;
+    if (n_rng < 1 || n_rng > 6 || !compact || !rows || ((uintptr_t)rows & 15)) return TAOAMD_ERR_ARG;
+    const unsigned blocks = (unsigned)((n_dt + 255) / 256 < 8192 ? (n_dt + 255) / 256 : 8192);
+    TAO_TIMED("expand_rows_kernel", (hipStream_t)stream, expand_rows_kernel<<<blocks, 256, 0, (hipStream_t)stream>>>(
+        n_dt, 0xffffffffu >> (32 - n_rng), compact, reinterpret_cast<ulonglong2 *>(rows)));
+    TAO_LAUNCH_CHECK();
+    return TAOAMD_OK;
+}
+
 __global__ void gather_rows_kernel(int64_t n, int32_t n_words,
                                    const uint64_t *__restrict__ sm,
                                    const uint64_t *__restrict__ si,
diff --git a/tao_amodal_amd/engine.py b/tao_amodal_amd/engine.py
--- a/tao_amodal_amd/engine.py
+++ b/tao_amodal_amd/engine.py
@@ -397,9 +397,14 @@
                               lib.taoamd_sort_sampled_workspace(
                                   dp.n_dt, dp.ss_sizes[3], int(dp.ss_merge)))
         self.sort_ws = buf(self.sort_bytes)
-        self.rows = torch.empty((max(dp.n_dt, 1), dp.n_words, 2),
-                                dtype=torch.int64, device=dev)
-        self.matched, self.ignored = self.rows[..., 0], self.rows[..., 1]
+        self._rows = torch.empty((max(dp.n_dt, 1), dp.n_words, 2),
+                                 dtype=torch.int64, device=dev)
+        self._matched, self._ignored = self._rows[..., 0], self._rows[..., 1]
+        self.compact_buf = torch.empty(max(dp.n_dt, 1), dtype=torch.int32, device=dev) \
+            if self.gather else None
+        self.rows_pending = False
+        self.rows_expanded = 0
+        self._dp = dp
         self.acc_bytes = lib.taoamd_accumulate_workspace(dp.n_dt, dp.n_cat,
                                                          dp.n_rng)
         self.acc_ws = buf(self.acc_bytes)
@@ -463,6 +468,23 @@
 Workspace.order = property(_order_of)
 
 
+def expand_rows(ws):
+    if ws.rows_pending:
+        dp = ws._dp
+        with torch.cuda.device(dp.device):
+            _lib.check(_lib.load().taoamd_expand_rows(
+                dp.n_dt, dp.n_rng, _ptr(ws.compact_buf), _ptr(ws._rows), _stream()),
+                "taoamd_expand_rows")
+        ws.rows_pending = False
+        ws.rows_expanded += 1
+    return ws
+
+
+Workspace.rows = property(lambda ws: expand_rows(ws)._rows)
+Workspace.matched = property(lambda ws: expand_rows(ws)._matched)
+Workspace.ignored = property(lambda ws: expand_rows(ws)._ignored)
+
+
 def stage_ranges(dp, ws):
     lib, t, s = _lib.load(), dp.t, _stream()
     if dp.kind == "lvis":
@@ -769,6 +791,18 @@
     fused = dp.kind == "lvis" and not dp.mask_iou
     if groups is None:
         ws.cell_order = not scatter
+    if (ws.gather and not scatter and groups is None and match_gt is None
+            and ws.match_gt is None and ws.ious_out is None):
+        _lib.check(lib.taoamd_match_compact(
+            dp.n_cells, _ptr(t["cell_dt_off"]), _ptr(t["cell_gt_off"]), dp.max_g,
+            _ptr(t["dt_box"]), _ptr(t["gt_box"]), dp.n_rng, _ptr(ws.gt_rng),
+            _ptr(t["gt_flags"]), _ptr(t["dt_flags"]), _ptr(ws._rows), _ptr(ws.compact_buf),
+            _ptr(t["dt_group"]), _ptr(t["dt_meta"]), g_ptr, n_g, s_ptr, n_s, s),
+            "taoamd_match_compact")
+        ws.rows_pending = True
+        return
+    if groups is None:
+        ws.rows_pending = False
     _lib.check(lib.taoamd_match(
         dp.n_cells, _ptr(t["cell_dt_off"]), _ptr(t["cell_gt_off"]),
         _ptr(t["cell_iou_off"]), dp.max_g,
@@ -786,7 +820,15 @@
 
 def stage_accumulate_by_order(dp, ws):
     lib, t, s = _lib.load(), dp.t, _stream()
-    fn = lib.taoamd_accumulate_by_order_prepared if ws.acc_prepared == _plan_key(dp) \
+    key = _plan_key(dp)
+    if ws.rows_pending and key[1] in (2, 3):
+        _lib.check(lib.taoamd_accumulate_by_order_compact(
+            dp.n_dt, dp.n_cat, dp.n_rng, _ptr(t["cat_off"]), _ptr(ws.order),
+            _ptr(ws.compact_buf), _ptr(ws._rows), _ptr(ws.num_gt), dp.acc_hint,
+            _ptr(ws.precision), _ptr(ws.recall), _ptr(ws.acc_ws), ws.acc_bytes,
+            int(ws.acc_prepared == key), s), "taoamd_accumulate_by_order_compact")
+        return
+    fn = lib.taoamd_accumulate_by_order_prepared if ws.acc_prepared == key \
         else lib.taoamd_accumulate_by_order
     _lib.check(fn(
         dp.n_dt, dp.n_cat, dp.n_rng, _ptr(t["cat_off"]), _ptr(ws.order),
```

New measurement: 44430 (median of 6 runs). 6.8% higher.
